# su1phurd/UAV-WRF-LES-PPO-LSTM

Hardware: AMD Instinct MI355X
Metric: env-steps/sec (rollout + GAE + 5-epoch PPO update), 4096 envs x 128 T per GPU, LSTM h=128 x1 (higher is better)
Workload: dtype f32

## Files before the change

### include/uavppo.h

```cpp
#ifndef UAVPPO_H
#define UAVPPO_H

#include <stddef.h>
#include <stdint.h>

#ifdef __cplusplus
extern "C" {
#endif

typedef struct uav_ctx uav_ctx;
typedef void* uav_stream;

#define UAV_ABI_VERSION 9

#define UAV_GAE_REFERENCE_EXACT 0
#define UAV_GAE_STANDARD        1
#define UAV_GAE_INLINE_V10      2

#define UAV_ENV_V20 0
#define UAV_ENV_V21 1
#define UAV_ENV_V11 2

#define UAV_FIELD_PROCEDURAL   0
#define UAV_FIELD_MATERIALISED 1

int         uav_abi_version(void);
const char* uav_last_error(void);

int  uav_create(uav_ctx** out, int device, size_t ws_bytes);
void uav_destroy(uav_ctx* ctx);

#define UAV_ARITH_FP16X3   0
#define UAV_ARITH_BF16X6   1
#define UAV_ARITH_F32_MFMA 2
int uav_set_lstm_arith(uav_ctx* ctx, int mode);
int uav_get_lstm_arith(const uav_ctx* ctx);
#define UAV_DEBUG_STEP_F32 1u
#define UAV_DEBUG_X_F32    2u
#define UAV_DEBUG_DG_F32   4u
#define UAV_DEBUG_GEMM_TN_OFF 0x10u
int uav_set_debug_flags(uav_ctx* ctx, unsigned flags);
int uav_absmax(uav_ctx* ctx, const float* x, int64_t n, float* out, uav_stream stream);

int uav_gae(uav_ctx* ctx, const float* rew, const float* val, const float* done,
            const float* last_val, int n_env, int horizon, float gamma, float lam, int mode,
            float* adv, uav_stream stream);

int uav_adv_stats(uav_ctx* ctx, const float* adv, int64_t n, double* stats3, uav_stream stream);
int uav_adv_normalise(uav_ctx* ctx, const float* adv, const float* val, int64_t n,
                      const double* stats3, float* adv_out, float* ret_out, uav_stream stream);
int uav_adv_normalise_inline(uav_ctx* ctx, const float* adv, const float* val, int64_t n,
                             const double* stats3, float* adv_out, float* ret_out, uav_stream stream);

int uav_pack_success_bits(uav_ctx* ctx, const uint8_t* flags, int64_t n, int cap, uint8_t* msg, uav_stream stream);

int uav_ppo_loss(uav_ctx* ctx, const float* logits, const float* value, const int32_t* act,
                 const float* logp_old, const float* adv, const float* ret, const float* val_old,
                 int64_t n, int n_act, float inv_n, float clip, float ent_beta,
                 double* loss_sums, float* dlogits, float* dvalue, float* dhead_bias,
                 uav_stream stream);

int uav_ppo_loss_from_y(uav_ctx* ctx, const float* y, const float* w_head, const float* b_head,
                        const int32_t* act, const float* logp_old, const float* adv, const float* ret,
                        const float* val_old, int64_t n, int hidden, int n_act, float inv_n, float clip,
                        float ent_beta, double* loss_sums, float* dheads, float* dhead_bias,
                        uav_stream stream);

int uav_policy_sample(uav_ctx* ctx, const float* logits, int64_t n, int n_act, const float* u,
                      uint64_t seed, uint64_t counter, int64_t index_offset, const int32_t* forced_act,
                      int32_t* act_out, float* logp_out, float* probs_out, int32_t* nan_count,
                      uav_stream stream);

int uav_policy_sample_at(uav_ctx* ctx, const float* heads, int64_t heads_stride, int64_t n, int n_act, uint64_t seed,
                         uint64_t counter, int64_t index_offset, const int32_t* forced_act, int32_t* act_out, int T, int t,
                         int32_t* act_buf, float* val_buf, float* logp_buf, int32_t* nan_count, uav_stream stream);
int uav_store_transition(uav_ctx* ctx, int n, int T, int t, float* keep, const float* rew, const float* done,
                         const uint8_t* flags, float* keep_buf, float* rew_buf, float* done_buf, uint8_t* flags_buf,
                         uav_stream stream);

int uav_clip_adam(uav_ctx* ctx, float* param, const float* grad, float* exp_avg,
                  float* exp_avg_sq, int64_t n, int64_t step, float lr, float beta1, float beta2,
                  float eps, float max_norm, float* gnorm_out, float* pmax_out, uav_stream stream);
int uav_clip_adamw(uav_ctx* ctx, float* param, const float* grad, float* exp_avg, float* exp_avg_sq, int64_t n,
                   int64_t step, float lr, float beta1, float beta2, float eps, float weight_decay, float max_norm,
                   float* gnorm_out, uav_stream stream);
int uav_smooth_l1(uav_ctx* ctx, const float* pred, const float* target, int64_t n, float beta, double* loss_mean,
                  float* dpred, uav_stream stream);
int uav_mse_bce(uav_ctx* ctx, const float* out, const float* target, int64_t n, double* loss_mean, float* dout,
                uav_stream stream);

size_t uav_disc_param_count(int obs_dim, int n_act, int hidden);

int uav_disc_grad(uav_ctx* ctx, const float* params, const float* obs_e, const int32_t* act_e, int64_t n_e, const float* obs_p,
                  const int32_t* act_p, int64_t n_p, int obs_dim, int n_act, int hidden, float inv_ne, float inv_np,
                  double* loss_sums, float* grad, uav_stream stream);

int uav_disc_reward(uav_ctx* ctx, const float* params, const float* obs, const int32_t* act, int64_t n, int obs_dim, int n_act,
                    int hidden, float env_coef, float gail_coef, const float* rew_env, float* rew_out, uav_stream stream);

size_t uav_lstm_stepper_bytes(int N, int I, int H);
int uav_lstm_stepper_begin(uav_ctx* ctx, void* state, const float* w_ih, const float* w_hh, const float* b_ih,
                           const float* b_hh, const float* h0, const float* c0, int N, int I, int H, uav_stream stream);
int uav_lstm_stepper_step(uav_ctx* ctx, void* state, const float* x, const void* below, const float* keep_t, int N, int T,
                          int t, int I, int H, float* y, float* stash, float* hn, float* cn, uav_stream stream);
typedef struct uav_stepper_call {
    void* state; const float* x; const void* below; const float* keep_t;
    int t, I;
    float *y, *stash, *hn, *cn;
} uav_stepper_call;
int uav_lstm_stepper_step_pair(uav_ctx* ctx, const uav_stepper_call* a, const uav_stepper_call* b, int N, int T, int H,
                               uav_stream stream);

int uav_gemm_f32(uav_ctx* ctx, int64_t M, int64_t N, int64_t K, const float* A, int64_t sa_m,
                 int64_t sa_k, const float* B, int64_t sb_k, int64_t sb_n, float* C, int64_t ldc,
                 const float* bias, int accumulate, uav_stream stream);

int uav_gemm_f16x3(uav_ctx* ctx, int64_t M, int64_t N, int64_t K, const float* A, int64_t sa_m,
                   int64_t sa_k, const float* B, int64_t sb_k, int64_t sb_n, float* C, int64_t ldc,
                   const float* bias, int accumulate, const float* a_absmax, uav_stream stream);

int uav_colsum(uav_ctx* ctx, const float* x, int64_t rows, int cols, float* out, uav_stream stream);
int uav_ln_relu(uav_ctx* ctx, float* z, float* a, float* rstd, const float* gamma, const float* beta, int64_t rows,
                int cols, uav_stream stream);
int uav_ln_relu_bwd(uav_ctx* ctx, float* d, const float* xhat, const float* rstd, const float* gamma, const float* beta,
                    int64_t rows, int cols, float* dgamma, float* dbeta, uav_stream stream);

int64_t uav_mlp_param_count(int in_dim, int h1, int h2, int n_act);
int64_t uav_mlp_stash_floats(int h1, int h2);
int uav_mlp_fwd(uav_ctx* ctx, const float* params, const float* x, int64_t B, int in_dim, int h1,
                int h2, int n_act, float* heads, float* stash, uav_stream stream);
int uav_mlp_bwd(uav_ctx* ctx, const float* params, const float* x, float* stash,
                const float* dheads, int64_t B, int in_dim, int h1, int h2, int n_act,
                float* grad, uav_stream stream);

int uav_mlp_ppo_grad(uav_ctx* ctx, const float* params, const float* obs, const int32_t* act, const float* logp_old,
                     const float* adv, const float* ret, const float* val_old, int64_t n, int in_dim, int h1, int h2,
                     int n_act, float inv_n, float clip, float ent_beta, double* loss_sums, float* grad,
                     uav_stream stream);

int uav_mlp_ppo_grad_trend(uav_ctx* ctx, const float* params, const float* obs, const int32_t* act, const float* logp_old,
                           const float* adv, const float* ret, const float* val_old, int64_t n, int trend_k, float inv_n,
                           float clip, float ent_beta, double* loss_sums, float* grad, uav_stream stream);

int uav_mlp_ppo_grad_rows(uav_ctx* ctx, const float* params, const float* obs, const int32_t* act, const float* logp_old,
                          const float* adv, const float* ret, const float* val_old, int64_t n_total, const int32_t* rows,
                          int64_t n_rows, int trend_k, float inv_n, float clip, float ent_beta, double* loss_sums, float* grad,
                          uav_stream stream);

typedef struct uav_gather_spec {
    const void* src;
    void* dst;
    int64_t row_bytes;
    int32_t planes;
    int32_t pad_;
    int64_t src_plane_stride_bytes;
    int64_t dst_plane_stride_bytes;
} uav_gather_spec;
#define UAV_GATHER_MAX_SPECS 12

int uav_gather_rows_multi(uav_ctx* ctx, const int32_t* idx, int64_t n_sel, int64_t n_rows, const uav_gather_spec* specs,
                          int n_specs, uav_stream stream);

int uav_lstm_fwd(uav_ctx* ctx, const float* x, const float* keep, const float* h0, const float* c0,
                 const float* w_ih, const float* w_hh, const float* b_ih, const float* b_hh,
                 int N, int T, int I, int H, float* y, float* hn, float* cn, float* stash,
                 const float* w_head, const float* b_head, int n_heads, float* heads,
                 uav_stream stream);
int uav_lstm_bwd(uav_ctx* ctx, const float* keep, const float* stash, const float* w_hh,
                 const float* dy, const float* dheads, const float* w_head, int n_heads,
                 const float* dhn, const float* dcn, int N, int T, int H, float* dgates, float* dh0,
                 float* dc0, const float* w_ih, int I, float* dx, uav_stream stream);
size_t uav_lstm_dgates_bytes(uav_ctx* ctx, int N, int T, int H);
int uav_lstm_dgates_f32(uav_ctx* ctx, const float* dgates, int N, int T, int H, float* out, uav_stream stream);
#define UAV_BWD_FUSES_DX 1
#define UAV_BWD_TAKES_DHEADS 2
#define UAV_BWD_STACKS 4
int uav_lstm_bwd_caps(uav_ctx* ctx, int I, int H);
typedef struct uav_lstm_bwd_layer {
    const float* keep;
    const float* stash;
    const float* w_hh;
    const float* w_ih;
    float* dgates;
    float* dx;
    const float* dhn;
    const float* dcn;
    float* dh0;
    float* dc0;
} uav_lstm_bwd_layer;
int uav_lstm_bwd_stack(uav_ctx* ctx, int n_layers, const uav_lstm_bwd_layer* layers, const float* dy, const float* dheads,
                       const float* w_head, int n_heads, int N, int T, int H, uav_stream stream);
int uav_lstm_wgrad(uav_ctx* ctx, const float* x, const float* keep, const float* h0, const float* y,
                   const float* stash, const float* dgates, const float* w_ih, const float* dheads,
                   int n_heads, int N, int T, int I, int H, float* dw_ih, float* dw_hh, float* db, float* db_hh,
                   float* dw_head, float* dx, uav_stream stream);
int uav_lstm_chunk_states(uav_ctx* ctx, const float* y, const float* stash, const float* keep, const float* h0, const float* c0,
                          int N, int T, int H, int chunk, float* h_out, float* c_out, uav_stream stream);

typedef struct uav_env_cfg {
    int32_t variant;
    int32_t field_mode;
    int32_t n_fields;
    int32_t bonus_is_f64;
    int32_t env_offset;
    int32_t n_env_total;
    int32_t trend_k;
    int32_t pad_;
    double  radius;
    double  bonus;
    uint64_t seed;
    const double* bank;
    const double* bank_src;
    const void*   curriculum;
} uav_env_cfg;

int uav_episode_rows(uav_ctx* ctx, const float* rew, const float* info, const uint8_t* flags, int n_env, int T, int env_offset,
                     double* carry, double* rows, int cap, int32_t* count, uav_stream stream);
size_t uav_curriculum_state_bytes(void);
int uav_curriculum_init(uav_ctx* ctx, void* state, double radius, double bonus, int bonus_is_f64, uav_stream stream);
int uav_curriculum_update(uav_ctx* ctx, void* state, const uint8_t* msgs, int world, int cap, uav_stream stream);

size_t uav_env_state_bytes(int n_env);
int uav_env_reset(uav_ctx* ctx, void* state, int n_env, const uav_env_cfg* cfg ,
                  float* obs_out, uav_stream stream);
int uav_env_step(uav_ctx* ctx, void* state, int n_env, const uav_env_cfg* cfg ,
                 const int32_t* act, const double* noise, float* obs_out, float* rew, float* done,
                 uint8_t* flags, float* info, float* term_obs, double* rew64, uav_stream stream);
int uav_env_peek(uav_ctx* ctx, const void* state, int n_env, float* pos, double* source,
                 int32_t* steps, int32_t* episode, uav_stream stream);

int uav_env_materialise(uav_ctx* ctx, const void* state, int n_env, const uav_env_cfg* cfg ,
                        int env_index, double* field_out, uav_stream stream);

int uav_rollout(uav_ctx* ctx, void* env_state, int n_env, const uav_env_cfg* cfg ,
                int policy_kind, const float* params, int hidden, int horizon, uint64_t iter,
                float* cur_obs, float* h, float* c, float* obs, int32_t* act, float* rew,
                float* val, float* logp, float* done, uint8_t* flags, float* keep, float* last_val,
                const int32_t* forced_act, const double* noise, int32_t* nan_count,
                float* stash, float* y_out, float* info, float* heads, uav_stream stream);

int uav_greedy_episodes(uav_ctx* ctx, void* env_state, int n_env, const uav_env_cfg* cfg , int policy_kind,
                        const float* params, int hidden, int steps, float* cur_obs, float* h, float* c, uint8_t* active,
                        const double* noise, int32_t* act, float* obs, float* pos, uint8_t* flags, int32_t* nan_count,
                        uav_stream stream);

typedef struct uav_stop_rule {
    int32_t window;
    float   pos_std_max, conc_coef, conc_peak, conc_min;
} uav_stop_rule;

int uav_greedy_episodes_stop(uav_ctx* ctx, void* env_state, int n_env, const uav_env_cfg* cfg , int policy_kind,
                             const float* params, int hidden, int steps, float* cur_obs, float* h, float* c, uint8_t* active,
                             const double* noise, int32_t* act, float* obs, float* pos, uint8_t* flags, int32_t* nan_count,
                             const uav_stop_rule* rule , float* stop_win, int32_t* stop_cnt, float* rule_val,
                             uav_stream stream);

int uav_stop_stability(uav_ctx* ctx, int n, const uav_stop_rule* rule , const float* pos, const float* obs2,
                       int64_t obs2_stride, const uint8_t* active, float* stop_win, int32_t* stop_cnt, uint8_t* stop,
                       float* value, uav_stream stream);

size_t uav_peak_stop_param_count(int hidden);

int uav_peak_stop_scan(uav_ctx* ctx, const float* params, int hidden, int window, const float* series, int64_t row_stride,
                       int64_t elem_stride, int n, int steps, const uint8_t* active, float* hist, int32_t* hist_cnt,
                       float prob_min, float* peak, float* prob, int32_t* first_hit, uav_stream stream);

int uav_threshold_windows(uav_ctx* ctx, const float* series, int64_t row_stride, int64_t elem_stride, int n, int steps,
                          const uint8_t* active, const float* hist, const int32_t* step_cnt, int window, int every, int min_steps,
                          double lo, double scale, double conc_scale, float* x, uav_stream stream);

int uav_threshold_rule(uav_ctx* ctx, const float* series, int64_t row_stride, int64_t elem_stride, int n, int steps,
                       const uint8_t* active, float* hist, int32_t* step_cnt, int window, int every, int min_steps, double conc_scale,
                       double factor, const float* pred, double* thr, int32_t* first_hit, uint8_t* stop, double* thr_out,
                       uav_stream stream);

int uav_rollout_tail(uav_ctx* ctx, void* env_state, int n_env, const uav_env_cfg* cfg , const float* y, int64_t y_stride,
                     int hidden, const float* w_head, const float* b_head, int n_act, float* heads, int64_t heads_stride, int T,
                     int t, uint64_t seed, uint64_t counter, int64_t index_offset, const int32_t* forced_act, const double* noise,
                     int32_t* act_out, float* cur_obs, float* obs_seq, float* keep, int32_t* act_buf, float* val_buf,
                     float* logp_buf, float* keep_buf, float* rew_buf, float* done_buf, uint8_t* flags_buf, int32_t* nan_count,
                     uav_stream stream);

int uav_greedy_tail(uav_ctx* ctx, void* env_state, int n_env, const uav_env_cfg* cfg , const float* y, int64_t y_stride,
                    int hidden, const float* w_head, const float* b_head, int n_act, int steps, int t, const double* noise_t,
                    float* cur_obs, uint8_t* active, int32_t* act, float* obs, float* pos, uint8_t* flags, int32_t* nan_count,
                    const uav_stop_rule* rule , float* stop_win, int32_t* stop_cnt, float* rule_val, uav_stream stream);

#define UAV_COMM_ID_BYTES 128
int uav_rccl_version(int* out );
int uav_comm_unique_id(void* id_out );
int uav_comm_init(uav_ctx* ctx, const void* id , int rank, int world);
int uav_comm_world(const uav_ctx* ctx);
int uav_comm_rank(const uav_ctx* ctx);
int uav_comm_destroy(uav_ctx* ctx);
int uav_allreduce(uav_ctx* ctx, float* flat_grad, int64_t count, uav_stream stream);
int uav_allreduce_f64(uav_ctx* ctx, double* buf, int64_t count, uav_stream stream);
int uav_allgather_bytes(uav_ctx* ctx, const void* send, void* recv, int64_t bytes_per_rank, uav_stream stream);

#ifdef __cplusplus
}
#endif
#endif
```

### uav-wrf-les-ppo-lstm_amd/csrc/common.h

```cpp
#pragma once
#include <hip/hip_runtime.h>
#include <stdint.h>
#include <stdio.h>
#include <stdlib.h>
#include <string.h>
#include "../../include/uavppo.h"

struct uav_form_table {
    struct { const void* p; int v; } e[8];
    int next;
    void record(const void* p, int v) {
        for (auto& x : e)
            if (x.p == p) { x.v = v; return; }
        e[next] = {p, v};
        next = (next + 1) % 8;
    }
    int find(const void* p) const {
        for (auto& x : e)
            if (x.p == p) return x.v;
        return -1;
    }
};
struct uav_ctx {
    int device;
    int num_cu;
    void* ws;
    size_t ws_bytes;
    double* pow075;
    double* wave;
    double* ftab;
    int lstm_arith;
    unsigned debug;
    hipStream_t side[3];
    hipEvent_t side_ev[8];
    void* comm;
    int comm_rank, comm_world;
    uav_form_table dg_form;
    uav_form_table hslot_form;
};
static inline void uav_dg_record(uav_ctx* ctx, const void* p, int packed) { ctx->dg_form.record(p, packed); }
static inline int uav_dg_form(const uav_ctx* ctx, const void* p) { return ctx->dg_form.find(p); }

extern thread_local int g_uav_arith;
extern thread_local unsigned g_uav_debug;
static inline bool uav_want_f32_mfma() { return g_uav_arith == UAV_ARITH_F32_MFMA; }
static inline bool uav_want_bf16x6() { return g_uav_arith == UAV_ARITH_BF16X6; }
static inline bool uav_debug(unsigned bit) { return (g_uav_debug & bit) != 0; }
static inline void uav_enter(const struct uav_ctx* ctx);

static inline void uav_enter(const uav_ctx* ctx) {
    g_uav_arith = ctx->lstm_arith;
    g_uav_debug = ctx->debug;
}

void uav_set_error(const char* fmt, ...);

hipError_t uav_dyn_lds(const void* kernel, int bytes);

#define UAV_CHECK_HIP(expr)                                                          \
    do {                                                                             \
        hipError_t e_ = (expr);                                                      \
        if (e_ != hipSuccess) {                                                      \
            uav_set_error("%s:%d: %s -> %s", __FILE__, __LINE__, #expr, hipGetErrorString(e_)); \
            return 1;                                                                \
        }                                                                            \
    } while (0)

#define UAV_REQUIRE(cond, ...)                                                       \
    do {                                                                             \
        if (!(cond)) {                                                               \
            uav_set_error(__VA_ARGS__);                                              \
            return 2;                                                                \
        }                                                                            \
    } while (0)

#define UAV_LAUNCH_CHECK() UAV_CHECK_HIP(hipGetLastError())

static inline hipStream_t as_stream(uav_stream s) { return reinterpret_cast<hipStream_t>(s); }

constexpr int WAVE = 64;

__device__ __forceinline__ void lds_barrier() {
    asm volatile("s_waitcnt lgkmcnt(0)\n\ts_barrier" ::: "memory");
}

__device__ __forceinline__ float fast_sigmoid(float x) { return __builtin_amdgcn_rcpf(1.0f + __expf(-x)); }
__device__ __forceinline__ float fast_tanh(float x) {
    const float big = 1.0f - 2.0f * __builtin_amdgcn_rcpf(__expf(2.0f * x) + 1.0f);
#ifdef UAV_TANH_LEGACY
    return big;
#else
    const float x2 = x * x;
    float p = __builtin_fmaf(x2, 62.0f / 2835.0f, -17.0f / 315.0f);
    p = __builtin_fmaf(p, x2, 2.0f / 15.0f);
    p = __builtin_fmaf(p, x2, -1.0f / 3.0f);
    p = __builtin_fmaf(p, x2, 1.0f);
    return __builtin_fabsf(x) < 0.25f ? x * p : big;
#endif
}

typedef __bf16 bf16x8 __attribute__((ext_vector_type(8)));
__device__ __forceinline__ void split3(float a, __bf16& p0, __bf16& p1, __bf16& p2) {
    p0 = (__bf16)a;
    const float r1 = a - (float)p0;
    p1 = (__bf16)r1;
    p2 = (__bf16)(r1 - (float)p1);
}
__device__ __forceinline__ unsigned short bf_bits(__bf16 v) { return __builtin_bit_cast(unsigned short, v); }

typedef _Float16 f16x8 __attribute__((ext_vector_type(8)));
constexpr float H3_LO = 1.0f / 2048.0f;
__device__ __forceinline__ void split2h(float a, _Float16& p0, _Float16& p1) {
    p0 = (_Float16)a;
    p1 = (_Float16)((a - (float)p0) * 2048.0f);
}
__device__ __forceinline__ unsigned short h_bits(_Float16 v) { return __builtin_bit_cast(unsigned short, v); }

typedef float f32x4 __attribute__((ext_vector_type(4)));

struct SplitF16x3 {
    typedef _Float16 piece;
    typedef f16x8 vec;
    static constexpr int NP = 2;
    static constexpr bool BLOCK_SCALE = true;
    static constexpr bool DG_STORES_LATE = true;
    static constexpr int fwd_park(int) { return 0; }
    static constexpr int bwd_park(int) { return 0; }
    __device__ __forceinline__ static void split(float a, piece (&p)[NP]) { split2h(a, p[0], p[1]); }
    __device__ __forceinline__ static unsigned short bits(piece v) { return h_bits(v); }
    __device__ __forceinline__ static f32x4 mma(vec a, vec b, f32x4 c) { return __builtin_amdgcn_mfma_f32_16x16x32_f16(a, b, c, 0, 0, 0); }
    template <class W>
    __device__ __forceinline__ static void gates_slab(f32x4 (&acc)[4], f32x4 (&acl)[4], W w, const vec (&a)[NP]) {
#pragma unroll
        for (int q = 0; q < 4; ++q) acl[q] = mma(w(q, 1), a[0], acl[q]);
#pragma unroll
        for (int q = 0; q < 4; ++q) acc[q] = mma(w(q, 0), a[0], acc[q]);
#pragma unroll
        for (int q = 0; q < 4; ++q) acl[q] = mma(w(q, 0), a[1], acl[q]);
    }
    template <class W, class B>
    __device__ __forceinline__ static void head_slab(f32x4& ha, f32x4& hb, W w, B h) {
        hb = mma(w(1), h(0), hb);
        hb = mma(w(0), h(1), hb);
        ha = mma(w(0), h(0), ha);
    }
    template <class V> __device__ __forceinline__ static V sum(V acc, V acl) { return acc + acl * H3_LO; }
    template <class W>
    __device__ __forceinline__ static void tile_slab(f32x4& a0, f32x4& a1, W w, const vec (&b)[NP]) {
        a1 = mma(w(1), b[0], a1);
        a0 = mma(w(0), b[0], a0);
        a1 = mma(w(0), b[1], a1);
    }
    __device__ __forceinline__ static f32x4 tile_sum(f32x4 a0, f32x4 a1) { return a0 + a1 * H3_LO; }
};

struct SplitBf16x6 {
    typedef __bf16 piece;
    typedef bf16x8 vec;
    static constexpr int NP = 3;
    static constexpr bool BLOCK_SCALE = false;
    static constexpr bool DG_STORES_LATE = false;
    static constexpr int fwd_park(int H) { return H >= 128 ? 3 : 0; }
    static constexpr int bwd_park(int H) { return H >= 128 ? 6 : 0; }
    __device__ __forceinline__ static void split(float a, piece (&p)[NP]) { split3(a, p[0], p[1], p[2]); }
    __device__ __forceinline__ static unsigned short bits(piece v) { return bf_bits(v); }
    __device__ __forceinline__ static f32x4 mma(vec a, vec b, f32x4 c) { return __builtin_amdgcn_mfma_f32_16x16x32_bf16(a, b, c, 0, 0, 0); }
    template <class W>
    __device__ __forceinline__ static void gates_slab(f32x4 (&acc)[4], f32x4 (&)[4], W w, const vec (&a)[NP]) {
#pragma unroll
        for (int q = 0; q < 4; ++q) acc[q] = mma(w(q, 0), a[2], acc[q]);
#pragma unroll
        for (int q = 0; q < 4; ++q) acc[q] = mma(w(q, 1), a[1], acc[q]);
#pragma unroll
        for (int q = 0; q < 4; ++q) acc[q] = mma(w(q, 2), a[0], acc[q]);
#pragma unroll
        for (int q = 0; q < 4; ++q) acc[q] = mma(w(q, 0), a[1], acc[q]);
#pragma unroll
        for (int q = 0; q < 4; ++q) acc[q] = mma(w(q, 1), a[0], acc[q]);
#pragma unroll
        for (int q = 0; q < 4; ++q) acc[q] = mma(w(q, 0), a[0], acc[q]);
    }
    template <class W, class B>
    __device__ __forceinline__ static void head_slab(f32x4& ha, f32x4&, W w, B h) {
        ha = mma(w(0), h(2), ha);
        ha = mma(w(1), h(1), ha);
        ha = mma(w(2), h(0), ha);
        ha = mma(w(0), h(1), ha);
        ha = mma(w(1), h(0), ha);
        ha = mma(w(0), h(0), ha);
    }
    template <class V> __device__ __forceinline__ static V sum(V acc, V) { return acc; }
    template <class W>
    __device__ __forceinline__ static void tile_slab(f32x4& a0, f32x4& a1, W w, const vec (&b)[NP]) {
        a0 = mma(w(0), b[2], a0);
        a1 = mma(w(1), b[1], a1);
        a0 = mma(w(2), b[0], a0);
        a1 = mma(w(0), b[1], a1);
        a0 = mma(w(1), b[0], a0);
        a1 = mma(w(0), b[0], a1);
    }
    __device__ __forceinline__ static f32x4 tile_sum(f32x4 a0, f32x4 a1) { return a0 + a1; }
};

struct DgPack {
    static constexpr int H = 256, NS = 4 * H / 32;
    int N, T, NP, RT;
    __host__ __device__ DgPack(int n, int t) : N(n), T(t), NP((n + 63) / 64 * 64), RT(NP / 16) {}
    __host__ __device__ size_t step_halves() const { return (size_t)RT * NS * 1024; }
    __host__ __device__ size_t piece_bytes() const { return (size_t)T * step_halves() * 2; }
    __host__ __device__ size_t bytes() const { return piece_bytes() + 2 * (size_t)T * NP * sizeof(float); }
    __host__ __device__ unsigned short* pieces(void* base, int t) const { return (unsigned short*)base + (size_t)t * step_halves(); }
    __host__ __device__ const unsigned short* pieces(const void* base, int t) const { return (const unsigned short*)base + (size_t)t * step_halves(); }
    __host__ __device__ float* isc(void* base, int t) const { return (float*)((char*)base + piece_bytes()) + (size_t)t * NP; }
    __host__ __device__ const float* isc(const void* base, int t) const { return (const float*)((const char*)base + piece_bytes()) + (size_t)t * NP; }
    __host__ __device__ float* iscm(void* base, int t) const { return isc(base, T) + (size_t)t * NP; }
    __host__ __device__ const float* iscm(const void* base, int t) const { return isc(base, T) + (size_t)t * NP; }
};

__device__ __forceinline__ double wave_sum(double v) {
#pragma unroll
    for (int o = 32; o > 0; o >>= 1) v += __shfl_down(v, o, 64);
    return v;
}
__device__ __forceinline__ float wave_sum(float v) {
#pragma unroll
    for (int o = 32; o > 0; o >>= 1) v += __shfl_down(v, o, 64);
    return v;
}
__device__ __forceinline__ float wave_allsum(float v) {
#pragma unroll
    for (int o = 32; o > 0; o >>= 1) v += __shfl_xor(v, o, 64);
    return v;
}
template <typename T>
__device__ __forceinline__ T block256_sum(T v, T* sm) {
    v = wave_sum(v);
    const int lane = threadIdx.x & 63, w = threadIdx.x >> 6;
    if (lane == 0) sm[w] = v;
    __syncthreads();
    T r = T(0);
    if (threadIdx.x == 0) r = ((sm[0] + sm[1]) + sm[2]) + sm[3];
    __syncthreads();
    return r;
}
```

### uav-wrf-les-ppo-lstm_amd/csrc/ctx.hip

```cpp
#include <stdarg.h>
#include <mutex>
#include <set>
#include <utility>
#include "common.h"

static thread_local char g_err[512] = "";
thread_local int g_uav_arith = 0;
thread_local unsigned g_uav_debug = 0;
int env_init_tables(uav_ctx* ctx);

void uav_set_error(const char* fmt, ...) {
    va_list ap;
    va_start(ap, fmt);
    vsnprintf(g_err, sizeof(g_err), fmt, ap);
    va_end(ap);
}

hipError_t uav_dyn_lds(const void* kernel, int bytes) {
    static std::mutex mu;
    static std::set<std::pair<int, const void*>> done;
    int dev = 0;
    hipError_t e = hipGetDevice(&dev);
    if (e != hipSuccess) return e;
    std::lock_guard<std::mutex> lock(mu);
    if (done.count({dev, kernel})) return hipSuccess;
    e = hipFuncSetAttribute(kernel, hipFuncAttributeMaxDynamicSharedMemorySize, bytes);
    if (e == hipSuccess) done.insert({dev, kernel});
    return e;
}

extern "C" {

int uav_abi_version(void) { return UAV_ABI_VERSION; }
const char* uav_last_error(void) { return g_err; }

int uav_create(uav_ctx** out, int device, size_t ws_bytes) {
    UAV_REQUIRE(out != nullptr, "uav_create: out is NULL");
    UAV_REQUIRE(ws_bytes >= (1u << 20), "uav_create: ws_bytes must be >= 1 MiB");
    UAV_CHECK_HIP(hipSetDevice(device));
    hipDeviceProp_t prop;
    UAV_CHECK_HIP(hipGetDeviceProperties(&prop, device));
    UAV_REQUIRE(strncmp(prop.gcnArchName, "gfx950", 6) == 0,
                "libuavppo is built for gfx950 (MI355X) only; device %d is %s", device, prop.gcnArchName);
    uav_ctx* c = new uav_ctx();
    c->device = device;
    c->num_cu = prop.multiProcessorCount;
    c->ws_bytes = ws_bytes;
    c->pow075 = nullptr;
    c->wave = nullptr;
    c->ftab = nullptr;
    c->comm = nullptr;
    c->comm_rank = -1;
    c->comm_world = 0;
    c->lstm_arith = getenv("UAV_LSTM_F32_MFMA") ? UAV_ARITH_F32_MFMA : (getenv("UAV_LSTM_BF16X6") ? UAV_ARITH_BF16X6 : UAV_ARITH_FP16X3);
    c->debug = (getenv("UAV_LSTM_STEP_F32") ? UAV_DEBUG_STEP_F32 : 0u) | (getenv("UAV_LSTM_X_F32") ? UAV_DEBUG_X_F32 : 0u) |
               (getenv("UAV_LSTM_DG_F32") ? UAV_DEBUG_DG_F32 : 0u);
    if (hipMalloc(&c->ws, ws_bytes) != hipSuccess) {
        (void)hipFree(c->ws);
        delete c;
        uav_set_error("uav_create: hipMalloc(%zu) failed", ws_bytes);
        return 1;
    }
    if (env_init_tables(c) != 0) {
        (void)hipFree(c->ws);
        (void)hipFree(c->pow075);
        (void)hipFree(c->wave);
        (void)hipFree(c->ftab);
        delete c;
        return 1;
    }
    *out = c;
    return 0;
}

int uav_set_lstm_arith(uav_ctx* ctx, int mode) {
    UAV_REQUIRE(ctx && mode >= UAV_ARITH_FP16X3 && mode <= UAV_ARITH_F32_MFMA, "uav_set_lstm_arith: bad argument");
    ctx->lstm_arith = mode;
    return 0;
}
int uav_get_lstm_arith(const uav_ctx* ctx) { return ctx ? ctx->lstm_arith : -1; }

int uav_set_debug_flags(uav_ctx* ctx, unsigned flags) {
    UAV_REQUIRE(ctx && (flags & ~(UAV_DEBUG_STEP_F32 | UAV_DEBUG_X_F32 | UAV_DEBUG_DG_F32 | UAV_DEBUG_GEMM_TN_OFF)) == 0, "uav_set_debug_flags: bad argument");
    ctx->debug = flags;
    return 0;
}

void uav_destroy(uav_ctx* ctx) {
    if (!ctx) return;
    (void)uav_comm_destroy(ctx);
    for (auto& e : ctx->side_ev)
        if (e) (void)hipEventDestroy(e);
    for (auto& s : ctx->side)
        if (s) (void)hipStreamDestroy(s);
    (void)hipFree(ctx->ws);
    (void)hipFree(ctx->pow075);
    (void)hipFree(ctx->wave);
    (void)hipFree(ctx->ftab);
    delete ctx;
}

}
```

### uav-wrf-les-ppo-lstm_amd/csrc/lstm.hip

```cpp
#include <stdlib.h>
#include <type_traits>
#include "common.h"

int gemm_f32(uav_ctx* ctx, int64_t M, int64_t N, int64_t K, const float* A, int64_t sa_m, int64_t sa_k,
             const float* B, int64_t sb_k, int64_t sb_n, float* C, int64_t ldc, const float* bias,
             int accumulate, hipStream_t st);
int colsum(uav_ctx* ctx, const float* X, int64_t B, int C, float* out, float* scratch, hipStream_t st);
int colsum_absmax(uav_ctx* ctx, const float* X, int64_t B, int C, float* out, float* scratch, unsigned* absmax_bits,
                  hipStream_t st);
int colsum_xw(uav_ctx* ctx, const float* X, int64_t B, int C, const float* x, int I, float* colsum_out, float* xw_out,
              float* scratch, unsigned* absmax_bits, hipStream_t st, int xw_transposed = 0);
bool gemm_h3_ok(int64_t M, int64_t N, int64_t K, const float* A, int64_t sa_m, int64_t sa_k, const float* B, int64_t sb_k,
                int64_t sb_n);
int gemm_h3(uav_ctx* ctx, int64_t M, int64_t N, int64_t K, const float* A, int64_t sa_m, int64_t sa_k, const float* B,
            int64_t sb_k, int64_t sb_n, float* C, int64_t ldc, const float* bias, int accumulate, const unsigned* a_absmax,
            hipStream_t st);
int lstm_generic_fwd(uav_ctx* ctx, const float* keep, const float* h0, const float* c0, const float* w_hh, int N, int T,
                     int H, float* y, float* hn, float* cn, float* stash, hipStream_t st);
int lstm_h3_fwd(uav_ctx* ctx, const float* x, int I, const float* w_ih, const float* b_ih, const float* b_hh,
                const float* keep, const float* h0, const float* c0, const float* w_hh, int N, int T, float* y, float* hn,
                float* cn, float* stash, hipStream_t st);
bool lstm_h3_step_path(int H);
int lstm_generic_bwd(uav_ctx* ctx, const float* keep, const float* stash, const float* w_hh, const float* dy,
                     const float* dheads, const float* w_head, int n_heads,
                     const float* dhn, const float* dcn, int N, int T, int H, float* dgates, float* dh0, float* dc0,
                     const float* w_ih, int I, float* dx, hipStream_t st);
int lstm_generic_bwd_caps(int I, int H);
bool lstm_h3_stack_ok(int H);
bool lstm_h3_dg_packed(int H);
int lstm_pc_unpack(const void* dgates, int N, int T, float* out, hipStream_t st);
int lstm_pc_hprev_rows(const float* y, const float* keep, const float* h0, int N, int T, float* out, hipStream_t st);
int lstm_pc_wgrad(uav_ctx* ctx, const float* x, const float* y, const float* h0, const void* dgates, int N, int T, int I, float* dw_ih,
                  float* dw_hh, float* db, float* db_hh, hipStream_t st);
int lstm_h3_bwd_stack(uav_ctx* ctx, int nl, const uav_lstm_bwd_layer* layers, const float* dy, const float* dheads,
                      const float* w_head, int n_heads, int N, int T, hipStream_t st);
int lstm_wgrad_fused(uav_ctx* ctx, const float* dgates, const float* y, const float* keep, const float* h0,
                     const float* x, int I, const float* dheads, int NH, int N, int T, int H,
                     float* dw_ih, float* dw_hh, float* db, float* db_hh, float* dw_head, hipStream_t st);

constexpr int MT = 16;
constexpr int TC = 32;

#define sigmoidf_ fast_sigmoid
#define tanhf_ fast_tanh

template <int H>
struct FwdGeom {
    static constexpr int NW = H / 16;
    static constexpr int KS = H / 4;
    static constexpr int SEG = KS + 4;
    static constexpr int S = 4 * SEG + 8;
    static constexpr size_t LDS = (2 * MT * S + TC * MT * 8 + (TC + 1) * MT) * sizeof(float);
};
template <int H>
__device__ __forceinline__ int hpos(int u) { return (u / (H / 4)) * FwdGeom<H>::SEG + (u % (H / 4)); }

template <int H, bool FUSE_X>
__global__ __launch_bounds__(H * 4) void lstm_fwd_kernel(
    const float* __restrict__ x, const float* __restrict__ keep, const float* __restrict__ h0,
    const float* __restrict__ c0, const float* __restrict__ w_ih, const float* __restrict__ w_hh,
    const float* __restrict__ b_ih, const float* __restrict__ b_hh, int N, int T, int I,
    float* __restrict__ y, float* __restrict__ hn, float* __restrict__ cn, float* __restrict__ stash) {
    using G = FwdGeom<H>;
    constexpr int KS = G::KS, SEG = G::SEG, S = G::S;
    extern __shared__ __attribute__((aligned(16))) float smem[];
    float* hbuf = smem;
    float* xbuf = hbuf + 2 * MT * S;
    float* kbuf = xbuf + TC * MT * 8;

    const int lane = threadIdx.x & 63, w = threadIdx.x >> 6;
    const int j = lane & 15, kq = lane >> 4;
    const int u = 16 * w + j;
    const int n0 = blockIdx.x * MT;

    float wh[4][KS];
#pragma unroll
    for (int q = 0; q < 4; ++q) {
        const float* src = w_hh + (size_t)(q * H + u) * H + kq * KS;
#pragma unroll
        for (int s = 0; s < KS; s += 4) {
            const float4 v = *reinterpret_cast<const float4*>(src + s);
            wh[q][s] = v.x; wh[q][s + 1] = v.y; wh[q][s + 2] = v.z; wh[q][s + 3] = v.w;
        }
    }
    float wx[4][2], bias[4];
#pragma unroll
    for (int q = 0; q < 4; ++q) {
        bias[q] = FUSE_X ? (b_ih[q * H + u] + b_hh[q * H + u]) : 0.f;
#pragma unroll
        for (int s = 0; s < 2; ++s) {
            const int k = 2 * kq + s;
            wx[q][s] = (FUSE_X && k < I) ? w_ih[(size_t)(q * H + u) * I + k] : 0.f;
        }
    }

    float c_reg[4], hin[4];
#pragma unroll
    for (int r = 0; r < 4; ++r) {
        const int e = 4 * kq + r;
        const int n = min(n0 + e, N - 1);
        const float k0 = keep ? keep[(size_t)n * T] : 1.f;
        c_reg[r] = c0[(size_t)n * H + u] * k0;
        hin[r] = h0[(size_t)n * H + u] * k0;
        hbuf[e * S + hpos<H>(u)] = hin[r];
    }
    int cur = 0;
    float h_last[4] = {0.f, 0.f, 0.f, 0.f};

    for (int t0 = 0; t0 < T; t0 += TC) {
        const int tc = min(TC, T - t0);
        if (FUSE_X) {
            for (int idx = threadIdx.x; idx < MT * tc * 8; idx += blockDim.x) {
                const int e = idx / (tc * 8), rem = idx % (tc * 8), tt = rem >> 3, f = rem & 7;
                const int n = min(n0 + e, N - 1);
                xbuf[(tt * MT + e) * 8 + f] = (f < I) ? x[((size_t)n * T + t0 + tt) * I + f] : 0.f;
            }
        }
        for (int idx = threadIdx.x; idx < MT * (tc + 1); idx += blockDim.x) {
            const int e = idx / (tc + 1), tt = idx % (tc + 1);
            const int n = min(n0 + e, N - 1);
            kbuf[tt * MT + e] = (keep && t0 + tt < T) ? keep[(size_t)n * T + t0 + tt] : 1.f;
        }
        lds_barrier();

        for (int tt = 0; tt < tc; ++tt) {
            const int t = t0 + tt;
            f32x4 acc[4];
#pragma unroll
            for (int q = 0; q < 4; ++q) {
                if (FUSE_X) {
                    acc[q] = f32x4{bias[q], bias[q], bias[q], bias[q]};
                } else {
#pragma unroll
                    for (int r = 0; r < 4; ++r) {
                        const int n = min(n0 + 4 * kq + r, N - 1);
                        acc[q][r] = stash[((size_t)n * T + t) * (6 * H) + q * H + u];
                    }
                }
            }
            if (FUSE_X) {
                const float2 ax = *reinterpret_cast<const float2*>(&xbuf[(tt * MT + j) * 8 + 2 * kq]);
#pragma unroll
                for (int q = 0; q < 4; ++q) {
                    acc[q] = __builtin_amdgcn_mfma_f32_16x16x4f32(ax.x, wx[q][0], acc[q], 0, 0, 0);
                    acc[q] = __builtin_amdgcn_mfma_f32_16x16x4f32(ax.y, wx[q][1], acc[q], 0, 0, 0);
                }
            }
            const float* hrow = hbuf + cur * MT * S + j * S + kq * SEG;
#pragma unroll
            for (int s = 0; s < KS; s += 4) {
                const float4 a = *reinterpret_cast<const float4*>(hrow + s);
#pragma unroll
                for (int q = 0; q < 4; ++q) acc[q] = __builtin_amdgcn_mfma_f32_16x16x4f32(a.x, wh[q][s], acc[q], 0, 0, 0);
#pragma unroll
                for (int q = 0; q < 4; ++q) acc[q] = __builtin_amdgcn_mfma_f32_16x16x4f32(a.y, wh[q][s + 1], acc[q], 0, 0, 0);
#pragma unroll
                for (int q = 0; q < 4; ++q) acc[q] = __builtin_amdgcn_mfma_f32_16x16x4f32(a.z, wh[q][s + 2], acc[q], 0, 0, 0);
#pragma unroll
                for (int q = 0; q < 4; ++q) acc[q] = __builtin_amdgcn_mfma_f32_16x16x4f32(a.w, wh[q][s + 3], acc[q], 0, 0, 0);
            }
            float* hnext = hbuf + (cur ^ 1) * MT * S;
#pragma unroll
            for (int r = 0; r < 4; ++r) {
                const int e = 4 * kq + r;
                const int n = n0 + e;
                const float gi = sigmoidf_(acc[0][r]), gf = sigmoidf_(acc[1][r]);
                const float gg = tanhf_(acc[2][r]), go = sigmoidf_(acc[3][r]);
                const float cp = c_reg[r];
                const float c = gf * cp + gi * gg;
                const float h = go * tanhf_(c);
                const float kn = kbuf[(tt + 1) * MT + e];
                if (n < N) {
                    const size_t row = (size_t)n * T + t;
                    y[row * H + u] = h;
                    if (stash) {
                        float* sp = stash + row * (6 * H);
                        sp[u] = gi; sp[H + u] = gf; sp[2 * H + u] = gg; sp[3 * H + u] = go;
                        sp[4 * H + u] = cp;
                        if (I > 6) sp[5 * H + u] = hin[r];
                    }
                }
                h_last[r] = h;
                if (t == T - 1) c_reg[r] = c;
                else c_reg[r] = c * kn;
                hin[r] = h * kn;
                hnext[e * S + hpos<H>(u)] = hin[r];
            }
            cur ^= 1;
            lds_barrier();
// ... 299 lines not shown
    float* __restrict__ y, float* __restrict__ hn, float* __restrict__ cn, float* __restrict__ stash,
    const float* __restrict__ w_head, const float* __restrict__ b_head, int NHD, float* __restrict__ heads) {
    lstm_fwd_split<SplitBf16x6, H, FUSE_X>(x, keep, h0, c0, w_ih, w_hh, b_ih, b_hh, N, T, I, y, hn, cn, stash, w_head,
                                           b_head, NHD, heads);
}

template <int H>
struct BwdGeom {
    static constexpr int S = 4 * H + 4;
    static constexpr size_t LDS = (2 * MT * S + TC * MT * 8 + (TC + 1) * MT) * sizeof(float);
};

template <int H>
__global__ __launch_bounds__(H * 4) void lstm_bwd_kernel(
    const float* __restrict__ keep, const float* __restrict__ stash, const float* __restrict__ w_hh,
    const float* __restrict__ dy, const float* __restrict__ dheads, const float* __restrict__ w_head, int NH,
    const float* __restrict__ dhn, const float* __restrict__ dcn, int N, int T, float* __restrict__ dgates,
    float* __restrict__ dh0, float* __restrict__ dc0) {
    using G = BwdGeom<H>;
    constexpr int S = G::S;
    extern __shared__ __attribute__((aligned(16))) float smem[];
    float* dgbuf = smem;
    float* dhbuf = dgbuf + 2 * MT * S;
    float* kbuf = dhbuf + TC * MT * 8;

    const int lane = threadIdx.x & 63, w = threadIdx.x >> 6;
    const int j = lane & 15, kq = lane >> 4;
    const int u = 16 * w + j;
    const int n0 = blockIdx.x * MT;

    float wt[H];
#pragma unroll
    for (int s = 0; s < H; ++s) wt[s] = w_hh[(size_t)(kq * H + s) * H + u];
    float whb[2];
#pragma unroll
    for (int a = 0; a < 2; ++a) whb[a] = (dheads && 4 * a + kq < NH) ? w_head[(size_t)(4 * a + kq) * H + u] : 0.f;

    float dh_rec[4], dc_next[4];
    size_t srow[4];
#pragma unroll
    for (int r = 0; r < 4; ++r) {
        const int n = min(n0 + 4 * kq + r, N - 1);
        dh_rec[r] = dhn ? dhn[(size_t)n * H + u] : 0.f;
        dc_next[r] = dcn ? dcn[(size_t)n * H + u] : 0.f;
        srow[r] = (size_t)n * T;
    }
    float pf[4][5], pdy[4];
    auto prefetch = [&](int t) {
#pragma unroll
        for (int r = 0; r < 4; ++r) {
            const float* sp = stash + (srow[r] + t) * (6 * H);
            pf[r][0] = sp[u]; pf[r][1] = sp[H + u]; pf[r][2] = sp[2 * H + u]; pf[r][3] = sp[3 * H + u];
            pf[r][4] = sp[4 * H + u];
            pdy[r] = dy ? dy[(srow[r] + t) * H + u] : 0.f;
        }
    };
    prefetch(T - 1);
    int cur = 0;
    const int nchunk = (T + TC - 1) / TC;
    for (int ch = nchunk - 1; ch >= 0; --ch) {
        const int t0 = ch * TC, tc = min(TC, T - t0);
        if (dheads) {
            for (int idx = threadIdx.x; idx < MT * tc * 8; idx += blockDim.x) {
                const int e = idx / (tc * 8), rem = idx % (tc * 8), tt = rem >> 3, f = rem & 7;
                const int n = min(n0 + e, N - 1);
                dhbuf[(tt * MT + e) * 8 + f] = (f < NH) ? dheads[((size_t)n * T + t0 + tt) * NH + f] : 0.f;
            }
        }
        for (int idx = threadIdx.x; idx < MT * tc; idx += blockDim.x) {
            const int e = idx / tc, tt = idx % tc;
            const int n = min(n0 + e, N - 1);
            kbuf[tt * MT + e] = keep ? keep[(size_t)n * T + t0 + tt] : 1.f;
        }
        lds_barrier();
        for (int tt = tc - 1; tt >= 0; --tt) {
            const int t = t0 + tt;
            float* dgw = dgbuf + cur * MT * S;
            f32x4 dyacc = {0.f, 0.f, 0.f, 0.f};
            if (dheads) {
                const float* dr = &dhbuf[(tt * MT + j) * 8];
                dyacc = __builtin_amdgcn_mfma_f32_16x16x4f32(dr[kq], whb[0], dyacc, 0, 0, 0);
                dyacc = __builtin_amdgcn_mfma_f32_16x16x4f32(dr[4 + kq], whb[1], dyacc, 0, 0, 0);
            }
#pragma unroll
            for (int r = 0; r < 4; ++r) {
                const int e = 4 * kq + r;
                const float gi = pf[r][0], gf = pf[r][1], gg = pf[r][2], go = pf[r][3], cp = pf[r][4];
                const float dyv = dheads ? dyacc[r] : pdy[r];
                const float dh = dyv + dh_rec[r];
                const float c = gf * cp + gi * gg;
                const float tch = tanhf_(c);
                const float dc = dh * go * (1.0f - tch * tch) + dc_next[r];
                const float dgi = dc * gg * gi * (1.0f - gi);
                const float dgf = dc * cp * gf * (1.0f - gf);
                const float dgg = dc * gi * (1.0f - gg * gg);
                const float dgo = dh * tch * go * (1.0f - go);
                const float kp = kbuf[tt * MT + e];
                dc_next[r] = dc * gf * kp;
                dgw[e * S + 0 * H + u] = dgi;
                dgw[e * S + 1 * H + u] = dgf;
                dgw[e * S + 2 * H + u] = dgg;
                dgw[e * S + 3 * H + u] = dgo;
                if (n0 + e < N) {
                    float* gp = dgates + (srow[r] + t) * (4 * H);
                    gp[u] = dgi; gp[H + u] = dgf; gp[2 * H + u] = dgg; gp[3 * H + u] = dgo;
                }
            }
            if (t > 0) prefetch(t - 1);
            lds_barrier();
            f32x4 a0 = {0.f, 0.f, 0.f, 0.f}, a1 = a0, a2 = a0, a3 = a0;
            const float* drow = dgw + j * S + kq * H;
#pragma unroll
            for (int s = 0; s < H; s += 4) {
                const float4 a = *reinterpret_cast<const float4*>(drow + s);
                a0 = __builtin_amdgcn_mfma_f32_16x16x4f32(a.x, wt[s], a0, 0, 0, 0);
                a1 = __builtin_amdgcn_mfma_f32_16x16x4f32(a.y, wt[s + 1], a1, 0, 0, 0);
                a2 = __builtin_amdgcn_mfma_f32_16x16x4f32(a.z, wt[s + 2], a2, 0, 0, 0);
                a3 = __builtin_amdgcn_mfma_f32_16x16x4f32(a.w, wt[s + 3], a3, 0, 0, 0);
            }
#pragma unroll
            for (int r = 0; r < 4; ++r) {
                const float kp = kbuf[tt * MT + 4 * kq + r];
                dh_rec[r] = ((a0[r] + a1[r]) + (a2[r] + a3[r])) * kp;
            }
            cur ^= 1;
        }
        lds_barrier();
    }
#pragma unroll
    for (int r = 0; r < 4; ++r) {
        const int n = n0 + 4 * kq + r;
        if (n < N) {
            if (dh0) dh0[(size_t)n * H + u] = dh_rec[r];
            if (dc0) dc0[(size_t)n * H + u] = dc_next[r];
        }
    }
}

template <class P, int H>
struct BwdSplitGeom {
    static constexpr int NW = H / 16;
    static constexpr int SLOT = 5 * MT * 16;
    static constexpr int SMALL = 128;
    static constexpr int PK = P::bwd_park(H);
    static constexpr int WPARK = PK * 64 * 8;
    static constexpr size_t LDS = (NW * NW * 64 * 4  + NW * SLOT + 2 * SMALL) * sizeof(float) +
                                  NW * WPARK * sizeof(unsigned short);
};

template <class P, int H>
__device__ __forceinline__ void lstm_bwd_split(
    const float* __restrict__ keep, const float* __restrict__ stash, const float* __restrict__ w_hh,
    const float* __restrict__ dheads, const float* __restrict__ w_head, int NH, const float* __restrict__ dhn,
    const float* __restrict__ dcn, int N, int T, float* __restrict__ dgates, float* __restrict__ dh0,
    float* __restrict__ dc0) {
    using G = BwdSplitGeom<P, H>;
    using vec = typename P::vec;
    using piece = typename P::piece;
    constexpr int NP = P::NP, SLOT = G::SLOT, NW = G::NW, SMALL = G::SMALL, PK = G::PK, WPARK = G::WPARK;
    extern __shared__ __attribute__((aligned(16))) float smem[];
    f32x4* part = reinterpret_cast<f32x4*>(smem);
    float* ring = smem + NW * NW * 64 * 4;
    float* small = ring + NW * SLOT;
    unsigned short* wpark = reinterpret_cast<unsigned short*>(small + 2 * SMALL);

    const int lane = threadIdx.x & 63;
    const int w = __builtin_amdgcn_readfirstlane(threadIdx.x >> 6);
    const int j = lane & 15, kq = lane >> 4;
    const int uw = 16 * w + j;
    const int uo = 16 * w + 4 * kq;
    const int n0 = blockIdx.x * MT;
    const int n = min(n0 + j, N - 1);
    const bool live = n0 + j < N;

    vec wa[NW][2][NP];
    vec* const wpk = reinterpret_cast<vec*>(wpark + w * WPARK) + lane;
#pragma unroll
    for (int m = 0; m < NW; ++m)
#pragma unroll
        for (int sb = 0; sb < 2; ++sb) {
#pragma unroll
            for (int e = 0; e < 8; ++e) {
                const int k = (2 * sb + e / 4) * H + 16 * w + 4 * kq + (e % 4);
                piece p[NP];
                P::split(w_hh[(size_t)k * H + 16 * m + j], p);
#pragma unroll
                for (int pc = 0; pc < NP; ++pc) wa[m][sb][pc][e] = p[pc];
            }
            if (2 * m + sb < PK) wpk[(2 * m + sb) * 64] = wa[m][sb][NP - 1];
        }
    float whb[2];
#pragma unroll
    for (int a = 0; a < 2; ++a) whb[a] = (4 * a + kq < NH) ? w_head[(size_t)(4 * a + kq) * H + uw] : 0.f;

    float dh_rec[4], dc_next[4];
    {
        const float4 a4 = dhn ? *reinterpret_cast<const float4*>(dhn + (size_t)n * H + uo) : float4{0.f, 0.f, 0.f, 0.f};
        const float4 c4 = dcn ? *reinterpret_cast<const float4*>(dcn + (size_t)n * H + uo) : float4{0.f, 0.f, 0.f, 0.f};
        dh_rec[0] = a4.x; dh_rec[1] = a4.y; dh_rec[2] = a4.z; dh_rec[3] = a4.w;
        dc_next[0] = c4.x; dc_next[1] = c4.y; dc_next[2] = c4.z; dc_next[3] = c4.w;
    }
    const size_t srow = (size_t)n * T;

    typedef __attribute__((address_space(3))) float lds_f;
    const int e_d = lane >> 2, g4 = lane & 3;
    const size_t drow = (size_t)min(n0 + e_d, N - 1) * T;
    const unsigned ring_base = __builtin_amdgcn_readfirstlane((unsigned)(unsigned long)((lds_f*)(ring + w * SLOT)));
    const unsigned small_base = __builtin_amdgcn_readfirstlane((unsigned)(unsigned long)((lds_f*)small));
    auto issue = [&](int t) {
        const float* src = stash + (drow + t) * (6 * H) + 16 * w + 4 * g4;
        unsigned m0save;
        asm volatile(
            "s_mov_b32 %0, m0\n\t"
            "s_mov_b32 m0, %6\n\ts_nop 0\n\tglobal_load_lds_dwordx4 %1, off\n\t"
            "s_add_u32 m0, m0, 1024\n\ts_nop 0\n\tglobal_load_lds_dwordx4 %2, off\n\t"
            "s_add_u32 m0, m0, 1024\n\ts_nop 0\n\tglobal_load_lds_dwordx4 %3, off\n\t"
            "s_add_u32 m0, m0, 1024\n\ts_nop 0\n\tglobal_load_lds_dwordx4 %4, off\n\t"
            "s_add_u32 m0, m0, 1024\n\ts_nop 0\n\tglobal_load_lds_dwordx4 %5, off\n\t"
            "s_mov_b32 m0, %0"
            : "=&s"(m0save)
            : "v"(src), "v"(src + H), "v"(src + 2 * H), "v"(src + 3 * H), "v"(src + 4 * H), "s"(ring_base)
            : "memory", "scc");
    };
    const float* small_at0;
    unsigned small_stride;
    {
        const int e = w * 64 + lane;
        if (e < 16 * NH) { small_at0 = dheads + (size_t)min(n0 + e / NH, N - 1) * T * NH + e % NH; small_stride = (unsigned)NH; }
        else if (e >= 112 && keep) { small_at0 = keep + (size_t)min(n0 + e - 112, N - 1) * T; small_stride = 1u; }
        else { small_at0 = w_hh + (lane & 15); small_stride = 0u; }
    }
    auto issue_small = [&](int t, int slot) {
        const float* src = small_at0 + (size_t)((unsigned)t * small_stride);
        const unsigned dst = small_base + (unsigned)((slot * SMALL + w * 64) * 4);
        unsigned m0save;
        asm volatile("s_mov_b32 %0, m0\n\ts_mov_b32 m0, %2\n\ts_nop 0\n\tglobal_load_lds_dword %1, off\n\ts_mov_b32 m0, %0"
                     : "=&s"(m0save) : "v"(src), "s"(dst) : "memory");
    };
    const bool small_wave = w < 2;
    issue(T - 1);
    if (small_wave) {
        issue_small(T - 1, (T - 1) & 1);
        issue_small(T >= 2 ? T - 2 : 0, (T - 2) & 1);
    }
    bool first = true;
    X6_PROF_DECL;
    for (int t = T - 1; t >= 0; --t) {
        X6_PROF_MARK(0);
        if (first) asm volatile("s_waitcnt vmcnt(0)" ::: "memory");
        else if (small_wave) asm volatile("s_waitcnt vmcnt(5)" ::: "memory");
        else asm volatile("s_waitcnt vmcnt(4)" ::: "memory");
        first = false;
        const float* sl = ring + w * SLOT + j * 16 + 4 * kq;
        float4 pf[5];
#pragma unroll
        for (int q = 0; q < 5; ++q) pf[q] = *reinterpret_cast<const float4*>(sl + q * 256);
        asm volatile("s_waitcnt lgkmcnt(0)" ::: "memory");
        issue(t >= 1 ? t - 1 : 0);
        X6_PROF_MARK(1);
        lds_barrier();
        X6_PROF_MARK(2);
        const float* sm = small + (t & 1) * SMALL;
        f32x4 dyacc = {0.f, 0.f, 0.f, 0.f};
        {
            const float d0 = (kq < NH) ? sm[j * NH + kq] : 0.f;
            const float d1 = (4 + kq < NH) ? sm[j * NH + 4 + kq] : 0.f;
            dyacc = __builtin_amdgcn_mfma_f32_16x16x4f32(whb[0], d0, dyacc, 0, 0, 0);
            dyacc = __builtin_amdgcn_mfma_f32_16x16x4f32(whb[1], d1, dyacc, 0, 0, 0);
        }
        const float kp = keep ? sm[112 + j] : 1.f;
        const float gi[4] = {pf[0].x, pf[0].y, pf[0].z, pf[0].w}, gf[4] = {pf[1].x, pf[1].y, pf[1].z, pf[1].w};
        const float gg[4] = {pf[2].x, pf[2].y, pf[2].z, pf[2].w}, go[4] = {pf[3].x, pf[3].y, pf[3].z, pf[3].w};
        const float cp[4] = {pf[4].x, pf[4].y, pf[4].z, pf[4].w};
        float dg[4][4];
#pragma unroll
        for (int r = 0; r < 4; ++r) {
            const float dh = dyacc[r] + dh_rec[r];
            const float c = __builtin_fmaf(gf[r], cp[r], gi[r] * gg[r]);
            const float tch = tanhf_(c);
            const float dc = dh * go[r] * (1.0f - tch * tch) + dc_next[r];
            dg[0][r] = dc * gg[r] * gi[r] * (1.0f - gi[r]);
            dg[1][r] = dc * cp[r] * gf[r] * (1.0f - gf[r]);
            dg[2][r] = dc * gi[r] * (1.0f - gg[r] * gg[r]);
            dg[3][r] = dh * tch * go[r] * (1.0f - go[r]);
            dc_next[r] = dc * gf[r] * kp;
        }
        int ex = 0;
        float unscale = 1.f;
        if constexpr (P::BLOCK_SCALE) {
            float mx = 0.f;
#pragma unroll
            for (int q = 0; q < 4; ++q)
#pragma unroll
                for (int r = 0; r < 4; ++r) mx = fmaxf(mx, fabsf(dg[q][r]));
            {
                const unsigned u = __builtin_bit_cast(unsigned, mx);
                const auto s16 = __builtin_amdgcn_permlane16_swap(u, u, false, false);
                mx = fmaxf(__builtin_bit_cast(float, (unsigned)s16[0]), __builtin_bit_cast(float, (unsigned)s16[1]));
                const unsigned v = __builtin_bit_cast(unsigned, mx);
                const auto s32 = __builtin_amdgcn_permlane32_swap(v, v, false, false);
                mx = fmaxf(__builtin_bit_cast(float, (unsigned)s32[0]), __builtin_bit_cast(float, (unsigned)s32[1]));
            }
            ex = 14 - __builtin_amdgcn_frexp_expf(mx);
            ex = mx > 0.f ? min(max(ex, -100), 100) : 0;
            unscale = __builtin_amdgcn_ldexpf(1.0f, -ex);
        }
        auto store_dg = [&](int q) {
            if (live) *reinterpret_cast<float4*>(dgates + (srow + t) * (4 * H) + q * H + uo) = float4{dg[q][0], dg[q][1], dg[q][2], dg[q][3]};
        };
        vec bp[2][NP];
#pragma unroll
        for (int q = 0; q < 4; ++q) {
#pragma unroll
            for (int r = 0; r < 4; ++r) {
                piece p[NP];
                P::split(P::BLOCK_SCALE ? __builtin_amdgcn_ldexpf(dg[q][r], ex) : dg[q][r], p);
#pragma unroll
                for (int pc = 0; pc < NP; ++pc) bp[q >> 1][pc][4 * (q & 1) + r] = p[pc];
            }
            if constexpr (!P::DG_STORES_LATE) store_dg(q);
        }
        X6_PROF_DEP(bp[1][NP - 1]); X6_PROF_DEP(bp[0][0]);
        X6_PROF_MARK(3);
#pragma unroll
        for (int m = 0; m < NW; ++m) {
            f32x4 a0 = {0.f, 0.f, 0.f, 0.f}, a1 = a0;
#pragma unroll
            for (int sb = 0; sb < 2; ++sb) {
                const int item = 2 * m + sb;
                P::tile_slab(a0, a1, [&](int p) { return (p == NP - 1 && item < PK) ? wpk[item * 64] : wa[m][sb][p]; }, bp[sb]);
            }
            part[(m * NW + w) * 64 + lane] = P::tile_sum(a0, a1) * unscale;
        }
        if constexpr (P::DG_STORES_LATE) {
#pragma unroll
            for (int q = 0; q < 4; ++q) store_dg(q);
        }
        asm volatile("s_waitcnt lgkmcnt(0)" ::: "memory");
        X6_PROF_MARK(4);
        lds_barrier();
        X6_PROF_MARK(5);
        if (small_wave) issue_small(t >= 2 ? t - 2 : 0, t & 1);
        f32x4 sum = part[(w * NW) * 64 + lane];
#pragma unroll
        for (int ww = 1; ww < NW; ++ww) sum += part[(w * NW + ww) * 64 + lane];
#pragma unroll
        for (int r = 0; r < 4; ++r) dh_rec[r] = sum[r] * kp;
        X6_PROF_DEP(dh_rec[3]);
        X6_PROF_MARK(6);
    }
    X6_PROF_FLUSH8();
    asm volatile("s_waitcnt vmcnt(0)" ::: "memory");
    if (live) {
        if (dh0) *reinterpret_cast<float4*>(dh0 + (size_t)n * H + uo) = float4{dh_rec[0], dh_rec[1], dh_rec[2], dh_rec[3]};
        if (dc0) *reinterpret_cast<float4*>(dc0 + (size_t)n * H + uo) = float4{dc_next[0], dc_next[1], dc_next[2], dc_next[3]};
    }
}

template <int H>
__global__ __launch_bounds__(H * 4) void lstm_bwd_h3k_kernel(
    const float* __restrict__ keep, const float* __restrict__ stash, const float* __restrict__ w_hh,
    const float* __restrict__ dheads, const float* __restrict__ w_head, int NH, const float* __restrict__ dhn,
    const float* __restrict__ dcn, int N, int T, float* __restrict__ dgates, float* __restrict__ dh0,
    float* __restrict__ dc0) {
    lstm_bwd_split<SplitF16x3, H>(keep, stash, w_hh, dheads, w_head, NH, dhn, dcn, N, T, dgates, dh0, dc0);
}
template <int H>
__global__ __launch_bounds__(H * 4) void lstm_bwd_x6k_kernel(
    const float* __restrict__ keep, const float* __restrict__ stash, const float* __restrict__ w_hh,
    const float* __restrict__ dheads, const float* __restrict__ w_head, int NH, const float* __restrict__ dhn,
    const float* __restrict__ dcn, int N, int T, float* __restrict__ dgates, float* __restrict__ dh0,
    float* __restrict__ dc0) {
    lstm_bwd_split<SplitBf16x6, H>(keep, stash, w_hh, dheads, w_head, NH, dhn, dcn, N, T, dgates, dh0, dc0);
}

template <class P, int H, bool FUSE_X>
static constexpr auto fwd_split_kernel() {
    if constexpr (std::is_same<P, SplitF16x3>::value) return &lstm_fwd_h3_kernel<H, FUSE_X>;
    else return &lstm_fwd_x6_kernel<H, FUSE_X>;
}
template <class P, int H>
static constexpr auto bwd_split_kernel() {
    if constexpr (std::is_same<P, SplitF16x3>::value) return &lstm_bwd_h3k_kernel<H>;
    else return &lstm_bwd_x6k_kernel<H>;
}

template <class F>
static int with_split(F&& f) {
    return uav_want_bf16x6() ? f(SplitBf16x6{}) : f(SplitF16x3{});
}

template <class P, int H>
static int launch_bwd_split(const float* keep, const float* stash, const float* w_hh, const float* dheads,
                            const float* w_head, int NH, const float* dhn, const float* dcn, int N, int T, float* dgates,
                            float* dh0, float* dc0, hipStream_t st) {
    const dim3 grid((N + MT - 1) / MT), block(H * 4);
    const size_t lx = BwdSplitGeom<P, H>::LDS;
    constexpr auto kern = bwd_split_kernel<P, H>();
    UAV_CHECK_HIP(uav_dyn_lds(reinterpret_cast<const void*>(kern), (int)lx));
    hipLaunchKernelGGL(kern, grid, block, lx, st, keep, stash, w_hh, dheads, w_head, NH, dhn, dcn, N, T, dgates, dh0, dc0);
    UAV_LAUNCH_CHECK();
    return 0;
}

template <class P, int H>
static int launch_fwd_split(bool fuse, const float* x, const float* keep, const float* h0, const float* c0,
                            const float* w_ih, const float* w_hh, const float* b_ih, const float* b_hh, int N, int T, int I,
                            float* y, float* hn, float* cn, float* stash, const float* w_head, const float* b_head, int NHD,
                            float* heads, hipStream_t st) {
    const dim3 grid((N + MT - 1) / MT), block(H * 4);
    const size_t lx = FwdSplitGeom<P, H>::LDS;
    constexpr auto fused = fwd_split_kernel<P, H, true>(), unfused = fwd_split_kernel<P, H, false>();
    UAV_CHECK_HIP(uav_dyn_lds(reinterpret_cast<const void*>(fused), (int)lx));
    UAV_CHECK_HIP(uav_dyn_lds(reinterpret_cast<const void*>(unfused), (int)lx));
    hipLaunchKernelGGL(fuse ? fused : unfused, grid, block, lx, st, x, keep, h0, c0, w_ih, w_hh, b_ih, b_hh, N, T, I, y, hn,
                       cn, stash, w_head, b_head, NHD, heads);
    UAV_LAUNCH_CHECK();
    return 0;
}

template <int H>
static int launch_fwd(bool fuse, const float* x, const float* keep, const float* h0, const float* c0,
                      const float* w_ih, const float* w_hh, const float* b_ih, const float* b_hh, int N, int T, int I,
                      float* y, float* hn, float* cn, float* stash, const float* w_head, const float* b_head, int NHD,
                      float* heads, bool* heads_done, hipStream_t st) {
    if (!uav_want_f32_mfma()) {
        *heads_done = heads != nullptr;
        return with_split([&](auto p) {
            return launch_fwd_split<decltype(p), H>(fuse, x, keep, h0, c0, w_ih, w_hh, b_ih, b_hh, N, T, I, y, hn, cn, stash,
                                                    w_head, b_head, NHD, heads, st);
        });
    }
    const dim3 grid((N + MT - 1) / MT), block(H * 4);
    const size_t lds = FwdGeom<H>::LDS;
    if (fuse)
        hipLaunchKernelGGL((lstm_fwd_kernel<H, true>), grid, block, lds, st, x, keep, h0, c0, w_ih, w_hh, b_ih, b_hh, N,
                           T, I, y, hn, cn, stash);
    else
        hipLaunchKernelGGL((lstm_fwd_kernel<H, false>), grid, block, lds, st, x, keep, h0, c0, w_ih, w_hh, b_ih, b_hh,
                           N, T, I, y, hn, cn, stash);
    UAV_LAUNCH_CHECK();
    return 0;
}

template <int H>
static int launch_bwd(const float* keep, const float* stash, const float* w_hh, const float* dy, const float* dheads,
                      const float* w_head, int NH, const float* dhn, const float* dcn, int N, int T, float* dgates,
                      float* dh0, float* dc0, hipStream_t st) {
    const dim3 grid((N + MT - 1) / MT), block(H * 4);
    UAV_CHECK_HIP(uav_dyn_lds(reinterpret_cast<const void*>(&lstm_bwd_kernel<H>), (int)BwdGeom<H>::LDS));
    hipLaunchKernelGGL((lstm_bwd_kernel<H>), grid, block, BwdGeom<H>::LDS, st, keep, stash, w_hh, dy, dheads, w_head, NH,
                       dhn, dcn, N, T, dgates, dh0, dc0);
    UAV_LAUNCH_CHECK();
    return 0;
}

__global__ void add2_kernel(const float* a0, const float* a1, float* b, int n) {
    const int i = blockIdx.x * 256 + threadIdx.x;
    if (i < n) b[i] = a0[i] + a1[i];
}

static int lstm_bwd_seq(const float* keep, const float* stash, const float* w_hh, const float* dy,
                        const float* dheads, const float* w_head, int NH, const float* dhn, const float* dcn, int N,
                        int T, int H, float* dgates, float* dh0, float* dc0, hipStream_t st) {
    if (dheads && NH <= 7 && !uav_want_f32_mfma()) {
        return with_split([&](auto p) {
            using P = decltype(p);
            return H == 64 ? launch_bwd_split<P, 64>(keep, stash, w_hh, dheads, w_head, NH, dhn, dcn, N, T, dgates, dh0, dc0, st)
                           : launch_bwd_split<P, 128>(keep, stash, w_hh, dheads, w_head, NH, dhn, dcn, N, T, dgates, dh0, dc0, st);
        });
    }
    switch (H) {
        case 64: return launch_bwd<64>(keep, stash, w_hh, dy, dheads, w_head, NH, dhn, dcn, N, T, dgates, dh0, dc0, st);
        case 128: return launch_bwd<128>(keep, stash, w_hh, dy, dheads, w_head, NH, dhn, dcn, N, T, dgates, dh0, dc0, st);
    }
    uav_set_error("uav_lstm_bwd: H=%d unsupported (64, 128)", H);
    return 2;
}

extern "C" {

int uav_lstm_fwd(uav_ctx* ctx, const float* x, const float* keep, const float* h0, const float* c0, const float* w_ih,
                 const float* w_hh, const float* b_ih, const float* b_hh, int N, int T, int I, int H, float* y,
                 float* hn, float* cn, float* stash, const float* w_head, const float* b_head, int n_heads, float* heads,
                 uav_stream stream) {
    UAV_REQUIRE(ctx && x && h0 && c0 && w_ih && w_hh && b_ih && b_hh && y && hn && cn, "uav_lstm_fwd: NULL argument");
    uav_enter(ctx);
    UAV_REQUIRE(N > 0 && T > 0 && I > 0, "uav_lstm_fwd: N=%d T=%d I=%d", N, T, I);
    UAV_REQUIRE(!heads || (w_head && b_head && n_heads > 0 && n_heads <= 8), "uav_lstm_fwd: heads needs w_head, b_head, 1..8 heads");
    hipStream_t st = as_stream(stream);
    const bool persistent = (H == 64 || H == 128);
    const bool fuse = I <= 8 && persistent;
    const bool step256 = lstm_h3_step_path(H);
    if (step256) UAV_REQUIRE(stash, "uav_lstm_fwd: stash is required when H is not 64/128");
    if (!fuse && !step256) {
        UAV_REQUIRE(stash, "uav_lstm_fwd: stash is required when I > 8 or H is not 64/128");
        float* bsum = (float*)ctx->ws;
        uav_ctx sub = *ctx;
        sub.ws = (char*)ctx->ws + 65536;
        sub.ws_bytes = ctx->ws_bytes - 65536;
        hipLaunchKernelGGL(add2_kernel, dim3((4 * H + 255) / 256), dim3(256), 0, st, b_ih, b_hh, bsum, 4 * H);
        int rc = gemm_f32(&sub, (int64_t)N * T, 4 * H, I, x, I, 1, w_ih, 1, I, stash, 6 * H, bsum, 0, st);
        if (rc) return rc;
    }
    bool heads_done = false;
    int rc;
    switch (H) {
        case 64: rc = launch_fwd<64>(fuse, x, keep, h0, c0, w_ih, w_hh, b_ih, b_hh, N, T, I, y, hn, cn, stash, w_head, b_head, n_heads, heads, &heads_done, st); break;
        case 128: rc = launch_fwd<128>(fuse, x, keep, h0, c0, w_ih, w_hh, b_ih, b_hh, N, T, I, y, hn, cn, stash, w_head, b_head, n_heads, heads, &heads_done, st); break;
        default:
            rc = step256 ? lstm_h3_fwd(ctx, x, I, w_ih, b_ih, b_hh, keep, h0, c0, w_hh, N, T, y, hn, cn, stash, st)
                         : lstm_generic_fwd(ctx, keep, h0, c0, w_hh, N, T, H, y, hn, cn, stash, st);
    }
    if (rc) return rc;
    if (H == DgPack::H) ctx->hslot_form.record(stash, step256 && lstm_h3_dg_packed(H) ? 0 : 1);
    if (heads && !heads_done)
        return gemm_f32(ctx, (int64_t)N * T, n_heads, H, y, H, 1, w_head, 1, H, heads, n_heads, b_head, 0, st);
    return 0;
}

int uav_lstm_bwd_caps(uav_ctx* ctx, int I, int H) {
    if (!ctx) return 0;
    if (H == 64 || H == 128) return UAV_BWD_TAKES_DHEADS;
    uav_enter(ctx);
    return lstm_generic_bwd_caps(I, H);
}

size_t uav_lstm_dgates_bytes(uav_ctx* ctx, int N, int T, int H) {
    if (!ctx || N <= 0 || T <= 0 || H <= 0) return 0;
    uav_enter(ctx);
    if (H == DgPack::H && lstm_h3_dg_packed(H)) return DgPack(N, T).bytes();
    return (size_t)N * T * 4 * H * sizeof(float);
}

int uav_lstm_dgates_f32(uav_ctx* ctx, const float* dgates, int N, int T, int H, float* out, uav_stream stream) {
    UAV_REQUIRE(ctx && dgates && out && N > 0 && T > 0 && H > 0, "uav_lstm_dgates_f32: bad argument");
    uav_enter(ctx);
    const int form = H == DgPack::H ? uav_dg_form(ctx, dgates) : 0;
    if (form > 0 || (form < 0 && H == DgPack::H && lstm_h3_dg_packed(H))) return lstm_pc_unpack(dgates, N, T, out, as_stream(stream));
    UAV_CHECK_HIP(hipMemcpyAsync(out, dgates, (size_t)N * T * 4 * H * sizeof(float), hipMemcpyDeviceToDevice, as_stream(stream)));
    return 0;
}

int uav_lstm_bwd_stack(uav_ctx* ctx, int n_layers, const uav_lstm_bwd_layer* layers, const float* dy, const float* dheads,
                       const float* w_head, int n_heads, int N, int T, int H, uav_stream stream) {
    UAV_REQUIRE(ctx && layers, "uav_lstm_bwd_stack: NULL argument");
    uav_enter(ctx);
    UAV_REQUIRE((dy != nullptr) != (dheads != nullptr), "uav_lstm_bwd_stack: give exactly one of dy / dheads");
    UAV_REQUIRE(!dheads || (w_head && n_heads > 0 && n_heads <= 8), "uav_lstm_bwd_stack: dheads needs w_head and 1..8 heads");
    UAV_REQUIRE(N > 0 && T > 0, "uav_lstm_bwd_stack: N=%d T=%d", N, T);
    UAV_REQUIRE(H == 256 && lstm_h3_stack_ok(H), "uav_lstm_bwd_stack: H = 256 on the fp16-split arithmetic only (uav_lstm_bwd_caps)");
    return lstm_h3_bwd_stack(ctx, n_layers, layers, dy, dheads, w_head, n_heads, N, T, as_stream(stream));
}

int uav_lstm_bwd(uav_ctx* ctx, const float* keep, const float* stash, const float* w_hh, const float* dy,
                 const float* dheads, const float* w_head, int n_heads, const float* dhn, const float* dcn, int N,
                 int T, int H, float* dgates, float* dh0, float* dc0, const float* w_ih, int I, float* dx,
                 uav_stream stream) {
    UAV_REQUIRE(ctx && stash && w_hh && dgates, "uav_lstm_bwd: NULL argument");
    uav_enter(ctx);
    UAV_REQUIRE((dy != nullptr) != (dheads != nullptr), "uav_lstm_bwd: give exactly one of dy / dheads");
    UAV_REQUIRE(!dheads || (w_head && n_heads > 0 && n_heads <= 8), "uav_lstm_bwd: dheads needs w_head and 1..8 heads");
    UAV_REQUIRE(N > 0 && T > 0, "uav_lstm_bwd: N=%d T=%d", N, T);
    if (H != 64 && H != 128) {
        return lstm_generic_bwd(ctx, keep, stash, w_hh, dy, dheads, w_head, n_heads, dhn, dcn, N, T, H, dgates, dh0, dc0, w_ih, I, dx,
                                as_stream(stream));
    }
    UAV_REQUIRE(!dx, "uav_lstm_bwd: dx is not formed by the H = 64 / 128 sequence kernels (uav_lstm_wgrad does it)");
    return lstm_bwd_seq(keep, stash, w_hh, dy, dheads, w_head, n_heads, dhn, dcn, N, T, H, dgates, dh0, dc0,
                        as_stream(stream));
}

int uav_lstm_wgrad(uav_ctx* ctx, const float* x, const float* keep, const float* h0, const float* y,
                   const float* stash, const float* dgates, const float* w_ih, const float* dheads, int n_heads, int N,
                   int T, int I, int H, float* dw_ih, float* dw_hh, float* db, float* db_hh, float* dw_head, float* dx,
                   uav_stream stream) {
    UAV_REQUIRE(ctx && x && h0 && y && dgates && w_ih && dw_ih && dw_hh && db, "uav_lstm_wgrad: NULL argument");
    uav_enter(ctx);
    UAV_REQUIRE(N > 0 && T > 0 && I > 0 && H > 0, "uav_lstm_wgrad: N=%d T=%d I=%d H=%d", N, T, I, H);
    UAV_REQUIRE(!dheads || (dw_head && n_heads > 0 && n_heads <= 8), "uav_lstm_wgrad: dheads needs dw_head, 1..8 heads");
    hipStream_t st = as_stream(stream);
    const int64_t NT = (int64_t)N * T;
    int rc;
    if (I <= 6 && (H == 64 || H == 128)) {
        if ((rc = lstm_wgrad_fused(ctx, dgates, y, keep, h0, x, I, dheads, n_heads, N, T, H, dw_ih, dw_hh, db, db_hh,
                                   dw_head, st))) return rc;
    } else {
        UAV_REQUIRE(stash, "uav_lstm_wgrad: stash is required when I > 6");
        const size_t red_floats = (size_t)1024 * 9 * 4 * H + 64;
        UAV_REQUIRE(ctx->ws_bytes >= red_floats * sizeof(float) * 2, "uav_lstm_wgrad: workspace too small");
        float* red = (float*)((char*)ctx->ws + ctx->ws_bytes) - red_floats;
        uav_ctx sub = *ctx;
        sub.ws_bytes = ctx->ws_bytes - red_floats * sizeof(float);
        bool done = false;
        const float* hprev = stash + 5 * H;
        int64_t ld_hprev = 6 * H;
        {
            const int form = uav_dg_form(ctx, dgates), want = lstm_h3_dg_packed(H) ? 1 : 0;
            UAV_REQUIRE(form < 0 || H != DgPack::H || form == want, "uav_lstm_wgrad: this dgates buffer was written as %s but the handle's "
                        "arithmetic mode / debug flags now read %s (they must not change between uav_lstm_bwd and uav_lstm_wgrad)",
                        form ? "fp16 piece chunks" : "f32 rows", want ? "fp16 piece chunks" : "f32 rows");
            UAV_REQUIRE(H != DgPack::H || want || ctx->hslot_form.find(stash) != 0, "uav_lstm_wgrad: this stash was written by "
                        "uav_lstm_fwd / the stepper on the fp16-split arithmetic, which leaves out its h_prev slot, but the handle's "
                        "arithmetic mode / debug flags now read that slot (they must not change between the forward pass and "
                        "uav_lstm_wgrad)");
        }
        if (lstm_h3_dg_packed(H)) {
            if ((I <= 8 || I == H) && !dx) {
                if ((rc = lstm_pc_wgrad(ctx, x, y, h0, dgates, N, T, I, dw_ih, dw_hh, db, db_hh, st))) return rc;
                done = true;
            } else {
                const size_t f32_bytes = (size_t)NT * 5 * H * sizeof(float);
                UAV_REQUIRE(sub.ws_bytes >= f32_bytes + (64u << 20), "uav_lstm_wgrad (h=256, I=%d%s): needs %zu bytes of workspace for "
                            "the gate gradients and h_prev as f32 rows", I, dx ? ", dx" : "", f32_bytes + (64u << 20));
                float* rows = (float*)((char*)sub.ws + sub.ws_bytes - f32_bytes);
                sub.ws_bytes -= f32_bytes;
                if ((rc = lstm_pc_unpack(dgates, N, T, rows, st))) return rc;
                float* hp = rows + (size_t)NT * 4 * H;
                if ((rc = lstm_pc_hprev_rows(y, keep, h0, N, T, hp, st))) return rc;
                dgates = rows;
                hprev = hp;
                ld_hprev = H;
            }
        }
        const bool h3 = !uav_want_f32_mfma() && !uav_want_bf16x6() && (reinterpret_cast<uintptr_t>(dgates) & 15) == 0;
        unsigned* amax = h3 ? reinterpret_cast<unsigned*>(red + (size_t)1024 * 9 * 4 * H) : nullptr;
        auto product = [&](int64_t M, int64_t Nn, int64_t K, const float* A, int64_t sa_m, int64_t sa_k, const float* B,
                           int64_t sb_k, int64_t sb_n, float* C, int64_t ldc) {
            if (h3 && gemm_h3_ok(M, Nn, K, A, sa_m, sa_k, B, sb_k, sb_n))
                return gemm_h3(&sub, M, Nn, K, A, sa_m, sa_k, B, sb_k, sb_n, C, ldc, nullptr, 0, amax, st);
            return gemm_f32(&sub, M, Nn, K, A, sa_m, sa_k, B, sb_k, sb_n, C, ldc, nullptr, 0, st);
        };
        if (!done) {
            const bool narrow = I <= 8 && (reinterpret_cast<uintptr_t>(dgates) & 15) == 0;
            if (narrow) rc = colsum_xw(&sub, dgates, NT, 4 * H, x, I, db, dw_ih, red, amax, st);
            else rc = colsum_absmax(&sub, dgates, NT, 4 * H, db, red, amax, st);
            if (rc) return rc;
            if (db_hh) UAV_CHECK_HIP(hipMemcpyAsync(db_hh, db, (size_t)4 * H * sizeof(float), hipMemcpyDeviceToDevice, st));
            if ((rc = product(4 * H, H, NT, dgates, 1, 4 * H, hprev, ld_hprev, 1, dw_hh, H))) return rc;
            if (!narrow && (rc = product(4 * H, I, NT, dgates, 1, 4 * H, x, I, 1, dw_ih, I))) return rc;
        }
        if (dheads) {
            if (H % 4 == 0 && (reinterpret_cast<uintptr_t>(y) & 15) == 0)
                rc = colsum_xw(&sub, y, NT, H, dheads, n_heads, nullptr, dw_head, red, nullptr, st, 1);
            else
                rc = gemm_f32(&sub, n_heads, H, NT, dheads, 1, n_heads, y, H, 1, dw_head, H, nullptr, 0, st);
            if (rc) return rc;
        }
        if (dx) return product(NT, I, 4 * H, dgates, 4 * H, 1, w_ih, I, 1, dx, I);
        return 0;
    }
    if (dx) return gemm_f32(ctx, NT, I, 4 * H, dgates, 4 * H, 1, w_ih, I, 1, dx, I, nullptr, 0, st);
    return 0;
}

}
```

### uav-wrf-les-ppo-lstm_amd/csrc/wgrad.hip

```cpp
#include <stdlib.h>
#include <type_traits>
#include "common.h"

typedef float f32x4 __attribute__((ext_vector_type(4)));

constexpr int KC = 16;

template <int H>
struct WG {
    static constexpr int NW = H / 16;
    static constexpr int NT_ = H / 16 + 1;
    static constexpr int NC = H + 16;
    static constexpr int SG = 4 * H + 16;
    static constexpr int SB = H + 16;
    static constexpr int SY = H + 16;
    static constexpr int SD = 48;
    static constexpr int BUF = KC * (SG + SB + SY + SD);
    static constexpr size_t LDS = 2 * BUF * sizeof(float);
    static constexpr size_t SLAB = (size_t)4 * H * NC + 16 * H;
};

template <int H>
__global__ __launch_bounds__(H * 4) void lstm_wgrad_kernel(
    const float* __restrict__ dgates, const float* __restrict__ y, const float* __restrict__ keep,
// ... 95 lines not shown
            for (int mi = 0; mi < 4; ++mi) a[mi] = lg[kr * SG + 64 * w + 16 * mi + j];
#pragma unroll
            for (int ni = 0; ni < NT_; ++ni) b[ni] = lb[kr * SB + 16 * ni + j];
            const float ah = ld[kr * SD + j];
            const float bh = ly[kr * SY + 16 * w + j];
#pragma unroll
            for (int mi = 0; mi < 4; ++mi)
#pragma unroll
                for (int ni = 0; ni < NT_; ++ni)
                    acc[mi][ni] = __builtin_amdgcn_mfma_f32_16x16x4f32(a[mi], b[ni], acc[mi][ni], 0, 0, 0);
            acch = __builtin_amdgcn_mfma_f32_16x16x4f32(ah, bh, acch, 0, 0, 0);
        }
    }
    float* slab = slabs + (size_t)blockIdx.x * G::SLAB;
#pragma unroll
    for (int mi = 0; mi < 4; ++mi)
#pragma unroll
        for (int ni = 0; ni < NT_; ++ni)
#pragma unroll
            for (int r = 0; r < 4; ++r)
                slab[(size_t)(64 * w + 16 * mi + 4 * kq + r) * G::NC + 16 * ni + j] = acc[mi][ni][r];
#pragma unroll
    for (int r = 0; r < 4; ++r) slab[(size_t)4 * H * G::NC + (size_t)(4 * kq + r) * H + 16 * w + j] = acch[r];
}


constexpr int KS6 = 32;

__device__ __forceinline__ void mac6(f32x4& d, const bf16x8 (&a)[3], const bf16x8 (&b)[3]) {
    d = __builtin_amdgcn_mfma_f32_16x16x32_bf16(a[2], b[0], d, 0, 0, 0);
    d = __builtin_amdgcn_mfma_f32_16x16x32_bf16(a[1], b[1], d, 0, 0, 0);
    d = __builtin_amdgcn_mfma_f32_16x16x32_bf16(a[0], b[2], d, 0, 0, 0);
    d = __builtin_amdgcn_mfma_f32_16x16x32_bf16(a[1], b[0], d, 0, 0, 0);
    d = __builtin_amdgcn_mfma_f32_16x16x32_bf16(a[0], b[1], d, 0, 0, 0);
    d = __builtin_amdgcn_mfma_f32_16x16x32_bf16(a[0], b[0], d, 0, 0, 0);
}

template <class P>
__device__ __forceinline__ void split8(const float (&v)[8], typename P::vec (&p)[P::NP]) {
#pragma unroll
    for (int i = 0; i < 8; ++i) {
        typename P::piece q[P::NP];
        P::split(v[i], q);
#pragma unroll
        for (int k = 0; k < P::NP; ++k) p[k][i] = q[k];
    }
}

struct WgBf16x6 {
    typedef __bf16 piece;
    typedef bf16x8 vec;
    static constexpr int NP = 3;
    static constexpr float BSCALE = 1.0f, XSCALE = 1.0f;
    static constexpr bool LOADS_BETWEEN_TILES = false;
    __device__ __forceinline__ static void split(float a, piece (&p)[NP]) { split3(a, p[0], p[1], p[2]); }
    __device__ __forceinline__ static unsigned short bits(piece v) { return bf_bits(v); }
    __device__ __forceinline__ static void mac(f32x4& d, const vec (&a)[NP], const vec (&b)[NP]) { mac6(d, a, b); }
    template <int NT_>
    __device__ __forceinline__ void split_a(int, const float (&raw)[8], vec (&ap)[NP], f32x4 (&)[NT_], int) {
        split8<WgBf16x6>(raw, ap);
    }
    __device__ __forceinline__ float row_unscale(int, int, int) const { return 1.0f; }
};

struct WgF16x3 {
    typedef _Float16 piece;
    typedef f16x8 vec;
    static constexpr int NP = 2;
    static constexpr float BSCALE = 1024.0f;
    static constexpr float XSCALE = 16.0f;
    static constexpr bool LOADS_BETWEEN_TILES = true;
    __device__ __forceinline__ static void split(float a, piece (&p)[NP]) {
        p[0] = (_Float16)a;
        p[1] = (_Float16)(a - (float)p[0]);
    }
    __device__ __forceinline__ static unsigned short bits(piece v) { return h_bits(v); }
    __device__ __forceinline__ static void mac(f32x4& d, const vec (&a)[NP], const vec (&b)[NP]) {
        d = __builtin_amdgcn_mfma_f32_16x16x32_f16(a[1], b[0], d, 0, 0, 0);
        d = __builtin_amdgcn_mfma_f32_16x16x32_f16(a[0], b[1], d, 0, 0, 0);
        d = __builtin_amdgcn_mfma_f32_16x16x32_f16(a[0], b[0], d, 0, 0, 0);
    }
    unsigned exr4 = 0xe4e4e4e4u;
    __device__ __forceinline__ int exr_get(int mi) const { return (int)((exr4 >> (8 * mi)) & 255u) - 128; }
    __device__ __forceinline__ void exr_set(int mi, int v) {
        exr4 = (exr4 & ~(255u << (8 * mi))) | ((unsigned)(v + 128) << (8 * mi));
    }
    __device__ __forceinline__ static float row_max4(float m) {
        const unsigned u = __builtin_bit_cast(unsigned, m);
        const auto s16 = __builtin_amdgcn_permlane16_swap(u, u, false, false);
        m = fmaxf(__builtin_bit_cast(float, (unsigned)s16[0]), __builtin_bit_cast(float, (unsigned)s16[1]));
        const unsigned v2 = __builtin_bit_cast(unsigned, m);
        const auto s32 = __builtin_amdgcn_permlane32_swap(v2, v2, false, false);
        return fmaxf(__builtin_bit_cast(float, (unsigned)s32[0]), __builtin_bit_cast(float, (unsigned)s32[1]));
    }
    template <int NT_>
    __device__ __forceinline__ void split_a(int mi, const float (&raw)[8], vec (&ap)[NP], f32x4 (&acc)[NT_], int kq) {
        float mx = 0.f;
#pragma unroll
        for (int e = 0; e < 8; ++e) mx = fmaxf(mx, fabsf(raw[e]));
        mx = row_max4(mx);
        const int eo = exr_get(mi);
        const int ne = mx > 0.f ? min(min(14 - __builtin_amdgcn_frexp_expf(mx), 100), eo) : eo;
        const int delta = eo - ne;
        if (__builtin_amdgcn_ballot_w64(delta != 0)) {
#pragma unroll
            for (int r = 0; r < 4; ++r) {
                const int dr = __builtin_amdgcn_ds_bpermute((4 * kq + r) * 4, delta);
                const float f = __builtin_amdgcn_ldexpf(1.0f, -dr);
#pragma unroll
                for (int ni = 0; ni < NT_; ++ni) acc[ni][r] *= f;
            }
            exr_set(mi, ne);
        }
        float sc[8];
#pragma unroll
        for (int e = 0; e < 8; ++e) sc[e] = __builtin_amdgcn_ldexpf(raw[e], ne);
        split8<WgF16x3>(sc, ap);
    }
    __device__ __forceinline__ float row_unscale(int mi, int r, int kq) const {
        const int er = __builtin_amdgcn_ds_bpermute((4 * kq + r) * 4, exr_get(mi));
        return __builtin_amdgcn_ldexpf(1.0f / BSCALE, -er);
    }
};

template <int H, class P>
struct WGS {
    static constexpr int NW = H / 16, NT = H * 4;
    static constexpr int NT_ = H / 16 + 1, NC = H + 16;
    static constexpr int KP = KS6 + 8;
    static constexpr int BPL = NC * KP, YPL = H * KP, DPL = 16 * KP;
    static constexpr int BUF = P::NP * BPL + 3 * (YPL + DPL);
    static constexpr size_t LDS = 2 * BUF * sizeof(unsigned short);
    static constexpr int XV = 16 * KS6 / NT;
    static constexpr int DV = (8 * KS6 + NT - 1) / NT;
};

#ifdef UAV_X6_PROFILE
__device__ unsigned long long g_wx6_prof[2][8];
#define WX_PROF_DECL unsigned long long pm_[8] = {0, 0, 0, 0, 0, 0, 0, 0}, pl_ = __builtin_readcyclecounter()
#define WX_PROF_MARK(i) do { const unsigned long long n_ = __builtin_readcyclecounter(); pm_[i] += n_ - pl_; pl_ = n_; } while (0)
#define WX_PROF_DEP(v) asm volatile("" ::"v"(v))
#define WX_PROF_FLUSH() do { if (blockIdx.x == 0 && lane == 0 && (w == 0 || w == H / 16 - 1)) \
        for (int i_ = 0; i_ < 8; ++i_) g_wx6_prof[w ? 1 : 0][i_] = pm_[i_]; } while (0)
extern "C" int uav_wx6_prof_read(unsigned long long* out) {
    return hipMemcpyFromSymbol(out, HIP_SYMBOL(g_wx6_prof), sizeof(g_wx6_prof)) == hipSuccess ? 0 : 1;
}
#else
#define WX_PROF_DECL
#define WX_PROF_MARK(i)
#define WX_PROF_DEP(v)
#define WX_PROF_FLUSH()
#endif

template <int H, bool HEADS, class P>
__device__ __forceinline__ void lstm_wgrad_split(
    const float* __restrict__ dgates, const float* __restrict__ y, const float* __restrict__ keep,
    const float* __restrict__ h0, const float* __restrict__ x, int I, const float* __restrict__ dheads, int NH,
    int N, int T, int rows_per_block, float* __restrict__ slabs) {
    using G = WGS<H, P>;
    using vec = typename P::vec;
    constexpr int NT_ = G::NT_, KP = G::KP, BPL = G::BPL, YPL = G::YPL, DPL = G::DPL, BUF = G::BUF, NT = G::NT;
    constexpr int XV = G::XV, DV = G::DV, NW = G::NW, NP = P::NP;
    extern __shared__ __attribute__((aligned(16))) unsigned short sm16[];
    const int tid = threadIdx.x, lane = tid & 63;
    const int w = __builtin_amdgcn_readfirstlane(tid >> 6);
    const bool late = w >= NW / 2;
    const int j = lane & 15, kq = lane >> 4;
    const int r_begin = blockIdx.x * rows_per_block;
    const int nslab = rows_per_block / KS6;
    P pol;

    const int c = tid % H;
    const int rg = __builtin_amdgcn_readfirstlane(tid / H);

    f32x4 acc[4][NT_];
    f32x4 acch = {0.f, 0.f, 0.f, 0.f};
#pragma unroll
    for (int mi = 0; mi < 4; ++mi)
#pragma unroll
        for (int ni = 0; ni < NT_; ++ni) acc[mi][ni] = f32x4{0.f, 0.f, 0.f, 0.f};

    for (int idx = tid; idx < 2 * 3 * DPL; idx += NT) {
        const int b = idx / (3 * DPL), rem = idx % (3 * DPL);
        sm16[b * BUF + NP * BPL + 3 * YPL + rem] = 0;
    }

    float raw[4][8];
    auto load_a_one = [&](int slab, int pair, int e) {
        slab = slab < nslab ? slab : nslab - 1;
        const unsigned off = (unsigned)(r_begin + slab * KS6 + 8 * kq) * (4 * H) + 64 * w + 32 * pair + 2 * j;
        const float2 t2 = *reinterpret_cast<const float2*>(dgates + (off + (unsigned)e * (4 * H)));
        raw[2 * pair][e] = t2.x;
        raw[2 * pair + 1][e] = t2.y;
    };
    auto load_a = [&](int slab, int pair) {
#pragma unroll
        for (int e = 0; e < 8; ++e) load_a_one(slab, pair, e);
    };
    constexpr int NV = HEADS ? 9 : 8;
    float v[NV], hz = 0.f, xv[XV], dv[DV];
    float kv = 1.f;
    int i_start = -1;
    auto load_b_y = [&](int slab, int i) {
        slab = slab < nslab ? slab : nslab - 1;
        const int rr = r_begin + slab * KS6 + 8 * rg - 1 + i;
        v[i] = y[(unsigned)(rr < 0 ? 0 : rr) * H + c];
    };
    auto load_b_rest = [&](int slab) {
        slab = slab < nslab ? slab : nslab - 1;
        const int q0 = r_begin + slab * KS6 + 8 * rg;
        const int tq = q0 % T;
        i_start = (tq == 0) ? 0 : (tq + 7 >= T ? T - tq : -1);
        if (i_start >= 0) hz = h0[(unsigned)((q0 + i_start) / T) * H + c];
        kv = keep ? keep[q0 + (lane & 7)] : 1.f;
#pragma unroll
        for (int k = 0; k < XV; ++k) {
            const int idx = tid + k * NT, q = idx >> 4, f = idx & 15;
            const unsigned r = (unsigned)(r_begin + slab * KS6 + q);
            xv[k] = (f < I) ? x[r * I + f] : (f == 6 ? 1.f : 0.f);
        }
#pragma unroll
        for (int k = 0; k < DV; ++k) {
            const int idx = tid + k * NT, q = idx >> 3, a = idx & 7;
            const unsigned r = (unsigned)(r_begin + slab * KS6 + (q < KS6 ? q : 0));
            dv[k] = (HEADS && a < NH && q < KS6) ? dheads[r * NH + a] : 0.f;
        }
    };
    auto load_b = [&](int slab) {
#pragma unroll
        for (int i = 0; i < NV; ++i) load_b_y(slab, i);
        load_b_rest(slab);
    };
    auto commit_b = [&](int buf) {
        unsigned short* bp = sm16 + buf * BUF;
        unsigned short* yp = bp + NP * BPL;
        unsigned short* dp = yp + 3 * YPL;
        float hp[8], yy[8];
#pragma unroll
        for (int i = 0; i < 8; ++i) {
            const float kpi = __builtin_bit_cast(float, __builtin_amdgcn_readlane(__builtin_bit_cast(int, kv), i));
            hp[i] = ((i == i_start) ? hz : v[i]) * (kpi * P::BSCALE);
            yy[i] = HEADS ? v[i + 1 < NV ? i + 1 : 0] : 0.f;
        }
        vec hq[NP];
        split8<P>(hp, hq);
#pragma unroll
        for (int p = 0; p < NP; ++p) *reinterpret_cast<vec*>(bp + p * BPL + c * KP + 8 * rg) = hq[p];
        if (HEADS) {
            bf16x8 yq[3];
            split8<WgBf16x6>(yy, yq);
#pragma unroll
            for (int p = 0; p < 3; ++p) *reinterpret_cast<bf16x8*>(yp + p * YPL + c * KP + 8 * rg) = yq[p];
        }
#pragma unroll
        for (int k = 0; k < XV; ++k) {
            const int idx = tid + k * NT, q = idx >> 4, f = idx & 15;
            typename P::piece xq[NP];
            P::split(xv[k] * P::XSCALE, xq);
            unsigned short* d = bp + (H + f) * KP + q;
#pragma unroll
            for (int p = 0; p < NP; ++p) d[p * BPL] = P::bits(xq[p]);
        }
        if (HEADS) {
#pragma unroll
            for (int k = 0; k < DV; ++k) {
                const int idx = tid + k * NT, q = idx >> 3, a = idx & 7;
                if (q < KS6) {
                    __bf16 pa, pb, pc;
                    split3(dv[k], pa, pb, pc);
                    unsigned short* d = dp + a * KP + q;
                    d[0] = bf_bits(pa);
                    d[DPL] = bf_bits(pb);
                    d[2 * DPL] = bf_bits(pc);
                }
            }
        }
    };
    vec ap[2][NP];
    auto split_pair = [&](int sl, int pair) {
#pragma unroll
        for (int m = 0; m < 2; ++m) pol.split_a(2 * pair + m, raw[2 * pair + m], ap[m], acc[2 * pair + m], kq);
        if constexpr (!P::LOADS_BETWEEN_TILES) load_a(sl + 1, pair);
    };
    auto mfma_pair = [&](int buf, int pair, int sl) {
        const unsigned short* bp = sm16 + buf * BUF;
#pragma unroll
        for (int ni = 0; ni < NT_; ++ni) {
            vec bb[NP];
            const unsigned short* src = bp + (16 * ni + j) * KP + 8 * kq;
#pragma unroll
            for (int p = 0; p < NP; ++p) bb[p] = *reinterpret_cast<const vec*>(src + p * BPL);
            P::mac(acc[2 * pair][ni], ap[0], bb);
            P::mac(acc[2 * pair + 1][ni], ap[1], bb);
            if constexpr (P::LOADS_BETWEEN_TILES) {
#pragma unroll
                for (int e = ni; e < 8; e += NT_) load_a_one(sl + 1, pair, e);
                if (pair == 1) {
#pragma unroll
                    for (int i = ni; i < NV; i += NT_) load_b_y(sl + 2, i);
                    if (ni == NT_ - 1) load_b_rest(sl + 2);
                }
                asm volatile("" ::: "memory");
            } else if (HEADS && (ni & 1)) {
                asm volatile("" ::: "memory");
            }
        }
        if (HEADS && pair == 1) {
            const unsigned short* yp = bp + NP * BPL;
            const unsigned short* dp = yp + 3 * YPL;
            bf16x8 da[3], yb[3];
            const unsigned short* sa = dp + j * KP + 8 * kq;
            const unsigned short* sb = yp + (16 * w + j) * KP + 8 * kq;
#pragma unroll
            for (int pc = 0; pc < 3; ++pc) {
                da[pc] = *reinterpret_cast<const bf16x8*>(sa + pc * DPL);
                yb[pc] = *reinterpret_cast<const bf16x8*>(sb + pc * YPL);
            }
            mac6(acch, da, yb);
        }
    };

    load_b(0);
    load_a(0, 0);
    load_a(0, 1);
    commit_b(0);
    load_b(1);
    split_pair(0, 0);
    lds_barrier();
    WX_PROF_DECL;
    for (int sl = 0; sl < nslab; ++sl) {
        const int buf = sl & 1;
        WX_PROF_MARK(0);
        mfma_pair(buf, 0, sl);
        WX_PROF_DEP(acc[0][NT_ - 1]); WX_PROF_DEP(acc[1][NT_ - 1]); WX_PROF_MARK(2);
        commit_b(buf ^ 1);
        if constexpr (!P::LOADS_BETWEEN_TILES) load_b(sl + 2);
        WX_PROF_MARK(5);
        split_pair(sl, 1);
        WX_PROF_DEP(ap[0][0]); WX_PROF_DEP(ap[1][NP - 1]); WX_PROF_MARK(3);
        mfma_pair(buf, 1, sl);
        WX_PROF_DEP(acc[2][NT_ - 1]); WX_PROF_DEP(acc[3][NT_ - 1]); WX_PROF_MARK(4);
        if (!late) { lds_barrier(); WX_PROF_MARK(7); }
        split_pair(sl + 1, 0);
        WX_PROF_DEP(ap[0][0]); WX_PROF_DEP(ap[1][NP - 1]); WX_PROF_MARK(1);
        if (late) { lds_barrier(); WX_PROF_MARK(7); }
    }
    WX_PROF_FLUSH();
    float* slab = slabs + (size_t)blockIdx.x * WG<H>::SLAB;
#pragma unroll
    for (int mi = 0; mi < 4; ++mi)
#pragma unroll
        for (int r = 0; r < 4; ++r) {
            const float usc = pol.row_unscale(mi, r, kq);
#pragma unroll
            for (int ni = 0; ni < NT_; ++ni)
                slab[(size_t)(64 * w + 32 * (mi >> 1) + 2 * (4 * kq + r) + (mi & 1)) * G::NC + 16 * ni + j] =
                    acc[mi][ni][r] * (ni == NT_ - 1 ? usc * (P::BSCALE / P::XSCALE) : usc);
        }
#pragma unroll
    for (int r = 0; r < 4; ++r) slab[(size_t)4 * H * G::NC + (size_t)(4 * kq + r) * H + 16 * w + j] = acch[r];
}

template <int H, bool HEADS>
__global__ __launch_bounds__(H * 4) void lstm_wgrad_x6_kernel(
    const float* __restrict__ dgates, const float* __restrict__ y, const float* __restrict__ keep,
    const float* __restrict__ h0, const float* __restrict__ x, int I, const float* __restrict__ dheads, int NH,
    int N, int T, int rows_per_block, float* __restrict__ slabs) {
    lstm_wgrad_split<H, HEADS, WgBf16x6>(dgates, y, keep, h0, x, I, dheads, NH, N, T, rows_per_block, slabs);
}
template <int H, bool HEADS>
__global__ __launch_bounds__(H * 4) void lstm_wgrad_h3_kernel(
    const float* __restrict__ dgates, const float* __restrict__ y, const float* __restrict__ keep,
    const float* __restrict__ h0, const float* __restrict__ x, int I, const float* __restrict__ dheads, int NH,
    int N, int T, int rows_per_block, float* __restrict__ slabs) {
    lstm_wgrad_split<H, HEADS, WgF16x3>(dgates, y, keep, h0, x, I, dheads, NH, N, T, rows_per_block, slabs);
}

template <int H>
__global__ __launch_bounds__(256) void wgrad_reduce_kernel(const float* __restrict__ slabs, int nb, int I, int NH,
                                                           float* __restrict__ dw_ih, float* __restrict__ dw_hh,
                                                           float* __restrict__ db, float* __restrict__ db_hh,
                                                           float* __restrict__ dw_head) {
    using G = WG<H>;
    const size_t o = (size_t)blockIdx.x * 256 + threadIdx.x;
    if (o >= G::SLAB) return;
    float p8[8] = {0.f, 0.f, 0.f, 0.f, 0.f, 0.f, 0.f, 0.f};
    int b = 0;
    for (; b + 8 <= nb; b += 8)
#pragma unroll
        for (int k = 0; k < 8; ++k) p8[k] += slabs[(size_t)(b + k) * G::SLAB + o];
    for (; b < nb; ++b) p8[0] += slabs[(size_t)b * G::SLAB + o];
    const float s = ((p8[0] + p8[1]) + (p8[2] + p8[3])) + ((p8[4] + p8[5]) + (p8[6] + p8[7]));
    const size_t gsz = (size_t)4 * H * G::NC;
    if (o < gsz) {
        const int m = (int)(o / G::NC), c = (int)(o % G::NC);
        if (c < H) dw_hh[(size_t)m * H + c] = s;
        else if (c - H < I) dw_ih[(size_t)m * I + (c - H)] = s;
        else if (c - H == 6) {
            db[m] = s;
            if (db_hh) db_hh[m] = s;
        }
    } else if (dw_head) {
        const int a = (int)((o - gsz) / H), uu = (int)((o - gsz) % H);
        if (a < NH) dw_head[(size_t)a * H + uu] = s;
    }
}

template <class P, int H, bool HEADS>
static constexpr auto wgrad_split_kernel() {
    if constexpr (std::is_same<P, WgF16x3>::value) return &lstm_wgrad_h3_kernel<H, HEADS>;
    else return &lstm_wgrad_x6_kernel<H, HEADS>;
}

template <class P, int H>
static int launch_wgrad_split(const float* dgates, const float* y, const float* keep, const float* h0, const float* x, int I,
                              const float* dheads, int NH, int N, int T, int nb, int rpb, float* slabs, hipStream_t st) {
    const auto kern = dheads ? wgrad_split_kernel<P, H, true>() : wgrad_split_kernel<P, H, false>();
    const size_t lds = WGS<H, P>::LDS;
    UAV_CHECK_HIP(uav_dyn_lds(reinterpret_cast<const void*>(kern), (int)lds));
    hipLaunchKernelGGL(kern, dim3(nb), dim3(H * 4), lds, st, dgates, y, keep, h0, x, I, dheads, NH, N, T, rpb, slabs);
    return 0;
}

template <int H>
static int launch_wgrad(uav_ctx* ctx, const float* dgates, const float* y, const float* keep, const float* h0,
                        const float* x, int I, const float* dheads, int NH, int N, int T,
                        float* dw_ih, float* dw_hh, float* db, float* db_hh, float* dw_head, hipStream_t st) {
    using G = WG<H>;
    const int64_t NTr = (int64_t)N * T;
    int nb = ctx->num_cu;
    const int64_t max_nb = (int64_t)(ctx->ws_bytes / (G::SLAB * sizeof(float)));
    if (nb > max_nb) nb = (int)max_nb;
    UAV_REQUIRE(nb >= 1, "uav_lstm_wgrad: workspace too small for one slab");
    int64_t rpb = (NTr + nb - 1) / nb;
    rpb = (rpb + KC - 1) / KC * KC;
    nb = (int)((NTr + rpb - 1) / rpb);
    float* slabs = (float*)ctx->ws;
    {
        int64_t rpx = (NTr + nb - 1) / nb;
        rpx = (rpx + KS6 - 1) / KS6 * KS6;
        const int nbx = (int)((NTr + rpx - 1) / rpx);
        const bool split_ok = (NTr % rpx == 0) && T >= 8 && I <= 6 && (!dheads || NH <= 8) && NTr * 4 * H < (1ll << 30) &&
                              !uav_want_f32_mfma();
        if (split_ok) {
            const int rc = uav_want_bf16x6()
                               ? launch_wgrad_split<WgBf16x6, H>(dgates, y, keep, h0, x, I, dheads, NH, N, T, nbx, (int)rpx, slabs, st)
                               : launch_wgrad_split<WgF16x3, H>(dgates, y, keep, h0, x, I, dheads, NH, N, T, nbx, (int)rpx, slabs, st);
            if (rc) return rc;
            hipLaunchKernelGGL((wgrad_reduce_kernel<H>), dim3((unsigned)((G::SLAB + 255) / 256)), dim3(256), 0, st, slabs,
                               nbx, I, NH, dw_ih, dw_hh, db, db_hh, dw_head);
            UAV_LAUNCH_CHECK();
            return 0;
        }
    }
    UAV_CHECK_HIP(uav_dyn_lds(reinterpret_cast<const void*>(&lstm_wgrad_kernel<H>), (int)G::LDS));
    hipLaunchKernelGGL((lstm_wgrad_kernel<H>), dim3(nb), dim3(H * 4), G::LDS, st, dgates, y, keep, h0, x, I, dheads, NH, N,
                       T, rpb, slabs);
    hipLaunchKernelGGL((wgrad_reduce_kernel<H>), dim3((unsigned)((G::SLAB + 255) / 256)), dim3(256), 0, st, slabs, nb, I,
                       NH, dw_ih, dw_hh, db, db_hh, dw_head);
    UAV_LAUNCH_CHECK();
    return 0;
}

int lstm_wgrad_fused(uav_ctx* ctx, const float* dgates, const float* y, const float* keep, const float* h0,
                     const float* x, int I, const float* dheads, int NH, int N, int T, int H,
                     float* dw_ih, float* dw_hh, float* db, float* db_hh, float* dw_head, hipStream_t st) {
    switch (H) {
        case 64: return launch_wgrad<64>(ctx, dgates, y, keep, h0, x, I, dheads, NH, N, T, dw_ih, dw_hh, db, db_hh, dw_head, st);
        case 128: return launch_wgrad<128>(ctx, dgates, y, keep, h0, x, I, dheads, NH, N, T, dw_ih, dw_hh, db, db_hh, dw_head, st);
    }
    uav_set_error("lstm_wgrad_fused: H=%d unsupported", H);
    return 2;
}
```

### uav-wrf-les-ppo-lstm_amd/uavppo/_lib.py

```python
from __future__ import annotations

import ctypes as C
import os

import torch

_HERE = os.path.dirname(os.path.abspath(__file__))
LIB_PATH = os.environ.get("UAVPPO_LIB") or os.path.join(_HERE, "libuavppo.so")

c_f32p = C.c_void_p
P, I32, I64, U64, F32, F64, SZ = C.c_void_p, C.c_int, C.c_int64, C.c_uint64, C.c_float, C.c_double, C.c_size_t


class EnvCfg(C.Structure):
    _fields_ = [("variant", C.c_int32), ("field_mode", C.c_int32), ("n_fields", C.c_int32),
                ("bonus_is_f64", C.c_int32), ("env_offset", C.c_int32), ("n_env_total", C.c_int32),
                ("trend_k", C.c_int32), ("pad_", C.c_int32),
                ("radius", C.c_double), ("bonus", C.c_double),
                ("seed", C.c_uint64), ("bank", C.c_void_p), ("bank_src", C.c_void_p), ("curriculum", C.c_void_p)]


class StopRule(C.Structure):
    _fields_ = [("window", C.c_int32), ("pos_std_max", C.c_float), ("conc_coef", C.c_float), ("conc_peak", C.c_float),
                ("conc_min", C.c_float)]


class StepperCall(C.Structure):
    _fields_ = [("state", C.c_void_p), ("x", C.c_void_p), ("below", C.c_void_p), ("keep_t", C.c_void_p), ("t", C.c_int), ("I", C.c_int),
                ("y", C.c_void_p), ("stash", C.c_void_p), ("hn", C.c_void_p), ("cn", C.c_void_p)]


class LstmBwdLayer(C.Structure):
    _fields_ = [(n, C.c_void_p) for n in ("keep", "stash", "w_hh", "w_ih", "dgates", "dx", "dhn", "dcn", "dh0", "dc0")]


class GatherSpec(C.Structure):
    _fields_ = [("src", C.c_void_p), ("dst", C.c_void_p), ("row_bytes", C.c_int64), ("planes", C.c_int32), ("pad_", C.c_int32),
                ("src_plane_stride_bytes", C.c_int64), ("dst_plane_stride_bytes", C.c_int64)]


GATHER_MAX_SPECS = 12


SIGNATURES = {
    "uav_abi_version": (I32, []),
    "uav_last_error": (C.c_char_p, []),
    "uav_create": (I32, [C.POINTER(C.c_void_p), I32, SZ]),
    "uav_destroy": (None, [P]),
    "uav_set_lstm_arith": (I32, [P, I32]),
    "uav_get_lstm_arith": (I32, [P]),
    "uav_set_debug_flags": (I32, [P, C.c_uint]),
    "uav_absmax": (I32, [P, P, I64, P, P]),
    "uav_gae": (I32, [P, P, P, P, P, I32, I32, F32, F32, I32, P, P]),
    "uav_adv_stats": (I32, [P, P, I64, P, P]),
    "uav_adv_normalise": (I32, [P, P, P, I64, P, P, P, P]),
    "uav_adv_normalise_inline": (I32, [P, P, P, I64, P, P, P, P]),
    "uav_pack_success_bits": (I32, [P, P, I64, I32, P, P]),
    "uav_episode_rows": (I32, [P, P, P, P, I32, I32, I32, P, P, I32, P, P]),
    "uav_curriculum_state_bytes": (SZ, []),
    "uav_curriculum_init": (I32, [P, P, C.c_double, C.c_double, I32, P]),
    "uav_curriculum_update": (I32, [P, P, P, I32, I32, P]),
    "uav_ppo_loss": (I32, [P, P, P, P, P, P, P, P, I64, I32, F32, F32, F32, P, P, P, P, P]),
    "uav_ppo_loss_from_y": (I32, [P, P, P, P, P, P, P, P, P, I64, I32, I32, F32, F32, F32, P, P, P, P]),
    "uav_policy_sample": (I32, [P, P, I64, I32, P, U64, U64, I64, P, P, P, P, P, P]),
    "uav_policy_sample_at": (I32, [P, P, I64, I64, I32, U64, U64, I64, P, P, I32, I32, P, P, P, P, P]),
    "uav_store_transition": (I32, [P, I32, I32, I32, P, P, P, P, P, P, P, P, P]),
    "uav_rollout_tail": (I32, [P, P, I32, P, P, I64, I32, P, P, I32, P, I64, I32, I32, U64, U64, I64, P, P, P, P, P, P, P, P, P, P, P, P, P, P, P]),
    "uav_clip_adam": (I32, [P, P, P, P, P, I64, I64, F32, F32, F32, F32, F32, P, P, P]),
    "uav_clip_adamw": (I32, [P, P, P, P, P, I64, I64, F32, F32, F32, F32, F32, F32, P, P]),
    "uav_smooth_l1": (I32, [P, P, P, I64, F32, P, P, P]),
    "uav_mse_bce": (I32, [P, P, P, I64, P, P, P]),
    "uav_disc_param_count": (SZ, [I32, I32, I32]),
    "uav_disc_grad": (I32, [P, P, P, P, I64, P, P, I64, I32, I32, I32, F32, F32, P, P, P]),
    "uav_disc_reward": (I32, [P, P, P, P, I64, I32, I32, I32, F32, F32, P, P, P]),
    "uav_lstm_stepper_bytes": (SZ, [I32, I32, I32]),
    "uav_lstm_stepper_begin": (I32, [P, P, P, P, P, P, P, P, I32, I32, I32, P]),
    "uav_lstm_stepper_step": (I32, [P, P, P, P, P, I32, I32, I32, I32, I32, P, P, P, P, P]),
    "uav_lstm_stepper_step_pair": (I32, [P, P, P, I32, I32, I32, P]),
    "uav_gemm_f32": (I32, [P, I64, I64, I64, P, I64, I64, P, I64, I64, P, I64, P, I32, P]),
    "uav_gemm_f16x3": (I32, [P, I64, I64, I64, P, I64, I64, P, I64, I64, P, I64, P, I32, P, P]),
    "uav_colsum": (I32, [P, P, I64, I32, P, P]),
    "uav_ln_relu": (I32, [P, P, P, P, P, P, I64, I32, P]),
    "uav_ln_relu_bwd": (I32, [P, P, P, P, P, P, I64, I32, P, P, P]),
    "uav_mlp_param_count": (I64, [I32, I32, I32, I32]),
    "uav_mlp_stash_floats": (I64, [I32, I32]),
    "uav_mlp_fwd": (I32, [P, P, P, I64, I32, I32, I32, I32, P, P, P]),
    "uav_mlp_bwd": (I32, [P, P, P, P, P, I64, I32, I32, I32, I32, P, P]),
    "uav_mlp_ppo_grad": (I32, [P, P, P, P, P, P, P, P, I64, I32, I32, I32, I32, F32, F32, F32, P, P, P]),
    "uav_mlp_ppo_grad_trend": (I32, [P, P, P, P, P, P, P, P, I64, I32, F32, F32, F32, P, P, P]),
    "uav_mlp_ppo_grad_rows": (I32, [P, P, P, P, P, P, P, P, I64, P, I64, I32, F32, F32, F32, P, P, P]),
    "uav_gather_rows_multi": (I32, [P, P, I64, I64, C.POINTER(GatherSpec), I32, P]),
    "uav_lstm_fwd": (I32, [P, P, P, P, P, P, P, P, P, I32, I32, I32, I32, P, P, P, P, P, P, I32, P, P]),
    "uav_lstm_bwd": (I32, [P, P, P, P, P, P, P, I32, P, P, I32, I32, I32, P, P, P, P, I32, P, P]),
    "uav_lstm_bwd_caps": (I32, [P, I32, I32]),
    "uav_lstm_dgates_bytes": (SZ, [P, I32, I32, I32]),
    "uav_lstm_dgates_f32": (I32, [P, P, I32, I32, I32, P, P]),
    "uav_lstm_bwd_stack": (I32, [P, I32, P, P, P, P, I32, I32, I32, I32, P]),
    "uav_lstm_wgrad": (I32, [P, P, P, P, P, P, P, P, P, I32, I32, I32, I32, I32, P, P, P, P, P, P, P]),
    "uav_lstm_chunk_states": (I32, [P, P, P, P, P, P, I32, I32, I32, I32, P, P, P]),
    "uav_env_state_bytes": (SZ, [I32]),
    "uav_env_reset": (I32, [P, P, I32, C.POINTER(EnvCfg), P, P]),
    "uav_env_step": (I32, [P, P, I32, C.POINTER(EnvCfg), P, P, P, P, P, P, P, P, P, P]),
    "uav_env_peek": (I32, [P, P, I32, P, P, P, P, P]),
    "uav_env_materialise": (I32, [P, P, I32, C.POINTER(EnvCfg), I32, P, P]),
    "uav_rollout": (I32, [P, P, I32, C.POINTER(EnvCfg), I32, P, I32, I32, U64, P, P, P, P, P, P, P, P, P, P,
                          P, P, P, P, P, P, P, P, P, P]),
    "uav_greedy_episodes": (I32, [P, P, I32, C.POINTER(EnvCfg), I32, P, I32, I32, P, P, P, P, P, P, P, P, P, P, P]),
    "uav_greedy_episodes_stop": (I32, [P, P, I32, C.POINTER(EnvCfg), I32, P, I32, I32, P, P, P, P, P, P, P, P, P, P,
                                       C.POINTER(StopRule), P, P, P, P]),
    "uav_greedy_tail": (I32, [P, P, I32, C.POINTER(EnvCfg), P, I64, I32, P, P, I32, I32, I32, P, P, P, P, P, P, P, P,
                              C.POINTER(StopRule), P, P, P, P]),
    "uav_stop_stability": (I32, [P, I32, C.POINTER(StopRule), P, P, I64, P, P, P, P, P, P]),
    "uav_peak_stop_param_count": (SZ, [I32]),
    "uav_peak_stop_scan": (I32, [P, P, I32, I32, P, I64, I64, I32, I32, P, P, P, F32, P, P, P, P]),
    "uav_threshold_windows": (I32, [P, P, I64, I64, I32, I32, P, P, P, I32, I32, I32, F64, F64, F64, P, P]),
    "uav_threshold_rule": (I32, [P, P, I64, I64, I32, I32, P, P, P, I32, I32, I32, F64, F64, P, P, P, P, P, P]),
    "uav_rccl_version": (I32, [C.POINTER(C.c_int)]),
    "uav_comm_unique_id": (I32, [P]),
    "uav_comm_init": (I32, [P, P, I32, I32]),
    "uav_comm_world": (I32, [P]),
    "uav_comm_rank": (I32, [P]),
    "uav_comm_destroy": (I32, [P]),
    "uav_allreduce": (I32, [P, P, I64, P]),
    "uav_allreduce_f64": (I32, [P, P, I64, P]),
    "uav_allgather_bytes": (I32, [P, P, P, I64, P]),
}

_lib = None


def lib():
    global _lib
    if _lib is None:
        if not os.path.exists(LIB_PATH):
            raise RuntimeError(
                f"{LIB_PATH} not found: build it with `make -C uav-wrf-les-ppo-lstm_amd/csrc` "
                "(or python -c 'import __graft_entry__ as g; g.build()'). There is no CPU fallback.")
        _lib = C.CDLL(LIB_PATH)
        for name, (res, args) in SIGNATURES.items():
            fn = getattr(_lib, name)
            fn.restype = res
            fn.argtypes = args
    return _lib


def check(rc, what):
    if rc != 0:
        raise RuntimeError(f"{what} failed ({rc}): {lib().uav_last_error().decode()}")
```

### uav-wrf-les-ppo-lstm_amd/uavppo/ops.py

```python
from __future__ import annotations

import ctypes as C

import torch

from . import _lib
from ._lib import EnvCfg, check, lib

GAE_MODES = {"reference_exact": 0, "standard": 1, "inline_v10": 2}
WS_BYTES = 256 << 20


class Context:
    _per_device: dict = {}

    def __init__(self, device_index):
        if not torch.cuda.is_available():
            raise RuntimeError("uavppo needs an MI355X (gfx950) GPU: torch.cuda.is_available() is False "
                               "and there is no CPU fallback")
        h = C.c_void_p()
        check(lib().uav_create(C.byref(h), int(device_index), WS_BYTES), "uav_create")
        self.handle = h
        self.device = device_index
        self.initial_arith = {0: "fp16x3", 1: "bf16x6", 2: "f32_mfma"}[int(lib().uav_get_lstm_arith(h))]
# ... 124 lines not shown

def curriculum_state(device, radius=50.0, bonus=0.6, bonus_is_f64=False):
    st = torch.zeros(int(lib().uav_curriculum_state_bytes()), dtype=U8, device=device)
    curriculum_init(st, radius, bonus, bonus_is_f64)
    return st


def curriculum_init(state, radius, bonus, bonus_is_f64=False):
    check(lib().uav_curriculum_init(_h(state), _p(state, U8, name="curriculum state"), float(radius), float(bonus), int(bool(bonus_is_f64)),
                                    _stream()), "uav_curriculum_init")


def curriculum_update(state, msgs, cap):
    world = int(msgs.shape[0])
    check(lib().uav_curriculum_update(_h(state), _p(state, U8, name="curriculum state"), _p(msgs, U8, (world, 4 + cap + 1), "msgs"), world,
                                      int(cap), _stream()), "uav_curriculum_update")


def curriculum_read(state_host):
    import numpy as np
    b = np.asarray(state_host, dtype=np.uint8)
    d = b[:32].view(np.float64)
    q = b[32:48].view(np.int64)
    i = b[48:56].view(np.int32)
    return {"radius": float(d[0]), "bonus": float(d[1]), "bonus_is_f64": bool(d[2] != 0.0), "overflow": bool(d[3] != 0.0),
            "episodes": int(q[0]), "successes": int(q[1]), "hist_len": int(i[0]), "win_succ": int(i[1])}


def ppo_loss(logits, value, act, logp_old, adv, ret, val_old, inv_n, clip, ent_beta,
             loss_sums=None, dlogits=None, dvalue=None, dhead_bias=None):
    n, A = logits.shape
    loss_sums = torch.empty(4, dtype=F64, device=logits.device) if loss_sums is None else loss_sums
    dlogits = torch.empty_like(logits) if dlogits is None else dlogits
    dvalue = torch.empty(n, dtype=F32, device=logits.device) if dvalue is None else dvalue
    check(lib().uav_ppo_loss(_h(logits), _p(logits, F32, (n, A), "logits"), _p(value.reshape(-1), F32, (n,), "value"),
                             _p(act, I32, (n,), "act"), _p(logp_old, F32, (n,), "logp_old"),
                             _p(adv, F32, (n,), "adv"), _p(ret, F32, (n,), "ret"), _p(val_old, F32, (n,), "val_old"),
                             n, A, float(inv_n), float(clip), float(ent_beta), _p(loss_sums, F64, (4,), "loss_sums"),
                             _p(dlogits, F32, (n, A), "dlogits"), _p(dvalue, F32, (n,), "dvalue"),
                             _p(dhead_bias, F32, (A + 1,), "dhead_bias"), _stream()),
          "uav_ppo_loss")
    return loss_sums, dlogits, dvalue


def policy_sample(logits, u=None, seed=0, counter=0, forced_act=None, want_probs=False, nan_count=None, index_offset=0,
                  iteration=0):
    n, A = logits.shape
    dev = logits.device
    act = torch.empty(n, dtype=I32, device=dev)
    logp = torch.empty(n, dtype=F32, device=dev)
    probs = torch.empty(n, A, dtype=F32, device=dev) if want_probs else None
    nan_count = torch.zeros(1, dtype=I32, device=dev) if nan_count is None else nan_count
    check(lib().uav_policy_sample(_h(logits), _p(logits, F32, (n, A), "logits"), n, A, _p(u, F32, (n,), "u"),
                                  int(seed), (int(iteration) << 32) | (int(counter) & 0xffffffff), int(index_offset),
                                  _p(forced_act, I32, (n,), "forced_act"),
                                  _p(act), _p(logp), _p(probs), _p(nan_count, I32, (1,), "nan_count"), _stream()),
          "uav_policy_sample")
    return act, logp, probs, nan_count


def policy_sample_at(heads_seq, t, act_out, act_buf, val_buf, logp_buf, nan_count, seed=0, iteration=0, index_offset=0,
                     forced_act=None):
    N, T, A1 = heads_seq.shape
    check(lib().uav_policy_sample_at(_h(heads_seq), C.c_void_p(_p(heads_seq, F32, (N, T, A1), "heads_seq").value + 4 * int(t) * A1),
                                     T * A1, N, A1 - 1, int(seed), (int(iteration) << 32) | (int(t) & 0xffffffff),
                                     int(index_offset), _p(forced_act, I32, (N,), "forced_act"), _p(act_out, I32, (N,), "act_out"),
                                     T, int(t), _p(act_buf, I32, (N, T), "act_buf"), _p(val_buf, F32, (N, T), "val_buf"),
                                     _p(logp_buf, F32, (N, T), "logp_buf"), _p(nan_count, I32, (1,), "nan_count"), _stream()),
          "uav_policy_sample_at")
    return act_out


def store_transition(t, keep, rew, done, flags, keep_buf, rew_buf, done_buf, flags_buf):
    N, T = keep_buf.shape
    check(lib().uav_store_transition(_h(keep), N, T, int(t), _p(keep, F32, (N,), "keep"), _p(rew, F32, (N,), "rew"),
                                     _p(done, F32, (N,), "done"), _p(flags, U8, (N,), "flags"), _p(keep_buf, F32, (N, T), "keep_buf"),
                                     _p(rew_buf, F32, (N, T), "rew_buf"), _p(done_buf, F32, (N, T), "done_buf"),
                                     _p(flags_buf, U8, (N, T), "flags_buf"), _stream()), "uav_store_transition")


def rollout_tail(env_state, cfg, y_seq, t, w_head, b_head, heads_seq, act_out, cur_obs, obs_seq, keep, act_buf, val_buf, logp_buf,
                 keep_buf, rew_buf, done_buf, flags_buf, nan_count, seed=0, iteration=0, index_offset=0, forced_act=None, noise=None):
    N, T, H = y_seq.shape
    A1 = heads_seq.shape[-1]
    od = cur_obs.shape[-1]
    check(lib().uav_rollout_tail(_h(y_seq), _p(env_state, U8, name="env state"), N, C.byref(cfg),
                                 C.c_void_p(_p(y_seq, F32, (N, T, H), "y_seq").value + 4 * int(t) * H), T * H, H,
                                 _p(w_head, F32, (A1, H), "w_head"), _p(b_head, F32, (A1,), "b_head"), A1 - 1,
                                 C.c_void_p(_p(heads_seq, F32, (N, T, A1), "heads_seq").value + 4 * int(t) * A1), T * A1, T, int(t),
                                 int(seed), (int(iteration) << 32) | (int(t) & 0xffffffff), int(index_offset),
                                 _p(forced_act, I32, (N,), "forced_act"), _p(noise, F64, (N, 2), "noise"),
                                 _p(act_out, I32, (N,), "act_out"), _p(cur_obs, F32, (N, od), "cur_obs"),
                                 _p(obs_seq, F32, (N, T, od), "obs_seq"), _p(keep, F32, (N,), "keep"),
                                 _p(act_buf, I32, (N, T), "act_buf"), _p(val_buf, F32, (N, T), "val_buf"),
                                 _p(logp_buf, F32, (N, T), "logp_buf"), _p(keep_buf, F32, (N, T), "keep_buf"),
                                 _p(rew_buf, F32, (N, T), "rew_buf"), _p(done_buf, F32, (N, T), "done_buf"),
                                 _p(flags_buf, U8, (N, T), "flags_buf"), _p(nan_count, I32, (1,), "nan_count"), _stream()),
          "uav_rollout_tail")
    return act_out


def ppo_loss_heads(heads, act, logp_old, adv, ret, val_old, inv_n, clip, ent_beta, loss_sums, dheads, dhead_bias=None):
    n, A1 = heads.shape
    check(lib().uav_ppo_loss(_h(heads), _p(heads, F32, (n, A1), "heads"), None, _p(act, I32, (n,), "act"),
                             _p(logp_old, F32, (n,), "logp_old"), _p(adv, F32, (n,), "adv"), _p(ret, F32, (n,), "ret"),
                             _p(val_old, F32, (n,), "val_old"), n, A1 - 1, float(inv_n), float(clip), float(ent_beta),
                             _p(loss_sums, F64, (4,), "loss_sums"), _p(dheads, F32, (n, A1), "dheads"), None,
                             _p(dhead_bias, F32, (A1,), "dhead_bias"), _stream()), "uav_ppo_loss")
    return loss_sums, dheads


def ppo_loss_from_y(y, w_head, b_head, act, logp_old, adv, ret, val_old, inv_n, clip, ent_beta, loss_sums, dheads,
                    dhead_bias=None):
    n, H = y.shape
    A1 = w_head.shape[0]
    _t = KERNEL_TIMER.bracket("ppo_loss")
    check(lib().uav_ppo_loss_from_y(_h(y), _p(y, F32, (n, H), "y"), _p(w_head, F32, (A1, H), "w_head"),
                                    _p(b_head, F32, (A1,), "b_head"), _p(act, I32, (n,), "act"),
                                    _p(logp_old, F32, (n,), "logp_old"), _p(adv, F32, (n,), "adv"),
                                    _p(ret, F32, (n,), "ret"), _p(val_old, F32, (n,), "val_old"), n, H, A1 - 1,
                                    float(inv_n), float(clip), float(ent_beta), _p(loss_sums, F64, (4,), "loss_sums"),
                                    _p(dheads, F32, (n, A1), "dheads"), _p(dhead_bias, F32, (A1,), "dhead_bias"),
                                    _stream()), "uav_ppo_loss_from_y")
    if _t is not None:
        _t.record()
    return loss_sums, dheads


ARITH = {"fp16x3": 0, "bf16x6": 1, "f32_mfma": 2}


def set_lstm_arith(mode, device=None):
    check(lib().uav_set_lstm_arith(Context.get(device).handle, ARITH[mode]), "uav_set_lstm_arith")


class lstm_arith:

    def __init__(self, mode, device=None):
        self.mode, self.device = mode, device

    def __enter__(self):
        self.prev = get_lstm_arith(self.device)
        set_lstm_arith(self.mode, self.device)

    def __exit__(self, *exc):
        set_lstm_arith(self.prev, self.device)


DEBUG_FLAGS = {"step_f32": 1, "x_f32": 2, "dg_f32": 4, "gemm_tn_off": 0x10}


def set_debug_flags(*names, device=None):
    check(lib().uav_set_debug_flags(Context.get(device).handle, sum(DEBUG_FLAGS[n] for n in names)), "uav_set_debug_flags")


def rccl_version():
    out = C.c_int(0)
    check(lib().uav_rccl_version(C.byref(out)), "uav_rccl_version")
    return int(out.value)


def comm_unique_id():
    buf = C.create_string_buffer(128)
    check(lib().uav_comm_unique_id(buf), "uav_comm_unique_id")
    return bytes(buf.raw)


def comm_init(uid, rank, world, device=None):
    if len(uid) != 128:
        raise RuntimeError("comm_init: the unique id is 128 bytes")
    check(lib().uav_comm_init(Context.get(device).handle, C.c_char_p(uid), int(rank), int(world)), "uav_comm_init")


def comm_world(device=None):
    return int(lib().uav_comm_world(Context.get(device).handle))


def comm_destroy(device=None):
    check(lib().uav_comm_destroy(Context.get(device).handle), "uav_comm_destroy")


def comm_allreduce(t):
    if t.dtype == torch.float32:
        check(lib().uav_allreduce(_h(t), _p(t, F32, name="t"), t.numel(), _stream()), "uav_allreduce")
    elif t.dtype == torch.float64:
        check(lib().uav_allreduce_f64(_h(t), _p(t, torch.float64, name="t"), t.numel(), _stream()), "uav_allreduce_f64")
    else:
        raise RuntimeError(f"comm_allreduce: f32 or f64, got {t.dtype}")
    return t


def comm_allgather_bytes(msg):
    w = comm_world(msg.device)
    if w < 1:
        raise RuntimeError("comm_allgather_bytes: no communicator on this device's handle")
    out = torch.empty(w, msg.numel(), dtype=torch.uint8, device=msg.device)
    check(lib().uav_allgather_bytes(_h(msg), _p(msg, torch.uint8, name="msg"), _p(out, torch.uint8, name="out"), msg.numel(), _stream()),
          "uav_allgather_bytes")
    return out


def get_lstm_arith(device=None):
    m = int(lib().uav_get_lstm_arith(Context.get(device).handle))
    return {v: k for k, v in ARITH.items()}[m]


def absmax(x, out=None):
    out = torch.empty(1, dtype=F32, device=x.device) if out is None else out
    check(lib().uav_absmax(_h(x), _p(x, F32, name="x"), x.numel(), _p(out, F32, (1,), "out"), _stream()), "uav_absmax")
    return out


def clip_adam(param, grad, exp_avg, exp_avg_sq, step, lr, beta1=0.9, beta2=0.999, eps=1e-8, max_norm=0.5,
              gnorm_out=None, pmax_out=None):
    n = param.numel()
    for t, nm in ((grad, "grad"), (exp_avg, "exp_avg"), (exp_avg_sq, "exp_avg_sq")):
        if t.numel() != n:
            raise RuntimeError(f"clip_adam: {nm} has {t.numel()} elements, param has {n}")
    check(lib().uav_clip_adam(_h(param), _p(param, F32, name="param"), _p(grad, F32, name="grad"),
                              _p(exp_avg, F32, name="exp_avg"), _p(exp_avg_sq, F32, name="exp_avg_sq"), n, int(step),
                              float(lr), float(beta1), float(beta2), float(eps), float(max_norm),
                              _p(gnorm_out, F32, (1,), "gnorm_out"), _p(pmax_out, F32, (1,), "pmax_out"), _stream()),
          "uav_clip_adam")


def gemm_rows(a, b_t, bias, out):
    N, K = a.shape
    M = b_t.shape[0]
    if a.stride(1) != 1 or out.stride(1) != 1 or tuple(out.shape) != (N, M) or b_t.shape[1] != K:
        raise RuntimeError("gemm_rows: a [N, K] and out [N, M] need unit stride along the last index; b_t is [M, K]")
    for t, nm in ((a, "a"), (out, "out")):
        if not t.is_cuda or t.dtype != F32:
            raise RuntimeError(f"gemm_rows: {nm}: expected a float32 GPU tensor")
    check(lib().uav_gemm_f32(_h(a), N, M, K, C.c_void_p(a.data_ptr()), a.stride(0), 1, _p(b_t, F32, name="b_t"), 1, K,
                             C.c_void_p(out.data_ptr()), out.stride(0), _p(bias, F32, (M,), "bias"), 0, _stream()),
          "uav_gemm_f32")
    return out


def gemm(a, b, trans_a=False, trans_b=False, bias=None, out=None, accumulate=False, split_fp16=False, a_absmax=None):
    if a.dim() != 2 or b.dim() != 2:
        raise RuntimeError("gemm: 2-D tensors expected")
    M, K = (a.shape[1], a.shape[0]) if trans_a else a.shape
    K2, N = (b.shape[1], b.shape[0]) if trans_b else b.shape
    if K != K2:
        raise RuntimeError(f"gemm: inner dimensions differ ({K} vs {K2})")
    sa_m, sa_k = (1, a.shape[1]) if trans_a else (a.shape[1], 1)
    sb_k, sb_n = (1, b.shape[1]) if trans_b else (b.shape[1], 1)
    if out is None:
        if accumulate:
            raise RuntimeError("gemm: accumulate needs out")
        out = torch.empty(M, N, dtype=F32, device=a.device)
    if split_fp16:
        check(lib().uav_gemm_f16x3(_h(a), M, N, K, _p(a, F32, name="a"), sa_m, sa_k, _p(b, F32, name="b"), sb_k, sb_n,
                                   _p(out, F32, (M, N), "out"), N, _p(bias, F32, (N,), "bias"), int(accumulate),
                                   _p(a_absmax, F32, (1,), "a_absmax"), _stream()), "uav_gemm_f16x3")
        return out
    check(lib().uav_gemm_f32(_h(a), M, N, K, _p(a, F32, name="a"), sa_m, sa_k, _p(b, F32, name="b"), sb_k, sb_n,
                             _p(out, F32, (M, N), "out"), N, _p(bias, F32, (N,), "bias"), int(accumulate), _stream()),
          "uav_gemm_f32")
    return out


def mlp_param_count(in_dim=6, h1=256, h2=128, n_act=5):
    return int(lib().uav_mlp_param_count(in_dim, h1, h2, n_act))


def mlp_fwd(params, x, in_dim=6, h1=256, h2=128, n_act=5, stash=None):
    B = x.shape[0]
    if params.numel() != mlp_param_count(in_dim, h1, h2, n_act):
        raise RuntimeError("mlp_fwd: flat parameter buffer has the wrong size")
    heads = torch.empty(B, n_act + 1, dtype=F32, device=x.device)
    per = int(lib().uav_mlp_stash_floats(h1, h2))
    if stash is None:
        stash = torch.empty(B * per, dtype=F32, device=x.device)
    elif stash.numel() < B * per:
        raise RuntimeError("mlp_fwd: stash too small")
    check(lib().uav_mlp_fwd(_h(x), _p(params, F32, name="params"), _p(x, F32, (B, in_dim), "x"), B, in_dim, h1, h2,
                            n_act, _p(heads), _p(stash, F32, name="stash"), _stream()), "uav_mlp_fwd")
    return heads, stash


def mlp_bwd(params, x, stash, dheads, in_dim=6, h1=256, h2=128, n_act=5, grad=None):
    B = x.shape[0]
    grad = torch.empty_like(params) if grad is None else grad
    check(lib().uav_mlp_bwd(_h(x), _p(params, F32, name="params"), _p(x, F32, (B, in_dim), "x"),
                            _p(stash, F32, name="stash"), _p(dheads, F32, (B, n_act + 1), "dheads"), B, in_dim, h1,
                            h2, n_act, _p(grad, F32, params.shape, "grad"), _stream()), "uav_mlp_bwd")
    return grad


def mlp_ppo_grad(params, obs, act, logp_old, adv, ret, val_old, inv_n, clip, ent_beta, loss_sums, grad, in_dim=6, h1=256,
                 h2=128, n_act=5):
    n = obs.shape[0]
    _t = KERNEL_TIMER.bracket("mlp_ppo_grad")
    check(lib().uav_mlp_ppo_grad(_h(obs), _p(params, F32, (mlp_param_count(in_dim, h1, h2, n_act),), "params"),
                                 _p(obs, F32, (n, in_dim), "obs"), _p(act, I32, (n,), "act"),
                                 _p(logp_old, F32, (n,), "logp_old"), _p(adv, F32, (n,), "adv"), _p(ret, F32, (n,), "ret"),
                                 _p(val_old, F32, (n,), "val_old"), n, in_dim, h1, h2, n_act, float(inv_n), float(clip),
                                 float(ent_beta), _p(loss_sums, F64, (4,), "loss_sums"), _p(grad, F32, params.shape, "grad"),
                                 _stream()), "uav_mlp_ppo_grad")
    if _t is not None:
        _t.record()
    return grad


# ... 97 lines not shown
    cfg.variant = ENV_VARIANTS[variant]
    cfg.field_mode = 1 if bank is not None else 0
    cfg.n_fields = 0 if bank is None else int(bank.shape[0])
    cfg.bonus_is_f64 = int(isinstance(bonus, np.float64))
    cfg.env_offset = int(env_offset)
    cfg.n_env_total = int(n_env_total)
    cfg.trend_k = int(trend_k)
    cfg.radius = float(radius)
    cfg.bonus = float(bonus)
    cfg.seed = int(seed)
    cfg.curriculum = None if curriculum is None else _p(curriculum, U8, name="curriculum state").value
    if bank is not None:
        F_ = bank.shape[0]
        cfg.bank = _p(bank, F64, (F_, 500, 500, 2), "bank").value
        cfg.bank_src = _p(bank_src, F64, (F_, 2), "bank_src").value
    return cfg


def env_reset(state, n_env, cfg, obs_out):
    check(lib().uav_env_reset(_h(state), _p(state, U8, name="env state"), n_env, C.byref(cfg),
                              _p(obs_out, F32, (n_env, 6 + cfg.trend_k), "obs_out"), _stream()), "uav_env_reset")


def env_step(state, n_env, cfg, act, obs_out, rew, done, flags, noise=None, info=None, term_obs=None, rew64=None):
    check(lib().uav_env_step(_h(state), _p(state, U8, name="env state"), n_env, C.byref(cfg),
                             _p(act, I32, (n_env,), "act"), _p(noise, F64, (n_env, 2), "noise"),
                             _p(obs_out, F32, (n_env, 6 + cfg.trend_k), "obs_out"), _p(rew, F32, (n_env,), "rew"),
                             _p(done, F32, (n_env,), "done"), _p(flags, U8, (n_env,), "flags"),
                             _p(info, F32, (n_env, 5), "info"), _p(term_obs, F32, (n_env, 6 + cfg.trend_k), "term_obs"),
                             _p(rew64, F64, (n_env,), "rew64"), _stream()), "uav_env_step")


def env_peek(state, n_env, pos=None, source=None, steps=None, episode=None):
    check(lib().uav_env_peek(_h(state), _p(state, U8, name="env state"), n_env, _p(pos, F32, (n_env, 2), "pos"),
                             _p(source, F64, (n_env, 2), "source"), _p(steps, I32, (n_env,), "steps"),
                             _p(episode, I32, (n_env,), "episode"), _stream()), "uav_env_peek")


def lstm_fwd(x, keep, h0, c0, w_ih, w_hh, b_ih, b_hh, stash=None, want_stash=True, y=None, w_head=None, b_head=None,
             heads=None):
    N, T, I = x.shape
    H = w_hh.shape[1]
    dev = x.device
    y = torch.empty(N, T, H, dtype=F32, device=dev) if y is None else y
    hn = torch.empty(N, H, dtype=F32, device=dev)
    cn = torch.empty(N, H, dtype=F32, device=dev)
    if stash is None and (want_stash or I > 8 or H not in (64, 128)):
        stash = torch.empty(N, T, 6 * H, dtype=F32, device=dev)
    _t = KERNEL_TIMER.bracket("lstm_fwd")
    check(lib().uav_lstm_fwd(_h(x), _p(x, F32, (N, T, I), "x"), _p(keep, F32, (N, T), "keep"),
                             _p(h0, F32, (N, H), "h0"), _p(c0, F32, (N, H), "c0"), _p(w_ih, F32, (4 * H, I), "w_ih"),
                             _p(w_hh, F32, (4 * H, H), "w_hh"), _p(b_ih, F32, (4 * H,), "b_ih"),
                             _p(b_hh, F32, (4 * H,), "b_hh"), N, T, I, H, _p(y, F32, (N, T, H), "y"), _p(hn), _p(cn),
                             _p(stash, F32, (N, T, 6 * H), "stash"),
                             _p(w_head, F32, None if w_head is None else (w_head.shape[0], H), "w_head"),
                             _p(b_head, F32, None if w_head is None else (w_head.shape[0],), "b_head"),
                             0 if w_head is None else int(w_head.shape[0]),
                             _p(heads, F32, None if w_head is None else (N, T, w_head.shape[0]), "heads"), _stream()),
          "uav_lstm_fwd")
    if _t is not None:
        _t.record()
    return y, hn, cn, stash


def lstm_chunk_states(y, stash, keep, h0, c0, chunk, h_out=None, c_out=None):
    N, T, H = y.shape
    chunk = int(chunk)
    rows = N * (T // chunk) if chunk >= 1 else 0
    h_out = torch.empty(rows, H, dtype=F32, device=y.device) if h_out is None else h_out
    c_out = torch.empty(rows, H, dtype=F32, device=y.device) if c_out is None else c_out
    check(lib().uav_lstm_chunk_states(_h(y), _p(y, F32, (N, T, H), "y"), _p(stash, F32, (N, T, 6 * H), "stash"),
                                      _p(keep, F32, (N, T), "keep"), _p(h0, F32, (N, H), "h0"), _p(c0, F32, (N, H), "c0"),
                                      N, T, H, chunk, _p(h_out, F32, (rows, H), "h_out"), _p(c_out, F32, (rows, H), "c_out"),
                                      _stream()), "uav_lstm_chunk_states")
    return h_out, c_out


class LstmStepper:

    def __init__(self, N, I, H, device):
        nbytes = lib().uav_lstm_stepper_bytes(int(N), int(I), int(H))
        if nbytes == 0:
            raise RuntimeError(f"uav_lstm_stepper: N={N} I={I} H={H} not supported (H = 256, I <= 256)")
        self.N, self.I, self.H = int(N), int(I), int(H)
        self.state = torch.empty(nbytes, dtype=torch.uint8, device=device)
        self.hn = torch.empty(N, H, dtype=F32, device=device)
        self.cn = torch.empty(N, H, dtype=F32, device=device)

    def begin(self, w_ih, w_hh, b_ih, b_hh, h0, c0):
        N, I, H = self.N, self.I, self.H
        check(lib().uav_lstm_stepper_begin(_h(self.state), _p(self.state), _p(w_ih, F32, (4 * H, I), "w_ih"),
                                           _p(w_hh, F32, (4 * H, H), "w_hh"), _p(b_ih, F32, (4 * H,), "b_ih"),
                                           _p(b_hh, F32, (4 * H,), "b_hh"), _p(h0, F32, (N, H), "h0"), _p(c0, F32, (N, H), "c0"),
                                           N, I, H, _stream()), "uav_lstm_stepper_begin")

    def step(self, x, t, y, stash, below=None, keep=None):
        N, I, H = self.N, self.I, self.H
        T = x.shape[1]
        check(lib().uav_lstm_stepper_step(_h(self.state), _p(self.state), _p(x, F32, (N, T, I), "x"),
                                          None if below is None else _p(below.state), _p(keep, F32, (N,), "keep"), N, T, int(t),
                                          I, H, _p(y, F32, (N, T, H), "y"), _p(stash, F32, (N, T, 6 * H), "stash"), _p(self.hn),
                                          _p(self.cn), _stream()), "uav_lstm_stepper_step")


def _stepper_call(sp, x, t, y, stash, below, keep):
    N, I, H = sp.N, sp.I, sp.H
    T = x.shape[1]
    c = _lib.StepperCall()
    c.state = _p(sp.state).value
    c.x = _p(x, F32, (N, T, I), "x").value
    c.below = None if below is None else _p(below.state).value
    c.keep_t = None if keep is None else _p(keep, F32, (N,), "keep").value
    c.t, c.I = int(t), I
    c.y = _p(y, F32, (N, T, H), "y").value
    c.stash = _p(stash, F32, (N, T, 6 * H), "stash").value
    c.hn, c.cn = _p(sp.hn).value, _p(sp.cn).value
    return c


def lstm_stepper_step_pair(a, b):
    ca, cb = _stepper_call(*a), _stepper_call(*b)
    sp, x = a[0], a[1]
    check(lib().uav_lstm_stepper_step_pair(_h(sp.state), C.byref(ca), C.byref(cb), sp.N, x.shape[1], sp.H, _stream()),
          "uav_lstm_stepper_step_pair")


def lstm_dgates_bytes(N, T, H, device):
    n = int(lib().uav_lstm_dgates_bytes(Context.get(torch.device(device)).handle, int(N), int(T), int(H)))
    if n <= 0:
        raise RuntimeError(f"uav_lstm_dgates_bytes({N}, {T}, {H}) = {n}")
    return n


def lstm_dgates(N, T, H, device):
    nbytes = lstm_dgates_bytes(N, T, H, device)
    if nbytes == N * T * 4 * H * 4:
        return torch.empty(N, T, 4 * H, dtype=F32, device=device)
    return torch.empty((nbytes + 3) // 4, dtype=F32, device=device)


def _pdg(dgates, N, T, H):
    need = lstm_dgates_bytes(N, T, H, dgates.device)
    if dgates.numel() * 4 < need:
        raise RuntimeError(f"dgates: {dgates.numel() * 4} bytes, uav_lstm_dgates_bytes({N}, {T}, {H}) = {need} (allocate with ops.lstm_dgates)")
    return _p(dgates, F32, None, "dgates")


def lstm_dgates_f32(dgates, N, T, H):
    out = torch.empty(N, T, 4 * H, dtype=F32, device=dgates.device)
    check(lib().uav_lstm_dgates_f32(_h(dgates), _pdg(dgates, N, T, H), N, T, H, _p(out), _stream()), "uav_lstm_dgates_f32")
    return out


def lstm_wgrad(x, keep, h0, y, stash, dgates, w_ih, dheads=None):
    N, T, I = x.shape
    H = y.shape[-1]
    dev = x.device
    nh = 0 if dheads is None else dheads.shape[-1]
    dw_ih = torch.empty(4 * H, I, dtype=F32, device=dev)
    dw_hh = torch.empty(4 * H, H, dtype=F32, device=dev)
    db = torch.empty(4 * H, dtype=F32, device=dev)
    dw_head = torch.empty(nh, H, dtype=F32, device=dev) if nh else None
    check(lib().uav_lstm_wgrad(_h(x), _p(x, F32, (N, T, I), "x"), _p(keep, F32, (N, T), "keep"), _p(h0, F32, (N, H), "h0"),
                               _p(y, F32, (N, T, H), "y"), _p(stash, F32, (N, T, 6 * H), "stash"),
                               _pdg(dgates, N, T, H), _p(w_ih, F32, (4 * H, I), "w_ih"),
                               _p(dheads, F32, (N, T, nh), "dheads"), nh, N, T, I, H,
                               _p(dw_ih, F32, (4 * H, I), "dw_ih"), _p(dw_hh, F32, (4 * H, H), "dw_hh"),
                               _p(db, F32, (4 * H,), "db"), None, _p(dw_head, F32, (nh, H), "dw_head"), _p(None), _stream()),
          "uav_lstm_wgrad")
    return {"dw_ih": dw_ih, "dw_hh": dw_hh, "db": db, "dw_head": dw_head}


def lstm_bwd_caps(device, I, H):
    return int(lib().uav_lstm_bwd_caps(Context.get(torch.device(device)).handle, int(I), int(H)))


def lstm_bwd_stack(layers, keep, dy=None, dheads=None, w_head=None):
    N, T, H6 = layers[0]["stash"].shape
    H = H6 // 6
    arr = (_lib.LstmBwdLayer * len(layers))()
    for a, d in zip(arr, layers):
        a.keep = None if keep is None else _p(keep, F32, (N, T), "keep").value
        a.stash = _p(d["stash"], F32, (N, T, 6 * H), "stash").value
        a.w_hh = _p(d["w_hh"], F32, (4 * H, H), "w_hh").value
        a.w_ih = None if d.get("w_ih") is None else _p(d["w_ih"], F32, (4 * H, H), "w_ih").value
        a.dgates = _pdg(d["dgates"], N, T, H).value
        a.dx = None if d.get("dx") is None else _p(d["dx"], F32, (N, T, H), "dx").value
        a.dhn = a.dcn = a.dh0 = a.dc0 = None
    nh = 0 if dheads is None else dheads.shape[-1]
    _t = KERNEL_TIMER.bracket("lstm_bwd")
    check(lib().uav_lstm_bwd_stack(_h(layers[0]["stash"]), len(layers), C.byref(arr), _p(dy, F32, (N, T, H), "dy"),
                                   _p(dheads, F32, (N, T, nh), "dheads"), _p(w_head, F32, (nh, H), "w_head"), nh, N, T, H, _stream()),
          "uav_lstm_bwd_stack")
    if _t is not None:
        _t.record()


def lstm_bwd(x, keep, stash, w_ih, w_hh, y, h0, dy=None, dheads=None, w_head=None, dhn=None, dcn=None, need_dx=False,
             dgates=None, dw_ih=None, dw_hh=None, db=None, dw_head=None, want_dstate=True, wgrad_dheads=None, bwd_done=False,
             db_hh=None):
    N, T, I = x.shape
    H = w_hh.shape[1]
    dev = x.device
    dgates = lstm_dgates(N, T, H, dev) if dgates is None else dgates
    dx = torch.empty(N, T, I, dtype=F32, device=dev) if (need_dx and not bwd_done) else None
    dw_ih = torch.empty(4 * H, I, dtype=F32, device=dev) if dw_ih is None else dw_ih
    dw_hh = torch.empty(4 * H, H, dtype=F32, device=dev) if dw_hh is None else dw_hh
    db = torch.empty(4 * H, dtype=F32, device=dev) if db is None else db
    dh0 = torch.empty(N, H, dtype=F32, device=dev) if want_dstate else None
    dc0 = torch.empty(N, H, dtype=F32, device=dev) if want_dstate else None
    nh = 0 if dheads is None else dheads.shape[-1]
    if wgrad_dheads is None:
        wgrad_dheads = dheads
    nhw = 0 if wgrad_dheads is None else wgrad_dheads.shape[-1]
    if wgrad_dheads is not None and dw_head is None:
        dw_head = torch.empty(nhw, H, dtype=F32, device=dev)
    dx_in_bwd = bool(need_dx and lstm_bwd_caps(x.device, I, H) & 1) or bwd_done
    _t = None if bwd_done else KERNEL_TIMER.bracket("lstm_bwd")
    if not bwd_done:
        check(lib().uav_lstm_bwd(_h(x), _p(keep, F32, (N, T), "keep"), _p(stash, F32, (N, T, 6 * H), "stash"),
                                 _p(w_hh, F32, (4 * H, H), "w_hh"), _p(dy, F32, (N, T, H), "dy"),
                                 _p(dheads, F32, (N, T, nh), "dheads"), _p(w_head, F32, (nh, H), "w_head"), nh,
                                 _p(dhn, F32, (N, H), "dhn"), _p(dcn, F32, (N, H), "dcn"), N, T, H,
                                 _pdg(dgates, N, T, H), _p(dh0), _p(dc0),
                                 _p(w_ih, F32, (4 * H, I), "w_ih") if dx_in_bwd else None, I, _p(dx) if dx_in_bwd else None,
                                 _stream()), "uav_lstm_bwd")
    if _t is not None:
        _t.record()
    _t = KERNEL_TIMER.bracket("lstm_wgrad")
    check(lib().uav_lstm_wgrad(_h(x), _p(x, F32, (N, T, I), "x"), _p(keep, F32, (N, T), "keep"), _p(h0, F32, (N, H), "h0"),
                               _p(y, F32, (N, T, H), "y"), _p(stash, F32, (N, T, 6 * H), "stash"),
                               _pdg(dgates, N, T, H), _p(w_ih, F32, (4 * H, I), "w_ih"),
                               _p(wgrad_dheads, F32, (N, T, nhw), "dheads"), nhw, N, T, I, H,
                               _p(dw_ih, F32, (4 * H, I), "dw_ih"), _p(dw_hh, F32, (4 * H, H), "dw_hh"),
                               _p(db, F32, (4 * H,), "db"), _p(db_hh, F32, (4 * H,), "db_hh"), _p(dw_head, F32, (nhw, H), "dw_head"),
                               None if dx_in_bwd else _p(dx), _stream()),
          "uav_lstm_wgrad")
    if _t is not None:
        _t.record()
    return {"dx": dx, "dw_ih": dw_ih, "dw_hh": dw_hh, "db": db, "dh0": dh0, "dc0": dc0, "dgates": dgates,
            "dw_head": dw_head}


def env_materialise(state, n_env, cfg, env_index, out=None):
    out = torch.empty(500, 500, 2, dtype=F64, device=state.device) if out is None else out
    check(lib().uav_env_materialise(_h(state), _p(state, U8, name="env state"), n_env, C.byref(cfg), int(env_index),
                                    _p(out, F64, (500, 500, 2), "field_out"), _stream()), "uav_env_materialise")
    return out


def ln_relu(z, gamma, beta, want_stats=False):
    rows, cols = z.shape
    a = torch.empty_like(z)
    rstd = torch.empty(rows, dtype=F32, device=z.device)
    check(lib().uav_ln_relu(_h(z), _p(z, F32, (rows, cols), "z"), _p(a, F32), _p(rstd, F32), _p(gamma, F32, (cols,), "gamma"),
                            _p(beta, F32, (cols,), "beta"), rows, cols, _stream()), "uav_ln_relu")
    return (a, rstd) if want_stats else a


def ln_relu_bwd(d, xhat, rstd, gamma, beta, dgamma=None, dbeta=None):
    rows, cols = d.shape
    dg = torch.empty(cols, dtype=F32, device=d.device) if dgamma is None else dgamma
    db = torch.empty(cols, dtype=F32, device=d.device) if dbeta is None else dbeta
    check(lib().uav_ln_relu_bwd(_h(d), _p(d, F32, (rows, cols), "d"), _p(xhat, F32, (rows, cols), "xhat"),
                                _p(rstd, F32, (rows,), "rstd"), _p(gamma, F32, (cols,), "gamma"), _p(beta, F32, (cols,), "beta"),
                                rows, cols, _p(dg, F32, (cols,), "dgamma"), _p(db, F32, (cols,), "dbeta"), _stream()),
          "uav_ln_relu_bwd")
    return d, dg, db


def smooth_l1(pred, target, beta):
    n = pred.numel()
    loss = torch.zeros(1, dtype=F64, device=pred.device)
    dpred = torch.empty(n, dtype=F32, device=pred.device)
    check(lib().uav_smooth_l1(_h(pred), _p(pred, F32, (n,), "pred"), _p(target, F32, (n,), "target"), n, float(beta),
                              _p(loss, F64), _p(dpred, F32), _stream()), "uav_smooth_l1")
    return loss, dpred


def mse_bce(out, target):
    n = out.shape[0]
    loss = torch.zeros(1, dtype=F64, device=out.device)
    dout = torch.empty(n, 2, dtype=F32, device=out.device)
    check(lib().uav_mse_bce(_h(out), _p(out, F32, (n, 2), "out"), _p(target, F32, (n, 2), "target"), n, _p(loss, F64),
                            _p(dout, F32), _stream()), "uav_mse_bce")
    return loss, dout


def clip_adamw(param, grad, exp_avg, exp_avg_sq, step, lr, beta1=0.9, beta2=0.999, eps=1e-8, weight_decay=0.01, max_norm=1.0,
               gnorm_out=None):
    n = param.numel()
    check(lib().uav_clip_adamw(_h(param), _p(param, F32, (n,), "param"), _p(grad, F32, (n,), "grad"),
                               _p(exp_avg, F32, (n,), "exp_avg"), _p(exp_avg_sq, F32, (n,), "exp_avg_sq"), n, int(step),
                               float(lr), float(beta1), float(beta2), float(eps), float(weight_decay), float(max_norm),
                               _p(gnorm_out, F32, (1,), "gnorm_out"), _stream()), "uav_clip_adamw")


def colsum(x, out=None):
    rows, cols = x.shape
    out = torch.empty(cols, dtype=F32, device=x.device) if out is None else out
    check(lib().uav_colsum(_h(x), _p(x, F32, (rows, cols), "x"), rows, cols, _p(out, F32, (cols,), "out"), _stream()),
          "uav_colsum")
    return out


def rollout_lstm(env_state, n_env, cfg, params, hidden, horizon, it, cur_obs, h, c, bufs, last_val=None,
                 forced_act=None, noise=None, nan_count=None, stash=None, y=None, info=None, heads=None):
    N, T, D = n_env, horizon, 6 + cfg.trend_k
    _t = KERNEL_TIMER.bracket("rollout")
    check(lib().uav_rollout(_h(cur_obs), _p(env_state, U8, name="env state"), N, C.byref(cfg), 1,
                            _p(params, F32, name="params"), int(hidden), T, int(it),
                            _p(cur_obs, F32, (N, D), "cur_obs"), _p(h, F32, (N, hidden), "h"), _p(c, F32, (N, hidden), "c"),
                            _p(bufs["obs"], F32, (N, T, D), "obs"), _p(bufs["act"], I32, (N, T), "act"),
                            _p(bufs["rew"], F32, (N, T), "rew"), _p(bufs["val"], F32, (N, T), "val"),
                            _p(bufs["logp"], F32, (N, T), "logp"), _p(bufs["done"], F32, (N, T), "done"),
                            _p(bufs["flags"], U8, (N, T), "flags"), _p(bufs["keep"], F32, (N, T), "keep"),
                            _p(last_val, F32, (N,), "last_val"), _p(forced_act, I32, (N, T), "forced_act"),
                            _p(noise, F64, (N, T, 2), "noise"), _p(nan_count, I32, (1,), "nan_count"),
                            _p(stash, F32, (N, T, 6 * hidden), "stash"), _p(y, F32, (N, T, hidden), "y"),
                            _p(info, F32, (N, T, 10), "info"), _p(heads, F32, (N, T, 6), "heads"), _stream()),
          "uav_rollout")
    if _t is not None:
        _t.record()


def rollout_mlp(env_state, n_env, cfg, params, horizon, it, cur_obs, bufs, last_val=None, forced_act=None, noise=None,
                nan_count=None, info=None, heads=None, trend=False):
    N, T, D = n_env, horizon, 6 + (cfg.trend_k if trend else 0)
    if trend:
        _mlp_trend_params("rollout_mlp", params, cfg.trend_k)
    _t = KERNEL_TIMER.bracket("rollout")
    check(lib().uav_rollout(_h(cur_obs), _p(env_state, U8, name="env state"), N, C.byref(cfg), 2 if trend else 0,
                            _p(params, F32, name="params"), 0, T, int(it), _p(cur_obs, F32, (N, D), "cur_obs"), None, None,
                            _p(bufs["obs"], F32, (N, T, D), "obs"), _p(bufs["act"], I32, (N, T), "act"),
                            _p(bufs["rew"], F32, (N, T), "rew"), _p(bufs["val"], F32, (N, T), "val"),
                            _p(bufs["logp"], F32, (N, T), "logp"), _p(bufs["done"], F32, (N, T), "done"),
                            _p(bufs["flags"], U8, (N, T), "flags"), None, _p(last_val, F32, (N,), "last_val"),
                            _p(forced_act, I32, (N, T), "forced_act"), _p(noise, F64, (N, T, 2), "noise"),
                            _p(nan_count, I32, (1,), "nan_count"), None, None, _p(info, F32, (N, T, 10), "info"),
                            _p(heads, F32, (N, T, 6), "heads"), _stream()), "uav_rollout")
    if _t is not None:
        _t.record()


def greedy_recs(n_env, steps, obs_dim, device):
    N, k = n_env, steps
    return {"act": torch.empty(N, k, dtype=I32, device=device), "obs": torch.empty(N, k, obs_dim, dtype=F32, device=device),
            "pos": torch.empty(N, k, 2, dtype=F32, device=device), "flags": torch.empty(N, k, dtype=U8, device=device)}


def _greedy(env_state, n_env, cfg, params, hidden, steps, cur_obs, h, c, active, recs, noise, nan_count, rule=None, stop_win=None,
            stop_cnt=None, rule_val=None, trend=False):
    N, T, D = n_env, steps, 6 + cfg.trend_k
# ... 191 lines not shown
```

### uav-wrf-les-ppo-lstm_amd/uavppo/policy.py

```python
from __future__ import annotations

import math

import numpy as np
import torch

from . import ops


class _FlatPolicy:

    def _alloc(self, layout, device):
        self.layout = layout
        total = sum(int(np.prod(s)) for _, s in layout)
        self.flat = torch.zeros(total, dtype=torch.float32, device=device)
        self.grad = torch.zeros_like(self.flat)
        self.views, self.grad_views = {}, {}
        o = 0
        for name, shape in layout:
            n = int(np.prod(shape))
            self.views[name] = self.flat[o:o + n].view(shape)
            self.grad_views[name] = self.grad[o:o + n].view(shape)
            o += n

    @property
    def device(self):
        return self.flat.device

    def num_params(self):
        return self.flat.numel()


def _orthogonal(shape, gain, gen):
    w = torch.empty(shape)
    torch.nn.init.orthogonal_(w, gain=gain, generator=gen)
    return w


class MLPActorCritic(_FlatPolicy):
    KEYS = ("feature.0.weight", "feature.0.bias", "feature.1.weight", "feature.1.bias",
            "feature.3.weight", "feature.3.bias", "feature.4.weight", "feature.4.bias",
            "actor.weight", "actor.bias", "critic.weight", "critic.bias")

    def __init__(self, input_size=6, output_size=5, h1=256, h2=128, device="cuda", seed=None):
        self.in_dim, self.n_act, self.h1, self.h2 = input_size, output_size, h1, h2
        A = output_size
        self._alloc([("feature.0.weight", (h1, input_size)), ("feature.0.bias", (h1,)),
                     ("feature.1.weight", (h1,)), ("feature.1.bias", (h1,)),
                     ("feature.3.weight", (h2, h1)), ("feature.3.bias", (h2,)),
                     ("feature.4.weight", (h2,)), ("feature.4.bias", (h2,)),
                     ("head.weight", (A + 1, h2)), ("head.bias", (A + 1,))], device)
        assert self.flat.numel() == ops.mlp_param_count(input_size, h1, h2, A)
        gen = torch.Generator().manual_seed(seed) if seed is not None else None
        sd = {
            "feature.0.weight": _orthogonal((h1, input_size), math.sqrt(2), gen), "feature.0.bias": torch.zeros(h1),
            "feature.1.weight": torch.ones(h1), "feature.1.bias": torch.zeros(h1),
            "feature.3.weight": _orthogonal((h2, h1), math.sqrt(2), gen), "feature.3.bias": torch.zeros(h2),
            "feature.4.weight": torch.ones(h2), "feature.4.bias": torch.zeros(h2),
            "actor.weight": _orthogonal((A, h2), 0.01, gen), "actor.bias": torch.zeros(A),
            "critic.weight": _orthogonal((1, h2), 1.0, gen), "critic.bias": torch.zeros(1),
        }
        self.load_state_dict(sd)
        self._stash = None

    def _named(self, src):
        A = self.n_act
        out = {k: src[k] for k in self.KEYS[:8]}
        out["actor.weight"], out["critic.weight"] = src["head.weight"][:A], src["head.weight"][A:]
        out["actor.bias"], out["critic.bias"] = src["head.bias"][:A], src["head.bias"][A:]
        return out

    def named_views(self):
        return self._named(self.views)

    def named_grads(self):
        return self._named(self.grad_views)

    def state_dict(self):
        return {k: v.detach().clone() for k, v in self.named_views().items()}

    def load_state_dict(self, sd):
        nv = self.named_views()
        for k in self.KEYS:
            nv[k].copy_(torch.as_tensor(sd[k], dtype=torch.float32).reshape(nv[k].shape))

    def heads(self, x, stash=None):
        heads, self._stash = ops.mlp_fwd(self.flat, x, self.in_dim, self.h1, self.h2, self.n_act, stash=stash)
        self._x = x
        return heads

    def backward(self, dheads):
        ops.mlp_bwd(self.flat, self._x, self._stash, dheads, self.in_dim, self.h1, self.h2, self.n_act, grad=self.grad)
        self._stash = None
        return self.grad


class LSTMActorCritic(_FlatPolicy):
    def __init__(self, obs_dim=6, hidden=128, num_layers=1, n_act=5, device="cuda", seed=0):
        self.obs_dim, self.hidden, self.num_layers, self.n_act = obs_dim, hidden, num_layers, n_act
        H, A = hidden, n_act
        layout = []
        for l in range(num_layers):
            i = obs_dim if l == 0 else H
            layout += [(f"lstm.weight_ih_l{l}", (4 * H, i)), (f"lstm.weight_hh_l{l}", (4 * H, H)),
                       (f"lstm.bias_ih_l{l}", (4 * H,)), (f"lstm.bias_hh_l{l}", (4 * H,))]
        layout += [("head.weight", (A + 1, H)), ("head.bias", (A + 1,))]
        self._alloc(layout, device)
        gen = torch.Generator().manual_seed(seed)
        k = 1.0 / math.sqrt(H)
        for name, shape in layout[:-2]:
            self.views[name].copy_((torch.rand(shape, generator=gen) * 2 - 1) * k)
        self.views["head.weight"][:A].copy_(_orthogonal((A, H), 0.01, gen))
        self.views["head.weight"][A:].copy_(_orthogonal((1, H), 1.0, gen))
        self.views["head.bias"].zero_()
        self._saved = None

    def _named(self, src):
        A = self.n_act
        out = {k: v for k, v in src.items() if k.startswith("lstm.")}
        out["actor.weight"], out["critic.weight"] = src["head.weight"][:A], src["head.weight"][A:]
        out["actor.bias"], out["critic.bias"] = src["head.bias"][:A], src["head.bias"][A:]
        return out

    def named_views(self):
        return self._named(self.views)

    def named_grads(self):
        return self._named(self.grad_views)

    def state_dict(self):
        return {k: v.detach().clone() for k, v in self.named_views().items()}

    def load_state_dict(self, sd):
        nv = self.named_views()
        for k, v in nv.items():
            v.copy_(torch.as_tensor(sd[k], dtype=torch.float32).reshape(v.shape))

    def zero_state(self, n):
        z = torch.zeros(self.num_layers, n, self.hidden, dtype=torch.float32, device=self.device)
        return z, z.clone()

    def heads(self, obs, keep, h0, c0, work=None, want_heads=True):
        N, T, _ = obs.shape
        v = self.views
        x = obs
        saved = []
        work = work or {}
        heads = None
        if self._interleaved_forward_ok(N, work, T):
            self.begin_steps(h0, c0)
            keep_t = None if keep is None else keep.t().contiguous()
            kt = (lambda t: None) if keep_t is None else (lambda t: keep_t[t])
            if self.num_layers == 2 and getattr(self, "use_step_pairs", True):
                s0, s1 = self._steppers
                y0, y1, st0, st1 = work["y0"], work["y1"], work["stash0"], work["stash1"]
                s0.step(obs, 0, y0, st0, keep=kt(0))
                for t in range(T - 1):
                    ops.lstm_stepper_step_pair((s0, obs, t + 1, y0, st0, None, kt(t + 1)), (s1, y0, t, y1, st1, s0, kt(t)))
                s1.step(y0, T - 1, y1, st1, below=s0, keep=kt(T - 1))
            else:
                for t in range(T):
                    self.step_layers_at(obs, t, work, keep=kt(t))
            for l in range(self.num_layers):
                saved.append((x, work[f"stash{l}"], work[f"y{l}"], h0[l]))
                x = work[f"y{l}"]
            self._saved = (saved, keep, x)
            if not want_heads:
                return x.view(N * T, self.hidden)
            heads = work.get("heads")
            if heads is None or heads.shape[0] != N:
                heads = torch.empty(N, T, self.n_act + 1, dtype=torch.float32, device=obs.device)
            ops.gemm_rows(x.view(N * T, self.hidden), v["head.weight"], v["head.bias"], heads.view(N * T, self.n_act + 1))
            return heads.view(N * T, self.n_act + 1)
        for l in range(self.num_layers):
            top = want_heads and l == self.num_layers - 1
            if top:
                heads = work.get("heads")
                if heads is None or heads.shape[0] != N:
                    heads = torch.empty(N, T, self.n_act + 1, dtype=torch.float32, device=obs.device)
            y, hn, cn, stash = ops.lstm_fwd(x, keep, h0[l], c0[l], v[f"lstm.weight_ih_l{l}"], v[f"lstm.weight_hh_l{l}"],
                                            v[f"lstm.bias_ih_l{l}"], v[f"lstm.bias_hh_l{l}"],
                                            stash=work.get(f"stash{l}"), y=work.get(f"y{l}"),
                                            w_head=v["head.weight"] if top else None,
                                            b_head=v["head.bias"] if top else None, heads=heads if top else None)
            saved.append((x, stash, y, h0[l]))
            x = y
        self._saved = (saved, keep, x)
        if not want_heads:
            return x.view(N * T, self.hidden)
        return heads.view(N * T, self.n_act + 1)

    def adopt_forward(self, obs, keep, h0, stash, y):
        stashes = stash if isinstance(stash, (list, tuple)) else [stash]
        ys = y if isinstance(y, (list, tuple)) else [y]
        saved, x = [], obs
        for l in range(len(ys)):
            saved.append((x, stashes[l], ys[l], h0[l]))
            x = ys[l]
        self._saved = (saved, keep, x)
        N, T, H = x.shape
        return x.view(N * T, H)

    def _interleaved_forward_ok(self, N, work, T=None):
        if not getattr(self, "use_stepper_forward", True) or self.num_layers < 2 or self.hidden != 256:
            return False
        sp = getattr(self, "_steppers", None)
        if sp is None or sp[0].N != N or ops.lstm_bwd_caps(self.device, self.obs_dim, 256) == 0:
            return False
        return all(work.get(f"y{l}") is not None and work[f"y{l}"].shape[0] == N and work.get(f"stash{l}") is not None
                   and work[f"stash{l}"].shape[0] == N
                   and (T is None or (work[f"y{l}"].shape[1] == T and work[f"stash{l}"].shape[1] == T))
                   for l in range(self.num_layers))

    def steppers(self, N, device):
        if getattr(self, "_steppers", None) is None or self._steppers[0].N != N:
            self._steppers = [ops.LstmStepper(N, self.obs_dim if l == 0 else self.hidden, self.hidden, device)
                              for l in range(self.num_layers)]
        return self._steppers

    def begin_steps(self, h, c):
        v = self.views
        for l, sp in enumerate(self.steppers(h.shape[1], h.device)):
            sp.begin(v[f"lstm.weight_ih_l{l}"], v[f"lstm.weight_hh_l{l}"], v[f"lstm.bias_ih_l{l}"], v[f"lstm.bias_hh_l{l}"],
                     h[l], c[l])

    def step_at(self, obs_seq, t, work, heads_seq, keep=None):
        x = self.step_layers_at(obs_seq, t, work, keep=keep)
        v = self.views
        return ops.gemm_rows(x[:, t], v["head.weight"], v["head.bias"], heads_seq[:, t])

    def step_layers_at(self, obs_seq, t, work, keep=None):
        x = obs_seq
        for l, sp in enumerate(self._steppers):
            sp.step(x, t, work[f"y{l}"], work[f"stash{l}"], below=self._steppers[l - 1] if l > 0 and self.hidden == 256 else None,
                    keep=keep)
            x = work[f"y{l}"]
        return x

    def step(self, obs, h, c, keep=None, work=None, want_heads=True):
        N = obs.shape[0]
        x = obs.view(N, 1, -1)
        k = None if keep is None else keep.view(N, 1)
        work = work if work is not None else {}
        v = self.views
        for l in range(self.num_layers):
            st = work.get(f"step_stash{l}")
            if st is None:
                st = work[f"step_stash{l}"] = torch.empty(N, 1, 6 * self.hidden, dtype=torch.float32, device=obs.device)
            y, hn, cn, _ = ops.lstm_fwd(x, k, h[l], c[l], v[f"lstm.weight_ih_l{l}"], v[f"lstm.weight_hh_l{l}"],
                                        v[f"lstm.bias_ih_l{l}"], v[f"lstm.bias_hh_l{l}"], stash=st)
            h[l].copy_(hn)
            c[l].copy_(cn)
            x = y
        if not want_heads:
            return x
        return ops.gemm(x.view(N, self.hidden), v["head.weight"], trans_b=True, bias=v["head.bias"])

    def backward(self, dheads, work=None, dhead_bias=None):
        saved, keep, y_last = self._saved
        N, T, H = y_last.shape
        v, g = self.views, self.grad_views
        work = work or {}
        if dhead_bias is not None:
            if dhead_bias.data_ptr() != g["head.bias"].data_ptr():
                g["head.bias"].copy_(dhead_bias)
        else:
            ops.colsum(dheads, out=g["head.bias"])
        dy = None
        top_in = self.obs_dim if self.num_layers == 1 else self.hidden
        caps = ops.lstm_bwd_caps(dheads.device, top_in, self.hidden)
        fused_heads = bool(caps & 2)
        L = self.num_layers
        if L >= 2 and (caps & 4) and getattr(self, "use_stack_bwd", True):
            specs = []
            for l in reversed(range(L)):
                x, stash, y, h0 = saved[l]
                key = f"dgates{l}"
                dg_bytes = ops.lstm_dgates_bytes(N, T, H, dheads.device)
                if work.get(key) is None or work[key].numel() * 4 < dg_bytes:
                    work[key] = work["dgates"] if (l == L - 1 and work.get("dgates") is not None and work["dgates"].numel() * 4 >= dg_bytes) \
                        else ops.lstm_dgates(N, T, H, dheads.device)
                if l > 0 and (work.get(f"dx{l}") is None or work[f"dx{l}"].shape[0] != N):
                    work[f"dx{l}"] = torch.empty(N, T, H, dtype=torch.float32, device=dheads.device)
                specs.append({"stash": stash, "w_hh": v[f"lstm.weight_hh_l{l}"], "w_ih": v[f"lstm.weight_ih_l{l}"] if l > 0 else None,
                              "dgates": work[key], "dx": work[f"dx{l}"] if l > 0 else None})
            ops.lstm_bwd_stack(specs, keep, dheads=dheads.view(N, T, -1), w_head=v["head.weight"])
            for l in reversed(range(L)):
                x, stash, y, h0 = saved[l]
                top = (l == L - 1)
                ops.lstm_bwd(x, keep, stash, v[f"lstm.weight_ih_l{l}"], v[f"lstm.weight_hh_l{l}"], y, h0,
                             wgrad_dheads=dheads.view(N, T, -1) if top else None, dgates=work[f"dgates{l}"],
                             dw_ih=g[f"lstm.weight_ih_l{l}"], dw_hh=g[f"lstm.weight_hh_l{l}"], db=g[f"lstm.bias_ih_l{l}"],
                             dw_head=g["head.weight"] if top else None, want_dstate=False, bwd_done=True,
                             db_hh=g[f"lstm.bias_hh_l{l}"])
            self._saved = None
            return self.grad
        if not fused_heads:
            if work.get("dy") is None or work["dy"].shape[0] != N * T:
                work["dy"] = torch.empty(N * T, H, dtype=torch.float32, device=dheads.device)
            dy = ops.gemm(dheads, v["head.weight"], out=work["dy"]).view(N, T, H)
        for l in reversed(range(self.num_layers)):
            x, stash, y, h0 = saved[l]
            top = (l == self.num_layers - 1)
            use_dheads = top and fused_heads
            r = ops.lstm_bwd(x, keep, stash, v[f"lstm.weight_ih_l{l}"], v[f"lstm.weight_hh_l{l}"], y, h0,
                             dy=None if use_dheads else dy,
                             dheads=dheads.view(N, T, -1) if use_dheads else None,
                             w_head=v["head.weight"] if use_dheads else None,
                             wgrad_dheads=dheads.view(N, T, -1) if top else None,
                             need_dx=(l > 0), dgates=work.get("dgates"), dw_ih=g[f"lstm.weight_ih_l{l}"],
                             dw_hh=g[f"lstm.weight_hh_l{l}"], db=g[f"lstm.bias_ih_l{l}"],
                             dw_head=g["head.weight"] if top else None, want_dstate=False, db_hh=g[f"lstm.bias_hh_l{l}"])
            dy = r["dx"]
        self._saved = None
        return self.grad
```

Baseline: 74.75 million.

## Write LSTM backward dgates in env-tile blocks read directly by wgrad

Adds a tiled dgates layout where each 16-env tile and timestep forms a contiguous block. The backward-sequence kernel writes this layout and the split wgrad kernel reads it, so the scattered per-env row-strided stores and loads become contiguous block accesses. The policy turns it on by default for single-layer H=64/128. In exchange it adds a form-tracking table, an unpack kernel for f32 export, and consistency checks that fail if the setting changes between bwd and wgrad.

```diff
diff --git a/include/uavppo.h b/include/uavppo.h
--- a/include/uavppo.h
+++ b/include/uavppo.h
@@ -172,6 +172,10 @@
                  float* dc0, const float* w_ih, int I, float* dx, uav_stream stream);
 size_t uav_lstm_dgates_bytes(uav_ctx* ctx, int N, int T, int H);
 int uav_lstm_dgates_f32(uav_ctx* ctx, const float* dgates, int N, int T, int H, float* out, uav_stream stream);
+#define UAV_DGATES_ROWS  0
+#define UAV_DGATES_TILES 1
+int uav_set_dgates_form(uav_ctx* ctx, int form);
+int uav_get_dgates_form(const uav_ctx* ctx);
 #define UAV_BWD_FUSES_DX 1
 #define UAV_BWD_TAKES_DHEADS 2
 #define UAV_BWD_STACKS 4
diff --git a/uav-wrf-les-ppo-lstm_amd/csrc/common.h b/uav-wrf-les-ppo-lstm_amd/csrc/common.h
--- a/uav-wrf-les-ppo-lstm_amd/csrc/common.h
+++ b/uav-wrf-les-ppo-lstm_amd/csrc/common.h
@@ -31,6 +31,7 @@
     double* ftab;
     int lstm_arith;
     unsigned debug;
+    int dg_tiles;
     hipStream_t side[3];
     hipEvent_t side_ev[8];
     void* comm;
@@ -217,6 +218,20 @@
     __host__ __device__ const float* iscm(const void* base, int t) const { return isc(base, T) + (size_t)t * NP; }
 };
 
+struct DgTiles {
+    static constexpr int ENVS = 16, FORM = 2;
+    int T, H;
+    __host__ __device__ DgTiles(int t, int h) : T(t), H(h) {}
+    __host__ __device__ static bool shape_ok(int N, int T, int H) {
+        return (H == 64 || H == 128) && N % ENVS == 0 && T % 8 == 0 && T >= 8 && (int64_t)N * T * 4 * H < (1ll << 30);
+    }
+    __host__ __device__ unsigned block_floats() const { return 4u * H * ENVS; }
+    __host__ __device__ unsigned block(int tile, int t) const { return ((unsigned)tile * T + t) * block_floats(); }
+    __host__ __device__ unsigned line(int p, int w, int j) const { return (((unsigned)p * (H / 16) + w) * ENVS + j) * 32; }
+    __host__ __device__ unsigned unit4(int q, int w, int kq, int j) const { return line(q >> 1, w, j) + 16 * (q & 1) + 4 * kq; }
+    __host__ __device__ int gate_row(int p, int w, int c) const { return (2 * p + (c >> 4)) * H + 16 * w + (c & 15); }
+};
+
 __device__ __forceinline__ double wave_sum(double v) {
 #pragma unroll
     for (int o = 32; o > 0; o >>= 1) v += __shfl_down(v, o, 64);
diff --git a/uav-wrf-les-ppo-lstm_amd/csrc/ctx.hip b/uav-wrf-les-ppo-lstm_amd/csrc/ctx.hip
--- a/uav-wrf-les-ppo-lstm_amd/csrc/ctx.hip
+++ b/uav-wrf-les-ppo-lstm_amd/csrc/ctx.hip
@@ -86,6 +86,13 @@
     return 0;
 }
 
+int uav_set_dgates_form(uav_ctx* ctx, int form) {
+    UAV_REQUIRE(ctx && (form == UAV_DGATES_ROWS || form == UAV_DGATES_TILES), "uav_set_dgates_form: bad argument");
+    ctx->dg_tiles = form;
+    return 0;
+}
+int uav_get_dgates_form(const uav_ctx* ctx) { return ctx ? ctx->dg_tiles : -1; }
+
 void uav_destroy(uav_ctx* ctx) {
     if (!ctx) return;
     (void)uav_comm_destroy(ctx);
diff --git a/uav-wrf-les-ppo-lstm_amd/csrc/lstm.hip b/uav-wrf-les-ppo-lstm_amd/csrc/lstm.hip
--- a/uav-wrf-les-ppo-lstm_amd/csrc/lstm.hip
+++ b/uav-wrf-les-ppo-lstm_amd/csrc/lstm.hip
@@ -34,7 +34,8 @@
                   float* dw_hh, float* db, float* db_hh, hipStream_t st);
 int lstm_h3_bwd_stack(uav_ctx* ctx, int nl, const uav_lstm_bwd_layer* layers, const float* dy, const float* dheads,
                       const float* w_head, int n_heads, int N, int T, hipStream_t st);
-int lstm_wgrad_fused(uav_ctx* ctx, const float* dgates, const float* y, const float* keep, const float* h0,
+bool lstm_wgrad_split_shape(const uav_ctx* ctx, int N, int T, int H);
+int lstm_wgrad_fused(uav_ctx* ctx, const float* dgates, int dg_tiles, const float* y, const float* keep, const float* h0,
                      const float* x, int I, const float* dheads, int NH, int N, int T, int H,
                      float* dw_ih, float* dw_hh, float* db, float* db_hh, float* dw_head, hipStream_t st);
 
@@ -640,7 +641,7 @@
 __device__ __forceinline__ void lstm_bwd_split(
     const float* __restrict__ keep, const float* __restrict__ stash, const float* __restrict__ w_hh,
     const float* __restrict__ dheads, const float* __restrict__ w_head, int NH, const float* __restrict__ dhn,
-    const float* __restrict__ dcn, int N, int T, float* __restrict__ dgates, float* __restrict__ dh0,
+    const float* __restrict__ dcn, int N, int T, float* __restrict__ dgates, int dg_tiles, float* __restrict__ dh0,
     float* __restrict__ dc0) {
     using G = BwdSplitGeom<P, H>;
     using vec = typename P::vec;
@@ -689,6 +690,10 @@
         dc_next[0] = c4.x; dc_next[1] = c4.y; dc_next[2] = c4.z; dc_next[3] = c4.w;
     }
     const size_t srow = (size_t)n * T;
+    const DgTiles tl(T, H);
+    float* const dg_at0 = dgates + (dg_tiles ? (size_t)tl.block(blockIdx.x, 0) + tl.unit4(0, w, kq, j) : srow * (4 * H) + uo);
+    const unsigned dg_step = dg_tiles ? tl.block_floats() : 4u * H;
+    const unsigned dg_pair = dg_tiles ? tl.unit4(2, 0, 0, 0) : 2u * H, dg_half = dg_tiles ? tl.unit4(1, 0, 0, 0) : (unsigned)H;
 
     typedef __attribute__((address_space(3))) float lds_f;
     const int e_d = lane >> 2, g4 = lane & 3;
@@ -794,7 +799,7 @@
             unscale = __builtin_amdgcn_ldexpf(1.0f, -ex);
         }
         auto store_dg = [&](int q) {
-            if (live) *reinterpret_cast<float4*>(dgates + (srow + t) * (4 * H) + q * H + uo) = float4{dg[q][0], dg[q][1], dg[q][2], dg[q][3]};
+            if (live) *reinterpret_cast<float4*>(dg_at0 + (size_t)t * dg_step + (q >> 1) * dg_pair + (q & 1) * dg_half) = float4{dg[q][0], dg[q][1], dg[q][2], dg[q][3]};
         };
         vec bp[2][NP];
 #pragma unroll
@@ -849,17 +854,17 @@
 __global__ __launch_bounds__(H * 4) void lstm_bwd_h3k_kernel(
     const float* __restrict__ keep, const float* __restrict__ stash, const float* __restrict__ w_hh,
     const float* __restrict__ dheads, const float* __restrict__ w_head, int NH, const float* __restrict__ dhn,
-    const float* __restrict__ dcn, int N, int T, float* __restrict__ dgates, float* __restrict__ dh0,
+    const float* __restrict__ dcn, int N, int T, float* __restrict__ dgates, int dg_tiles, float* __restrict__ dh0,
     float* __restrict__ dc0) {
-    lstm_bwd_split<SplitF16x3, H>(keep, stash, w_hh, dheads, w_head, NH, dhn, dcn, N, T, dgates, dh0, dc0);
+    lstm_bwd_split<SplitF16x3, H>(keep, stash, w_hh, dheads, w_head, NH, dhn, dcn, N, T, dgates, dg_tiles, dh0, dc0);
 }
 template <int H>
 __global__ __launch_bounds__(H * 4) void lstm_bwd_x6k_kernel(
     const float* __restrict__ keep, const float* __restrict__ stash, const float* __restrict__ w_hh,
     const float* __restrict__ dheads, const float* __restrict__ w_head, int NH, const float* __restrict__ dhn,
-    const float* __restrict__ dcn, int N, int T, float* __restrict__ dgates, float* __restrict__ dh0,
+    const float* __restrict__ dcn, int N, int T, float* __restrict__ dgates, int dg_tiles, float* __restrict__ dh0,
     float* __restrict__ dc0) {
-    lstm_bwd_split<SplitBf16x6, H>(keep, stash, w_hh, dheads, w_head, NH, dhn, dcn, N, T, dgates, dh0, dc0);
+    lstm_bwd_split<SplitBf16x6, H>(keep, stash, w_hh, dheads, w_head, NH, dhn, dcn, N, T, dgates, dg_tiles, dh0, dc0);
 }
 
 template <class P, int H, bool FUSE_X>
@@ -881,12 +886,12 @@
 template <class P, int H>
 static int launch_bwd_split(const float* keep, const float* stash, const float* w_hh, const float* dheads,
                             const float* w_head, int NH, const float* dhn, const float* dcn, int N, int T, float* dgates,
-                            float* dh0, float* dc0, hipStream_t st) {
+                            int dg_tiles, float* dh0, float* dc0, hipStream_t st) {
     const dim3 grid((N + MT - 1) / MT), block(H * 4);
     const size_t lx = BwdSplitGeom<P, H>::LDS;
     constexpr auto kern = bwd_split_kernel<P, H>();
     UAV_CHECK_HIP(uav_dyn_lds(reinterpret_cast<const void*>(kern), (int)lx));
-    hipLaunchKernelGGL(kern, grid, block, lx, st, keep, stash, w_hh, dheads, w_head, NH, dhn, dcn, N, T, dgates, dh0, dc0);
+    hipLaunchKernelGGL(kern, grid, block, lx, st, keep, stash, w_hh, dheads, w_head, NH, dhn, dcn, N, T, dgates, dg_tiles, dh0, dc0);
     UAV_LAUNCH_CHECK();
     return 0;
 }
@@ -948,14 +953,33 @@
     if (i < n) b[i] = a0[i] + a1[i];
 }
 
+static bool lstm_bwd_is_split(const float* dheads, int NH) { return dheads && NH <= 7 && !uav_want_f32_mfma(); }
+
+static bool lstm_dg_tiles_ok(const uav_ctx* ctx, const float* dheads, int NH, int N, int T, int I, int H) {
+    return lstm_bwd_is_split(dheads, NH) && I >= 1 && I <= 6 && DgTiles::shape_ok(N, T, H) && lstm_wgrad_split_shape(ctx, N, T, H);
+}
+
+__global__ __launch_bounds__(256) void dg_tiles_unpack_kernel(const float* __restrict__ tiles, int N, int T, int H,
+                                                               float* __restrict__ out) {
+    const unsigned per_block = 16u * H;
+    const unsigned idx = blockIdx.x * 256u + threadIdx.x;
+    if (idx >= (unsigned)(N / 16) * T * per_block) return;
+    const unsigned b = idx / per_block, f = idx % per_block;
+    const int tile = b / T, t = b % T, NW = H / 16;
+    const int j = f & 15, kq = (f >> 4) & 3, w = (f >> 6) % NW, q = (f >> 6) / NW;
+    const DgTiles tl(T, H);
+    const float4 v = *reinterpret_cast<const float4*>(tiles + tl.block(tile, t) + tl.unit4(q, w, kq, j));
+    *reinterpret_cast<float4*>(out + ((size_t)(16 * tile + j) * T + t) * (4 * H) + q * H + 16 * w + 4 * kq) = v;
+}
+
 static int lstm_bwd_seq(const float* keep, const float* stash, const float* w_hh, const float* dy,
                         const float* dheads, const float* w_head, int NH, const float* dhn, const float* dcn, int N,
-                        int T, int H, float* dgates, float* dh0, float* dc0, hipStream_t st) {
-    if (dheads && NH <= 7 && !uav_want_f32_mfma()) {
+                        int T, int H, float* dgates, int dg_tiles, float* dh0, float* dc0, hipStream_t st) {
+    if (lstm_bwd_is_split(dheads, NH)) {
         return with_split([&](auto p) {
             using P = decltype(p);
-            return H == 64 ? launch_bwd_split<P, 64>(keep, stash, w_hh, dheads, w_head, NH, dhn, dcn, N, T, dgates, dh0, dc0, st)
-                           : launch_bwd_split<P, 128>(keep, stash, w_hh, dheads, w_head, NH, dhn, dcn, N, T, dgates, dh0, dc0, st);
+            return H == 64 ? launch_bwd_split<P, 64>(keep, stash, w_hh, dheads, w_head, NH, dhn, dcn, N, T, dgates, dg_tiles, dh0, dc0, st)
+                           : launch_bwd_split<P, 128>(keep, stash, w_hh, dheads, w_head, NH, dhn, dcn, N, T, dgates, dg_tiles, dh0, dc0, st);
         });
     }
     switch (H) {
@@ -1024,6 +1048,13 @@
 int uav_lstm_dgates_f32(uav_ctx* ctx, const float* dgates, int N, int T, int H, float* out, uav_stream stream) {
     UAV_REQUIRE(ctx && dgates && out && N > 0 && T > 0 && H > 0, "uav_lstm_dgates_f32: bad argument");
     uav_enter(ctx);
+    if ((H == 64 || H == 128) && uav_dg_form(ctx, dgates) == DgTiles::FORM) {
+        UAV_REQUIRE(DgTiles::shape_ok(N, T, H), "uav_lstm_dgates_f32: this buffer was written as tile blocks for another shape");
+        const unsigned n4 = (unsigned)N * T * H;
+        hipLaunchKernelGGL(dg_tiles_unpack_kernel, dim3((n4 + 255) / 256), dim3(256), 0, as_stream(stream), dgates, N, T, H, out);
+        UAV_LAUNCH_CHECK();
+        return 0;
+    }
     const int form = H == DgPack::H ? uav_dg_form(ctx, dgates) : 0;
     if (form > 0 || (form < 0 && H == DgPack::H && lstm_h3_dg_packed(H))) return lstm_pc_unpack(dgates, N, T, out, as_stream(stream));
     UAV_CHECK_HIP(hipMemcpyAsync(out, dgates, (size_t)N * T * 4 * H * sizeof(float), hipMemcpyDeviceToDevice, as_stream(stream)));
@@ -1055,8 +1086,11 @@
                                 as_stream(stream));
     }
     UAV_REQUIRE(!dx, "uav_lstm_bwd: dx is not formed by the H = 64 / 128 sequence kernels (uav_lstm_wgrad does it)");
-    return lstm_bwd_seq(keep, stash, w_hh, dy, dheads, w_head, n_heads, dhn, dcn, N, T, H, dgates, dh0, dc0,
-                        as_stream(stream));
+    const int tiles = ctx->dg_tiles == UAV_DGATES_TILES && lstm_dg_tiles_ok(ctx, dheads, n_heads, N, T, I, H);
+    const int rc = lstm_bwd_seq(keep, stash, w_hh, dy, dheads, w_head, n_heads, dhn, dcn, N, T, H, dgates, tiles, dh0, dc0,
+                                as_stream(stream));
+    if (rc == 0) uav_dg_record(ctx, dgates, tiles ? DgTiles::FORM : 0);
+    return rc;
 }
 
 int uav_lstm_wgrad(uav_ctx* ctx, const float* x, const float* keep, const float* h0, const float* y,
@@ -1070,8 +1104,20 @@
     hipStream_t st = as_stream(stream);
     const int64_t NT = (int64_t)N * T;
     int rc;
+    int tiles = 0;
+    if (H == 64 || H == 128) {
+        const int form = uav_dg_form(ctx, dgates);
+        const bool want = ctx->dg_tiles == UAV_DGATES_TILES && lstm_dg_tiles_ok(ctx, dheads, n_heads, N, T, I, H);
+        tiles = form == DgTiles::FORM;
+        UAV_REQUIRE(!tiles || (ctx->dg_tiles == UAV_DGATES_TILES && !uav_want_f32_mfma() && I <= 6 && !dx && DgTiles::shape_ok(N, T, H)),
+                    "uav_lstm_wgrad: this dgates buffer was written as tile blocks (uav_set_dgates_form) but the handle now reads f32 "
+                    "rows, or this call (arithmetic, I = %d, dx) cannot read tiles: the setting must not change between "
+                    "uav_lstm_bwd and uav_lstm_wgrad", I);
+        UAV_REQUIRE(form != 0 || !want, "uav_lstm_wgrad: this dgates buffer was written as f32 rows but the handle now reads tile "
+                    "blocks (uav_set_dgates_form must not change between uav_lstm_bwd and uav_lstm_wgrad)");
+    }
     if (I <= 6 && (H == 64 || H == 128)) {
-        if ((rc = lstm_wgrad_fused(ctx, dgates, y, keep, h0, x, I, dheads, n_heads, N, T, H, dw_ih, dw_hh, db, db_hh,
+        if ((rc = lstm_wgrad_fused(ctx, dgates, tiles, y, keep, h0, x, I, dheads, n_heads, N, T, H, dw_ih, dw_hh, db, db_hh,
                                    dw_head, st))) return rc;
     } else {
         UAV_REQUIRE(stash, "uav_lstm_wgrad: stash is required when I > 6");
diff --git a/uav-wrf-les-ppo-lstm_amd/csrc/wgrad.hip b/uav-wrf-les-ppo-lstm_amd/csrc/wgrad.hip
--- a/uav-wrf-les-ppo-lstm_amd/csrc/wgrad.hip
+++ b/uav-wrf-les-ppo-lstm_amd/csrc/wgrad.hip
@@ -271,7 +271,7 @@
 #define WX_PROF_FLUSH()
 #endif
 
-template <int H, bool HEADS, class P>
+template <int H, bool HEADS, class P, bool TILES>
 __device__ __forceinline__ void lstm_wgrad_split(
     const float* __restrict__ dgates, const float* __restrict__ y, const float* __restrict__ keep,
     const float* __restrict__ h0, const float* __restrict__ x, int I, const float* __restrict__ dheads, int NH,
@@ -287,6 +287,7 @@
     const int j = lane & 15, kq = lane >> 4;
     const int r_begin = blockIdx.x * rows_per_block;
     const int nslab = rows_per_block / KS6;
+    const DgTiles tl(T, H);
     P pol;
 
     const int c = tid % H;
@@ -307,8 +308,16 @@
     float raw[4][8];
     auto load_a_one = [&](int slab, int pair, int e) {
         slab = slab < nslab ? slab : nslab - 1;
-        const unsigned off = (unsigned)(r_begin + slab * KS6 + 8 * kq) * (4 * H) + 64 * w + 32 * pair + 2 * j;
-        const float2 t2 = *reinterpret_cast<const float2*>(dgates + (off + (unsigned)e * (4 * H)));
+        unsigned off, estep;
+        if constexpr (TILES) {
+            const unsigned q0 = (unsigned)(r_begin + slab * KS6 + 8 * kq), n = q0 / (unsigned)T, t = q0 - n * (unsigned)T;
+            off = tl.block(n >> 4, t) + tl.line(pair, w, n & 15) + 2 * j;
+            estep = tl.block_floats();
+        } else {
+            off = (unsigned)(r_begin + slab * KS6 + 8 * kq) * (4 * H) + 64 * w + 32 * pair + 2 * j;
+            estep = 4 * H;
+        }
+        const float2 t2 = *reinterpret_cast<const float2*>(dgates + (off + (unsigned)e * estep));
         raw[2 * pair][e] = t2.x;
         raw[2 * pair + 1][e] = t2.y;
     };
@@ -473,7 +482,7 @@
             const float usc = pol.row_unscale(mi, r, kq);
 #pragma unroll
             for (int ni = 0; ni < NT_; ++ni)
-                slab[(size_t)(64 * w + 32 * (mi >> 1) + 2 * (4 * kq + r) + (mi & 1)) * G::NC + 16 * ni + j] =
+                slab[(size_t)(TILES ? tl.gate_row(mi >> 1, w, 2 * (4 * kq + r) + (mi & 1)) : 64 * w + 32 * (mi >> 1) + 2 * (4 * kq + r) + (mi & 1)) * G::NC + 16 * ni + j] =
                     acc[mi][ni][r] * (ni == NT_ - 1 ? usc * (P::BSCALE / P::XSCALE) : usc);
         }
 #pragma unroll
@@ -485,14 +494,28 @@
     const float* __restrict__ dgates, const float* __restrict__ y, const float* __restrict__ keep,
     const float* __restrict__ h0, const float* __restrict__ x, int I, const float* __restrict__ dheads, int NH,
     int N, int T, int rows_per_block, float* __restrict__ slabs) {
-    lstm_wgrad_split<H, HEADS, WgBf16x6>(dgates, y, keep, h0, x, I, dheads, NH, N, T, rows_per_block, slabs);
+    lstm_wgrad_split<H, HEADS, WgBf16x6, false>(dgates, y, keep, h0, x, I, dheads, NH, N, T, rows_per_block, slabs);
 }
 template <int H, bool HEADS>
 __global__ __launch_bounds__(H * 4) void lstm_wgrad_h3_kernel(
     const float* __restrict__ dgates, const float* __restrict__ y, const float* __restrict__ keep,
     const float* __restrict__ h0, const float* __restrict__ x, int I, const float* __restrict__ dheads, int NH,
     int N, int T, int rows_per_block, float* __restrict__ slabs) {
-    lstm_wgrad_split<H, HEADS, WgF16x3>(dgates, y, keep, h0, x, I, dheads, NH, N, T, rows_per_block, slabs);
+    lstm_wgrad_split<H, HEADS, WgF16x3, false>(dgates, y, keep, h0, x, I, dheads, NH, N, T, rows_per_block, slabs);
+}
+template <int H, bool HEADS>
+__global__ __launch_bounds__(H * 4) void lstm_wgrad_x6_kernel_tiles(
+    const float* __restrict__ dgates, const float* __restrict__ y, const float* __restrict__ keep,
+    const float* __restrict__ h0, const float* __restrict__ x, int I, const float* __restrict__ dheads, int NH,
+    int N, int T, int rows_per_block, float* __restrict__ slabs) {
+    lstm_wgrad_split<H, HEADS, WgBf16x6, true>(dgates, y, keep, h0, x, I, dheads, NH, N, T, rows_per_block, slabs);
+}
+template <int H, bool HEADS>
+__global__ __launch_bounds__(H * 4) void lstm_wgrad_h3_kernel_tiles(
+    const float* __restrict__ dgates, const float* __restrict__ y, const float* __restrict__ keep,
+    const float* __restrict__ h0, const float* __restrict__ x, int I, const float* __restrict__ dheads, int NH,
+    int N, int T, int rows_per_block, float* __restrict__ slabs) {
+    lstm_wgrad_split<H, HEADS, WgF16x3, true>(dgates, y, keep, h0, x, I, dheads, NH, N, T, rows_per_block, slabs);
 }
 
 template <int H>
@@ -525,16 +548,16 @@
     }
 }
 
-template <class P, int H, bool HEADS>
+template <class P, int H, bool HEADS, bool TILES>
 static constexpr auto wgrad_split_kernel() {
-    if constexpr (std::is_same<P, WgF16x3>::value) return &lstm_wgrad_h3_kernel<H, HEADS>;
-    else return &lstm_wgrad_x6_kernel<H, HEADS>;
-}
-
-template <class P, int H>
+    if constexpr (std::is_same<P, WgF16x3>::value) return TILES ? &lstm_wgrad_h3_kernel_tiles<H, HEADS> : &lstm_wgrad_h3_kernel<H, HEADS>;
+    else return TILES ? &lstm_wgrad_x6_kernel_tiles<H, HEADS> : &lstm_wgrad_x6_kernel<H, HEADS>;
+}
+
+template <class P, int H, bool TILES = false>
 static int launch_wgrad_split(const float* dgates, const float* y, const float* keep, const float* h0, const float* x, int I,
                               const float* dheads, int NH, int N, int T, int nb, int rpb, float* slabs, hipStream_t st) {
-    const auto kern = dheads ? wgrad_split_kernel<P, H, true>() : wgrad_split_kernel<P, H, false>();
+    const auto kern = dheads ? wgrad_split_kernel<P, H, true, TILES>() : wgrad_split_kernel<P, H, false, TILES>();
     const size_t lds = WGS<H, P>::LDS;
     UAV_CHECK_HIP(uav_dyn_lds(reinterpret_cast<const void*>(kern), (int)lds));
     hipLaunchKernelGGL(kern, dim3(nb), dim3(H * 4), lds, st, dgates, y, keep, h0, x, I, dheads, NH, N, T, rpb, slabs);
@@ -542,7 +565,28 @@
 }
 
 template <int H>
-static int launch_wgrad(uav_ctx* ctx, const float* dgates, const float* y, const float* keep, const float* h0,
+static bool wgrad_split_cut(const uav_ctx* ctx, int64_t NTr, int* nbx, int64_t* rpx) {
+    int nb = ctx->num_cu;
+    const int64_t max_nb = (int64_t)(ctx->ws_bytes / (WG<H>::SLAB * sizeof(float)));
+    if (nb > max_nb) nb = (int)max_nb;
+    if (nb < 1) return false;
+    int64_t rpb = (NTr + nb - 1) / nb;
+    rpb = (rpb + KC - 1) / KC * KC;
+    nb = (int)((NTr + rpb - 1) / rpb);
+    *rpx = (NTr + nb - 1) / nb;
+    *rpx = (*rpx + KS6 - 1) / KS6 * KS6;
+    *nbx = (int)((NTr + *rpx - 1) / *rpx);
+    return NTr % *rpx == 0;
+}
+bool lstm_wgrad_split_shape(const uav_ctx* ctx, int N, int T, int H) {
+    int nbx;
+    int64_t rpx;
+    const int64_t NTr = (int64_t)N * T;
+    return T >= 8 && NTr * 4 * H < (1ll << 30) && (H == 64 ? wgrad_split_cut<64>(ctx, NTr, &nbx, &rpx) : H == 128 && wgrad_split_cut<128>(ctx, NTr, &nbx, &rpx));
+}
+
+template <int H>
+static int launch_wgrad(uav_ctx* ctx, const float* dgates, int dg_tiles, const float* y, const float* keep, const float* h0,
                         const float* x, int I, const float* dheads, int NH, int N, int T,
                         float* dw_ih, float* dw_hh, float* db, float* db_hh, float* dw_head, hipStream_t st) {
     using G = WG<H>;
@@ -556,15 +600,18 @@
     nb = (int)((NTr + rpb - 1) / rpb);
     float* slabs = (float*)ctx->ws;
     {
-        int64_t rpx = (NTr + nb - 1) / nb;
-        rpx = (rpx + KS6 - 1) / KS6 * KS6;
-        const int nbx = (int)((NTr + rpx - 1) / rpx);
-        const bool split_ok = (NTr % rpx == 0) && T >= 8 && I <= 6 && (!dheads || NH <= 8) && NTr * 4 * H < (1ll << 30) &&
+        int64_t rpx = 0;
+        int nbx = 0;
+        const bool split_ok = wgrad_split_cut<H>(ctx, NTr, &nbx, &rpx) && T >= 8 && I <= 6 && (!dheads || NH <= 8) && NTr * 4 * H < (1ll << 30) &&
                               !uav_want_f32_mfma();
+        UAV_REQUIRE(!dg_tiles || (split_ok && DgTiles::shape_ok(N, T, H)), "uav_lstm_wgrad: tile-form dgates need the split kernels' shapes, "
+                    "N %% 16 == 0, T %% 8 == 0, I <= 6 and a split arithmetic");
         if (split_ok) {
-            const int rc = uav_want_bf16x6()
-                               ? launch_wgrad_split<WgBf16x6, H>(dgates, y, keep, h0, x, I, dheads, NH, N, T, nbx, (int)rpx, slabs, st)
-                               : launch_wgrad_split<WgF16x3, H>(dgates, y, keep, h0, x, I, dheads, NH, N, T, nbx, (int)rpx, slabs, st);
+            const bool x6 = uav_want_bf16x6();
+            const int rc = dg_tiles ? (x6 ? launch_wgrad_split<WgBf16x6, H, true>(dgates, y, keep, h0, x, I, dheads, NH, N, T, nbx, (int)rpx, slabs, st)
+                                          : launch_wgrad_split<WgF16x3, H, true>(dgates, y, keep, h0, x, I, dheads, NH, N, T, nbx, (int)rpx, slabs, st))
+                           : x6 ? launch_wgrad_split<WgBf16x6, H>(dgates, y, keep, h0, x, I, dheads, NH, N, T, nbx, (int)rpx, slabs, st)
+                                : launch_wgrad_split<WgF16x3, H>(dgates, y, keep, h0, x, I, dheads, NH, N, T, nbx, (int)rpx, slabs, st);
             if (rc) return rc;
             hipLaunchKernelGGL((wgrad_reduce_kernel<H>), dim3((unsigned)((G::SLAB + 255) / 256)), dim3(256), 0, st, slabs,
                                nbx, I, NH, dw_ih, dw_hh, db, db_hh, dw_head);
@@ -581,12 +628,12 @@
     return 0;
 }
 
-int lstm_wgrad_fused(uav_ctx* ctx, const float* dgates, const float* y, const float* keep, const float* h0,
+int lstm_wgrad_fused(uav_ctx* ctx, const float* dgates, int dg_tiles, const float* y, const float* keep, const float* h0,
                      const float* x, int I, const float* dheads, int NH, int N, int T, int H,
                      float* dw_ih, float* dw_hh, float* db, float* db_hh, float* dw_head, hipStream_t st) {
     switch (H) {
-        case 64: return launch_wgrad<64>(ctx, dgates, y, keep, h0, x, I, dheads, NH, N, T, dw_ih, dw_hh, db, db_hh, dw_head, st);
-        case 128: return launch_wgrad<128>(ctx, dgates, y, keep, h0, x, I, dheads, NH, N, T, dw_ih, dw_hh, db, db_hh, dw_head, st);
+        case 64: return launch_wgrad<64>(ctx, dgates, dg_tiles, y, keep, h0, x, I, dheads, NH, N, T, dw_ih, dw_hh, db, db_hh, dw_head, st);
+        case 128: return launch_wgrad<128>(ctx, dgates, dg_tiles, y, keep, h0, x, I, dheads, NH, N, T, dw_ih, dw_hh, db, db_hh, dw_head, st);
     }
     uav_set_error("lstm_wgrad_fused: H=%d unsupported", H);
     return 2;
diff --git a/uav-wrf-les-ppo-lstm_amd/uavppo/_lib.py b/uav-wrf-les-ppo-lstm_amd/uavppo/_lib.py
--- a/uav-wrf-les-ppo-lstm_amd/uavppo/_lib.py
+++ b/uav-wrf-les-ppo-lstm_amd/uavppo/_lib.py
@@ -95,6 +95,8 @@
     "uav_lstm_bwd_caps": (I32, [P, I32, I32]),
     "uav_lstm_dgates_bytes": (SZ, [P, I32, I32, I32]),
     "uav_lstm_dgates_f32": (I32, [P, P, I32, I32, I32, P, P]),
+    "uav_set_dgates_form": (I32, [P, I32]),
+    "uav_get_dgates_form": (I32, [P]),
     "uav_lstm_bwd_stack": (I32, [P, I32, P, P, P, P, I32, I32, I32, I32, P]),
     "uav_lstm_wgrad": (I32, [P, P, P, P, P, P, P, P, P, I32, I32, I32, I32, I32, P, P, P, P, P, P, P]),
     "uav_lstm_chunk_states": (I32, [P, P, P, P, P, P, I32, I32, I32, I32, P, P, P]),
diff --git a/uav-wrf-les-ppo-lstm_amd/uavppo/ops.py b/uav-wrf-les-ppo-lstm_amd/uavppo/ops.py
--- a/uav-wrf-les-ppo-lstm_amd/uavppo/ops.py
+++ b/uav-wrf-les-ppo-lstm_amd/uavppo/ops.py
@@ -300,6 +300,18 @@
 
 def set_debug_flags(*names, device=None):
     check(lib().uav_set_debug_flags(Context.get(device).handle, sum(DEBUG_FLAGS[n] for n in names)), "uav_set_debug_flags")
+
+
+DGATES_FORMS = {"rows": 0, "tiles": 1}
+
+
+def set_dgates_form(form, device=None):
+    check(lib().uav_set_dgates_form(Context.get(device).handle, DGATES_FORMS[form]), "uav_set_dgates_form")
+
+
+def get_dgates_form(device=None):
+    m = int(lib().uav_get_dgates_form(Context.get(device).handle))
+    return {v: k for k, v in DGATES_FORMS.items()}[m]
 
 
 def rccl_version():
@@ -703,7 +715,14 @@
     return out
 
 
-def lstm_wgrad(x, keep, h0, y, stash, dgates, w_ih, dheads=None):
+def lstm_wgrad(x, keep, h0, y, stash, dgates, w_ih, dheads=None, dgates_form=None):
+    if dgates_form is not None:
+        prev = get_dgates_form(x.device)
+        set_dgates_form(dgates_form, x.device)
+        try:
+            return lstm_wgrad(x, keep, h0, y, stash, dgates, w_ih, dheads=dheads)
+        finally:
+            set_dgates_form(prev, x.device)
     N, T, I = x.shape
     H = y.shape[-1]
     dev = x.device
@@ -749,7 +768,16 @@
 
 def lstm_bwd(x, keep, stash, w_ih, w_hh, y, h0, dy=None, dheads=None, w_head=None, dhn=None, dcn=None, need_dx=False,
              dgates=None, dw_ih=None, dw_hh=None, db=None, dw_head=None, want_dstate=True, wgrad_dheads=None, bwd_done=False,
-             db_hh=None):
+             db_hh=None, dgates_form=None):
+    if dgates_form is not None:
+        prev = get_dgates_form(x.device)
+        set_dgates_form(dgates_form, x.device)
+        try:
+            return lstm_bwd(x, keep, stash, w_ih, w_hh, y, h0, dy=dy, dheads=dheads, w_head=w_head, dhn=dhn, dcn=dcn,
+                            need_dx=need_dx, dgates=dgates, dw_ih=dw_ih, dw_hh=dw_hh, db=db, dw_head=dw_head,
+                            want_dstate=want_dstate, wgrad_dheads=wgrad_dheads, bwd_done=bwd_done, db_hh=db_hh)
+        finally:
+            set_dgates_form(prev, x.device)
     N, T, I = x.shape
     H = w_hh.shape[1]
     dev = x.device
diff --git a/uav-wrf-les-ppo-lstm_amd/uavppo/policy.py b/uav-wrf-les-ppo-lstm_amd/uavppo/policy.py
--- a/uav-wrf-les-ppo-lstm_amd/uavppo/policy.py
+++ b/uav-wrf-les-ppo-lstm_amd/uavppo/policy.py
@@ -98,6 +98,7 @@
 class LSTMActorCritic(_FlatPolicy):
     def __init__(self, obs_dim=6, hidden=128, num_layers=1, n_act=5, device="cuda", seed=0):
         self.obs_dim, self.hidden, self.num_layers, self.n_act = obs_dim, hidden, num_layers, n_act
+        self.dgates_form = "tiles"
         H, A = hidden, n_act
         layout = []
         for l in range(num_layers):
@@ -310,7 +311,8 @@
                              wgrad_dheads=dheads.view(N, T, -1) if top else None,
                              need_dx=(l > 0), dgates=work.get("dgates"), dw_ih=g[f"lstm.weight_ih_l{l}"],
                              dw_hh=g[f"lstm.weight_hh_l{l}"], db=g[f"lstm.bias_ih_l{l}"],
-                             dw_head=g["head.weight"] if top else None, want_dstate=False, db_hh=g[f"lstm.bias_hh_l{l}"])
+                             dw_head=g["head.weight"] if top else None, want_dstate=False, db_hh=g[f"lstm.bias_hh_l{l}"],
+                             dgates_form=self.dgates_form if (L == 1 and H in (64, 128)) else None)
             dy = r["dx"]
         self._saved = None
         return self.grad
```

Result: no change. 74.74 million (median of 2 runs) (-0.0%).
